# zouyunkai/MedicalSemSeg

Measured on AMD Instinct MI355X. Metric: 96^3 vols/sec fwd+bwd (train), higher is better.
Workload: dtype bf16; 1 GPU; UNet base (MONAI BasicUNet 32-32-64-128-256-32) 1->3cls, 96^3 patches, DiceCE + AdamW, per-GPU batch 2; global_batch=2, parallelism=dp1, grad_sync=none (single rank)

## Files before the change

include/msseg.h:

```cpp
#ifndef MSSEG_H_
#define MSSEG_H_

#include <stddef.h>
#include <stdint.h>

#ifdef __cplusplus
extern "C" {
#endif

#define MSSEG_ABI_VERSION 1

#define MSSEG_OK 0
#define MSSEG_EINVAL (-1)
#define MSSEG_ELAUNCH (-2)
#define MSSEG_EWORKSPACE (-3)

#define MSSEG_F32 0
#define MSSEG_BF16 1

typedef void* msseg_stream_t;

int msseg_abi_version(void);
const char* msseg_last_error(void);
int msseg_num_cus(void);

int msseg_ktimer_enable(int on);
int msseg_ktimer_reset(void);
int msseg_ktimer_count(void);
int msseg_ktimer_get(int i, char* name, int cap, float* ms);

size_t msseg_packed_weight_bytes(int M, int T, int K, int cout_block, int dtype);
int msseg_pack_weights(const float* src, void* dst, int dtype, int M, int M0, int T, int K, int K0,
                       long long s_m1, long long s_m0, long long s_t, long long s_k1, long long s_k0,
                       int flip, int cout_block, msseg_stream_t stream);
typedef struct msseg_pack_job {
    const float* src;
    void* dst;
    long long s_m1, s_m0, s_t, s_k1, s_k0;
    long long total;
    int M, M0, T, K, K0, flip, cout_block, nkb;
} msseg_pack_job;
int msseg_pack_weights_batch(const msseg_pack_job* jobs_dev, int njobs, long long max_total, long long sum_total, int dtype,
                             msseg_stream_t stream);
int msseg_cout_block(int M);
int msseg_conv3d_k3_cout_block(int N, int D, int H, int W, int Cout);
int msseg_conv3d_k3_variant(int N, int D, int H, int W, int Cout);
int msseg_conv3d_k3_kernel(int N, int D, int H, int W, int Cin, int Cout, int dtype);

int msseg_conv3d_k3_fwd(const void* x, long long ldx, const void* wp, const float* bias, void* y, long long ldy,
                        int N, int D, int H, int W, int Cin, int Cout, float* stats ,
                        void* scratch, size_t scratch_bytes, int dtype, msseg_stream_t stream);
int msseg_conv3d_k3_fwd_accumulate(const void* x, long long ldx, const void* wp, void* y, long long ldy, int N, int D, int H,
                                   int W, int Cin, int Cout, float* stats, void* scratch, size_t scratch_bytes, int dtype,
                                   msseg_stream_t stream);
int msseg_conv3d_k3_dgrad_inbwd(const void* dy, long long lddy, const void* wp, void* da, long long ldda, int N, int D,
                                int H, int W, int Cin, int Cout, const void* yraw, long long ldyraw, const void* act,
                                long long ldact, const float* fwd_stats, float slope, float eps, float* red,
                                float* dgamma, float* dbeta, int accumulate, void* scratch, size_t scratch_bytes,
                                int dtype, msseg_stream_t stream);
int msseg_conv3d_k3s2_fwd(const void* x, long long ldx, const void* wp, const float* bias, void* y, long long ldy,
                          int N, int ID, int IH, int IW, int Cin, int Cout, int dtype, msseg_stream_t stream);
int msseg_zero_stuff2(const void* dy, long long lddy, void* out, long long ldo, int N, int OD, int OH, int OW, int ID,
                      int IH, int IW, int C, int dtype, msseg_stream_t stream);
int msseg_conv3d_stem_fwd(const void* x, long long ldx, const void* wp, const float* bias, void* y, long long ldy,
                          int N, int D, int H, int W, int Cout, float* stats, void* scratch, size_t scratch_bytes,
                          int dtype, msseg_stream_t stream);
int msseg_conv3d_stem_k1_fwd(const void* x, long long ldx, const void* wp, const float* bias, void* y, long long ldy,
                             int N, int D, int H, int W, int Cout, float* stats, void* scratch, size_t scratch_bytes,
                             int dtype, msseg_stream_t stream);
int msseg_conv3d_stem_norm_fwd(const void* x, long long ldx, const void* wp, const float* bias, const float* stats,
                               const float* gamma, const float* beta, float eps, float slope, void* y, long long ldy, int N,
                               int D, int H, int W, int Cout, int dtype, msseg_stream_t stream);
int msseg_conv3d_k1_fwd(const void* x, long long ldx, const void* wp, const float* bias, void* y, long long ldy,
                        long long NV, int Cin, int Cout, int dtype, msseg_stream_t stream);
int msseg_conv3d_k1_head_fwd(const void* x, long long ldx, const float* w, const float* bias, void* y, long long ldy,
                             long long NV, int Cin, int Cout, int dtype, msseg_stream_t stream);
int msseg_conv3d_k1_head_dgrad_inbwd(const void* dy, long long lddy, const float* w, void* da, long long ldda, int N,
                                     long long S, int C, int Cout, const void* yraw, long long ldyraw,
                                     const float* fwd_stats, const float* gamma, const float* beta, float slope, float eps,
                                     float* red, float* dgamma, float* dbeta, int accumulate, void* scratch,
                                     size_t scratch_bytes, int dtype, msseg_stream_t stream);
int msseg_conv3d_k1_head_norm_fwd(const void* x, long long ldx, const float* stats, const float* gamma, const float* beta,
                                  float slope, float eps, const float* w, const float* bias, void* y, long long ldy, int N,
                                  long long S, int Cin, int Cout, int dtype, msseg_stream_t stream);
int msseg_conv3d_k1_head_bwd_fused(const void* dy, long long lddy, const float* w, void* da, long long ldda, int N,
                                   long long S, int C, int Cout, const void* yraw, long long ldyraw, const float* fwd_stats,
                                   const float* gamma, const float* beta, float slope, float eps, float* red, float* dgamma,
                                   float* dbeta, int accumulate, float* dw, int dw_accumulate, void* scratch,
                                   size_t scratch_bytes, int dtype, msseg_stream_t stream);

int msseg_conv3d_gather_fwd(const void* x, long long ldx, const void* wp, const float* bias, void* y, long long ldy,
                            int N, int ID, int IH, int IW, int Cin, int Cout, int k, int s, int p, int dtype,
                            msseg_stream_t stream);
int msseg_deconv_k2s2_fwd(const void* x, long long ldx, const void* wp, const float* bias, void* y, long long ldy,
                          int N, int D, int H, int W, int Cin, int Cout, int dtype, msseg_stream_t stream);
int msseg_deconv_k2s2_bwd_data(const void* dy, long long lddy, const void* wp, void* dx, long long lddx,
                               int N, int D, int H, int W, int Cin, int Cout, int dtype, msseg_stream_t stream);
int msseg_deconv_k4s4_fwd(const void* x, long long ldx, const void* wp, const float* bias, void* y, long long ldy,
                          int N, int D, int H, int W, int Cin, int Cout, int dtype, msseg_stream_t stream);
int msseg_deconv_k4s4_bwd_data(const void* dy, long long lddy, const void* wp, void* dx, long long lddx,
                               int N, int D, int H, int W, int Cin, int Cout, int dtype, msseg_stream_t stream);
int msseg_conv3d_k1_dgrad_inbwd(const void* dy, long long lddy, const void* wp, void* da, long long ldda, int N,
                                long long S, int Cin, int Cout, const void* yraw, long long ldyraw, const void* act,
                                long long ldact, const float* fwd_stats, float slope, float eps, float* red,
                                float* dgamma, float* dbeta, int accumulate, void* scratch, size_t scratch_bytes,
                                int dtype, msseg_stream_t stream);
int msseg_deconv_k2s2_bwd_data_inbwd(const void* dy, long long lddy, const void* wp, void* dx, long long lddx, int N,
                                     int D, int H, int W, int Cin, int Cout, const void* yraw, long long ldyraw,
                                     const void* act, long long ldact, const float* fwd_stats, float slope, float eps,
                                     float* red, float* dgamma, float* dbeta, int accumulate, void* scratch,
                                     size_t scratch_bytes, int dtype, msseg_stream_t stream);
int msseg_deconv_k2s2_bwd_fused(const void* dy, long long lddy, const void* wp, void* dx, long long lddx, int N,
                                int D, int H, int W, int Cin, int Cout, const void* yraw, long long ldyraw,
                                const void* act, long long ldact, const float* fwd_stats, float slope, float eps,
                                float* red, float* dgamma, float* dbeta, int accumulate, float* dbias, int dbias_accumulate,
                                void* scratch, size_t scratch_bytes, int dtype, msseg_stream_t stream);

int msseg_deconv_k2s2_bwd_partials_ok(int Cin, int Cout, int dtype);
int msseg_deconv_k2s2_bwd_partials(const void* dy, long long lddy, const void* wp, float* part, size_t part_bytes, int N,
                                   int D, int H, int W, int Cin, int Cout, int dtype, msseg_stream_t stream);


size_t msseg_wgrad_workspace_bytes(int M, int T, int K);
int msseg_conv3d_k3_wgrad_kernel(int N, int D, int H, int W, int Cin, int Cout, int dtype);
int msseg_conv3d_k3_wgrad(const void* x, long long ldx, const void* dy, long long lddy, float* dw,
                          int N, int D, int H, int W, int Cin, int Cout, int accumulate,
                          void* workspace, size_t workspace_bytes, int dtype, msseg_stream_t stream);
int msseg_conv3d_k1_wgrad(const void* x, long long ldx, const void* dy, long long lddy, float* dw,
                          long long NV, int Cin, int Cout, int accumulate,
                          void* workspace, size_t workspace_bytes, int dtype, msseg_stream_t stream);
int msseg_linear_wgrad_ok(long long NV, int Cin, int Cout, int dtype);
int msseg_linear_wgrad(const void* x, long long ldx, const void* dy, long long lddy, float* dw, float* dbias, long long NV,
                       int Cin, int Cout, int accumulate_w, int accumulate_b, void* workspace, size_t workspace_bytes,
                       int dtype, msseg_stream_t stream);
int msseg_conv3d_gather_wgrad(const void* x, long long ldx, const void* dy, long long lddy, float* dw,
                              int N, int ID, int IH, int IW, int Cin, int Cout, int k, int s, int p, int accumulate,
                              void* workspace, size_t workspace_bytes, int dtype, msseg_stream_t stream);
int msseg_deconv_k2s2_wgrad(const void* x, long long ldx, const void* dy, long long lddy, float* dw,
                            int N, int D, int H, int W, int Cin, int Cout, int accumulate,
                            void* workspace, size_t workspace_bytes, int dtype, msseg_stream_t stream);
int msseg_deconv_k4s4_wgrad(const void* x, long long ldx, const void* dy, long long lddy, float* dw,
                            int N, int D, int H, int W, int Cin, int Cout, int accumulate,
                            void* workspace, size_t workspace_bytes, int dtype, msseg_stream_t stream);

int msseg_conv3d_k3_small_ok(int N, int D, int H, int W, int Cin, int Cout, int dtype);
int msseg_conv3d_k3_small_stage_groups(int N, int D, int H, int W, int Cin, int Cout);
size_t msseg_conv3d_k3_small_workspace_bytes(int N, int D, int H, int W, int Cin, int Cout);
int msseg_conv3d_k3_small_partials(const void* x, long long ldx, const void* wp, float* part, size_t part_bytes, int N,
                                   int D, int H, int W, int Cin, int Cout, msseg_stream_t stream);
int msseg_conv3d_k3_small_fwd_finish(const float* part, int nstages, const float* bias, const float* gamma,
                                     const float* beta, float eps, float slope, void* yraw, long long ldy, void* act,
                                     long long lda, void* pooled, long long ldp, float* stats, int N, int D, int H, int W,
                                     int Cout, msseg_stream_t stream);
int msseg_conv3d_k3_small_fwd_finish_res(const float* part, int nstages, const float* bias, const float* gamma,
                                         const float* beta, float eps, float slope, void* yraw, long long ldy, void* act,
                                         long long lda, const void* residual, long long ldr, void* pooled, long long ldp,
                                         float* stats, int N, int D, int H, int W, int Cout, msseg_stream_t stream);
int msseg_conv3d_k3_small_bwd_finish(const float* part, int nstages, void* dx, long long lddx, const void* unit_yraw,
                                     long long lduy, const float* unit_stats, const float* unit_gamma,
                                     const float* unit_beta, float eps, float slope, float* dgamma, float* dbeta,
                                     int accumulate, int N, int D, int H, int W, int Cin, msseg_stream_t stream);

int msseg_dwconv3d_k3_fwd(const void* x, long long ldx, const void* w_taps, const float* bias, void* y, long long ldy, int N,
                          int D, int H, int W, int C, int flip, int dtype, msseg_stream_t stream);
int msseg_avgpool3d_k3(const void* x, long long ldx, void* y, long long ldy, int N, int D, int H, int W, int C, int dtype,
                       msseg_stream_t stream);
int msseg_dwconv3d_k3_wgrad(const void* x, long long ldx, const void* dy, long long lddy, float* dw, float* dbias,
                            int accumulate_w, int accumulate_b, int N, int D, int H, int W, int C, void* scratch,
                            size_t scratch_bytes, int dtype, msseg_stream_t stream);

int msseg_interp_trilinear_fwd(const void* x, long long ldx, void* y, long long ldy, int N, int ID, int IH, int IW, int OD,
                               int OH, int OW, int C, int dtype, msseg_stream_t stream);
size_t msseg_interp_trilinear_bwd_workspace_bytes(int N, int ID, int IH, int IW, int OD, int OH, int OW, int C);
int msseg_interp_trilinear_bwd(const void* dy, long long lddy, void* dx, long long lddx, int N, int ID, int IH, int IW, int OD,
                               int OH, int OW, int C, void* workspace, size_t workspace_bytes, int dtype, msseg_stream_t stream);
int msseg_kv_attention_fwd(const void* q, const void* kv, void* o, float* lse, int B, int N, int M, int heads, int head_dim,
                           float scale, int dtype, msseg_stream_t stream);
size_t msseg_kv_attention_bwd_workspace_bytes(int B, int N, int M, int heads, int head_dim);
int msseg_kv_attention_bwd(const void* q, const void* kv, const void* o, const float* lse, const void* dout, void* dq, void* dkv,
                           int B, int N, int M, int heads, int head_dim, float scale, void* workspace, size_t workspace_bytes,
                           int dtype, msseg_stream_t stream);
int msseg_scale_channels(const void* x, const float* scale, void* y, int N, long long S, int C, int dtype, msseg_stream_t stream);

size_t msseg_reduce_scratch_bytes(void);
int msseg_channel_stats(const void* x, long long ldx, float* stats, int N, long long S, int C, void* scratch,
                        size_t scratch_bytes, int dtype, msseg_stream_t stream);
int msseg_instnorm_act_fwd(const void* x, long long ldx, const float* stats, const float* gamma, const float* beta,
                           const void* residual, long long ldr, void* y, long long ldy, int N, long long S, int C,
                           float eps, float slope, int dtype, msseg_stream_t stream);
int msseg_instnorm_act_pool_fwd(const void* x, long long ldx, const float* stats, const float* gamma, const float* beta,
                                void* y, long long ldy, void* pooled, long long ldp, int N, int D, int H, int W, int C,
                                float eps, float slope, int dtype, msseg_stream_t stream);
int msseg_instnorm_act_poolbwd_reduce(const void* x, long long ldx, const float* stats, const float* gamma,
                                      const float* beta, const void* skip, long long lds, const void* g, long long ldg,
                                      void* da, long long ldda, float* red, float* dgamma, float* dbeta, int accumulate,
                                      int N, int D, int H, int W, int C, float eps, float slope, void* scratch,
                                      size_t scratch_bytes, int dtype, msseg_stream_t stream);
int msseg_instnorm_act_bwd_reduce(const void* x, long long ldx, const float* stats, const float* gamma,
                                  const float* beta, const void* y, long long ldy,
                                  const void* dy, long long lddy, float* red, float* dgamma, float* dbeta,
                                  int accumulate, int N, long long S, int C, float eps, float slope, void* scratch,
                                  size_t scratch_bytes, int dtype, msseg_stream_t stream);
int msseg_instnorm_act_bwd_apply(const void* x, long long ldx, const float* stats, const float* gamma,
                                 const float* beta, const void* y, long long ldy, const void* dy, long long lddy, const float* red, void* dx,
                                 long long lddx, void* dres, long long lddres, int N, long long S, int C, float eps,
                                 float slope, int dtype, msseg_stream_t stream);
int msseg_maxpool2_fwd(const void* x, long long ldx, void* y, long long ldy, int N, int D, int H, int W, int C,
                       int dtype, msseg_stream_t stream);
int msseg_maxpool2_bwd(const void* x, long long ldx, const void* dy, long long lddy, void* dx, long long lddx,
                       int N, int D, int H, int W, int C, int accumulate, int dtype, msseg_stream_t stream);
int msseg_ncdhw_to_ndhwc(const void* src, int src_dtype, void* dst, long long ldd, int dst_dtype, int N, int C,
                         long long S, msseg_stream_t stream);
int msseg_ndhwc_to_ncdhw(const void* src, long long lds, int src_dtype, void* dst, int dst_dtype, int N, int C,
                         long long S, msseg_stream_t stream);
int msseg_channel_sum(const void* x, long long ldx, float* out, long long rows, int C, int accumulate, void* scratch,
                      size_t scratch_bytes, int dtype, msseg_stream_t stream);
int msseg_add(const void* a, long long lda, const void* b, long long ldb, void* y, long long ldy, long long rows,
              int C, int dtype, msseg_stream_t stream);
int msseg_axpy_rows(const void* a, const void* b, const float* scale, void* y, int N, long long elems_per_sample, int dtype,
                    msseg_stream_t stream);


int msseg_window_attention_fwd(const void* qkv, const float* qkv_bias, const float* table, void* out, float* lse, int B,
                               int S, int H, int W, int C, int heads, int ws, int shift, int dtype,
                               msseg_stream_t stream);
int msseg_window_attention_bwd(const void* qkv, const float* qkv_bias, const float* table, const void* out,
                               const float* lse, const void* dout, void* dqkv, float* dtable, int B, int S, int H, int W,
                               int C, int heads, int ws, int shift, int dtype, msseg_stream_t stream);
size_t msseg_window_attention_bwd_workspace_bytes(int B, int S, int H, int W, int C, int heads, int ws, int shift, int dtype);
int msseg_window_attention_fwd2(const void* qkv, const float* qkv_bias, const float* table, void* out, float* lse, int B,
                                int S, int H, int W, int C, int heads, int ws, int shift, int bias_ws, int dtype,
                                msseg_stream_t stream);
int msseg_window_attention_bwd2(const void* qkv, const float* qkv_bias, const float* table, const void* out,
                                const float* lse, const void* dout, void* dqkv, float* dtable, int B, int S, int H, int W,
                                int C, int heads, int ws, int shift, int bias_ws, int dtype, void* workspace,
                                size_t workspace_bytes, msseg_stream_t stream);
int msseg_window_attention_bwd_ws(const void* qkv, const float* qkv_bias, const float* table, const void* out,
                                  const float* lse, const void* dout, void* dqkv, float* dtable, int B, int S, int H, int W,
                                  int C, int heads, int ws, int shift, int dtype, void* workspace, size_t workspace_bytes,
                                  msseg_stream_t stream);
int msseg_window_attention_fwd3(const void* qkv, const float* qkv_bias, const float* table, void* out, float* lse, int B,
                                int S, int H, int W, int C, int heads, int ws, int shift, int bias_ws, long long table_stride,
                                int dtype, msseg_stream_t stream);
int msseg_window_attention_bwd3(const void* qkv, const float* qkv_bias, const float* table, const void* out,
                                const float* lse, const void* dout, void* dqkv, float* dtable, int B, int S, int H, int W,
                                int C, int heads, int ws, int shift, int bias_ws, long long table_stride, int dtype,
                                void* workspace, size_t workspace_bytes, msseg_stream_t stream);
size_t msseg_window_attention_bwd3_workspace_bytes(int B, int S, int H, int W, int C, int heads, int ws, int shift,
                                                   int bias_ws, long long table_stride, int dtype);
int msseg_rel_bias_affine_fold(const float* table, const float* emb, const float* lin_w, const float* lin_b,
                               const float* aff, float* T, int B, int M3, int heads, msseg_stream_t stream);
size_t msseg_rel_bias_affine_grad_workspace_bytes(int M3, int heads);
#define MSSEG_AFFINE_ACC_TABLE 1
#define MSSEG_AFFINE_ACC_EMB 2
#define MSSEG_AFFINE_ACC_LIN_W 4
#define MSSEG_AFFINE_ACC_LIN_B 8
int msseg_rel_bias_affine_grad(const float* dT, const float* emb, const float* lin_w, const float* aff, float* dtable,
                               float* demb, float* dlin_w, float* dlin_b, int B, int M3, int heads, int flags,
                               void* workspace, size_t workspace_bytes, msseg_stream_t stream);
int msseg_layernorm_fwd(const void* x, long long ldx, const float* gamma, const float* beta, void* y, long long ldy,
                        float* mean, float* rstd, long long rows, int C, float eps, int dtype, msseg_stream_t stream);
int msseg_layernorm_bwd(const void* x, long long ldx, const float* gamma, const float* mean, const float* rstd,
                        const void* dy, long long lddy, void* dx, long long lddx, long long rows, int C, int dtype,
                        msseg_stream_t stream);
int msseg_layernorm_bwd_add(const void* x, long long ldx, const float* gamma, const float* mean, const float* rstd,
                            const void* dy, long long lddy, const void* add, long long ldadd, void* dx, long long lddx,
                            long long rows, int C, int dtype, msseg_stream_t stream);
int msseg_layernorm_param_grad(const void* x, long long ldx, const float* mean, const float* rstd, const void* dy,
                               long long lddy, float* dgamma, float* dbeta, int accumulate, long long rows, int C,
                               void* scratch, size_t scratch_bytes, int dtype, msseg_stream_t stream);
int msseg_gelu_fwd(const void* x, void* y, long long n, int dtype, msseg_stream_t stream);
int msseg_gelu_bwd(const void* x, const void* dy, void* dx, long long n, int dtype, msseg_stream_t stream);
int msseg_linear_gelu_ok(long long NV, int Cin, int Cout, int dtype);
int msseg_linear_gelu_fwd(const void* x, long long ldx, const void* wp, const float* bias, void* pre, long long ldpre, void* act,
                          long long ldact, long long NV, int Cin, int Cout, int dtype, msseg_stream_t stream);
int msseg_linear_gelu_bwd(const void* dy, long long lddy, const void* wp, const void* pre, long long ldpre, void* dpre,
                          long long lddpre, long long NV, int Cin, int Cout, int dtype, msseg_stream_t stream);
int msseg_linear_add_ok(long long NV, int Cin, int Cout, int dtype);
int msseg_linear_add_fwd(const void* x, long long ldx, const void* wp, const float* bias, const void* res, long long ldres,
                         void* y, long long ldy, long long NV, int Cin, int Cout, int dtype, msseg_stream_t stream);
// ... 74 lines not shown
```

medicalsemseg_amd/csrc/common.h:

```cpp
#pragma once
#include <hip/hip_runtime.h>
#include <stdint.h>
#include <stdio.h>

#include "../../include/msseg.h"

typedef __bf16 bf16_t;
typedef __attribute__((ext_vector_type(8))) __bf16 bf16x8_t;
typedef __attribute__((ext_vector_type(4))) __bf16 bf16x4_t;
typedef __attribute__((ext_vector_type(4))) float f32x4_t;
typedef __attribute__((ext_vector_type(4))) uint32_t u32x4_t;
typedef __attribute__((ext_vector_type(2))) uint32_t u32x2_t;

#define MSSEG_DEVFN __device__ __forceinline__

void msseg_set_error(const char* fmt, ...);
#define MSSEG_FAIL(code, ...)           \
    do {                                \
        msseg_set_error(__VA_ARGS__);   \
        return (code);                  \
    } while (0)
#define MSSEG_CHECK_LAUNCH(name)                                              \
    do {                                                                      \
        hipError_t e__ = hipGetLastError();                                   \
        if (e__ != hipSuccess) MSSEG_FAIL(MSSEG_ELAUNCH, "%s: %s", name, hipGetErrorString(e__)); \
    } while (0)

bool msseg_ktimer_on();
int msseg_ktimer_begin(const char* name, hipStream_t stream);
void msseg_ktimer_end(int slot, hipStream_t stream);
#define MSSEG_KTIMED(name, stream, launch_stmt)                               \
    do {                                                                      \
        const int kt__ = msseg_ktimer_on() ? msseg_ktimer_begin(name, stream) : -1; \
        launch_stmt;                                                          \
        if (kt__ >= 0) msseg_ktimer_end(kt__, stream);                        \
    } while (0)

#include <atomic>
struct msseg_lds_attr_once {
    std::atomic<unsigned long long> done{0};
    bool ensure(const void* kern, int bytes) {
        int dev = 0;
        if (hipGetDevice(&dev) != hipSuccess) return false;
        const bool tracked = dev >= 0 && dev < 64;
        if (tracked && ((done.load(std::memory_order_acquire) >> dev) & 1ull)) return true;
        if (hipFuncSetAttribute(kern, hipFuncAttributeMaxDynamicSharedMemorySize, bytes) != hipSuccess) return false;
        if (tracked) done.fetch_or(1ull << dev, std::memory_order_release);
        return true;
    }
};

template <typename T> struct DT;
template <> struct DT<float> {
    static constexpr int EPC = 4;
    static constexpr int CODE = MSSEG_F32;
    static MSSEG_DEVFN float ld(const float* p) { return *p; }
    static MSSEG_DEVFN void st(float* p, float v) { *p = v; }
};
template <> struct DT<bf16_t> {
    static constexpr int EPC = 8;
    static constexpr int CODE = MSSEG_BF16;
    static MSSEG_DEVFN float ld(const bf16_t* p) { return (float)*p; }
    static MSSEG_DEVFN void st(bf16_t* p, float v) { *p = (bf16_t)v; }
};

template <typename T> MSSEG_DEVFN void mma_chunk(f32x4_t& acc, const u32x4_t& a, const u32x4_t& b);
template <> MSSEG_DEVFN void mma_chunk<bf16_t>(f32x4_t& acc, const u32x4_t& a, const u32x4_t& b) {
    acc = __builtin_amdgcn_mfma_f32_16x16x32_bf16(__builtin_bit_cast(bf16x8_t, a), __builtin_bit_cast(bf16x8_t, b),
                                                  acc, 0, 0, 0);
}
template <> MSSEG_DEVFN void mma_chunk<float>(f32x4_t& acc, const u32x4_t& a, const u32x4_t& b) {
    f32x4_t af = __builtin_bit_cast(f32x4_t, a), bf = __builtin_bit_cast(f32x4_t, b);
#pragma unroll
    for (int j = 0; j < 4; ++j) acc = __builtin_amdgcn_mfma_f32_16x16x4f32(af[j], bf[j], acc, 0, 0, 0);
}

template <typename T> MSSEG_DEVFN void store4(T* p, const f32x4_t& v);
template <> MSSEG_DEVFN void store4<float>(float* p, const f32x4_t& v) { *(f32x4_t*)p = v; }
template <> MSSEG_DEVFN void store4<bf16_t>(bf16_t* p, const f32x4_t& v) {
    bf16x4_t o = {(bf16_t)v[0], (bf16_t)v[1], (bf16_t)v[2], (bf16_t)v[3]};
    *(bf16x4_t*)p = o;
}

MSSEG_DEVFN float wave_sum(float v) {
#pragma unroll
    for (int o = 32; o > 0; o >>= 1) v += __shfl_xor(v, o);
    return v;
}

MSSEG_DEVFN bool grid_last_block(unsigned int* counter, unsigned int total_blocks, int* lds_flag) {
    asm volatile("s_waitcnt vmcnt(0)" ::: "memory");
    __syncthreads();
    if (threadIdx.x == 0) {
        __builtin_amdgcn_fence(__ATOMIC_RELEASE, "agent");
        asm volatile("s_waitcnt vmcnt(0)" ::: "memory");
        const unsigned int prev = __hip_atomic_fetch_add(counter, 1u, __ATOMIC_RELAXED, __HIP_MEMORY_SCOPE_AGENT);
        const int last = (prev == total_blocks - 1u) ? 1 : 0;
        if (last) {
            __builtin_amdgcn_fence(__ATOMIC_ACQUIRE, "agent");
            asm volatile("s_waitcnt vmcnt(0)" ::: "memory");
            __hip_atomic_store(counter, 0u, __ATOMIC_RELAXED, __HIP_MEMORY_SCOPE_AGENT);
        }
        *lds_flag = last;
    }
    __syncthreads();
    return *lds_flag != 0;
}

template <int NT>
MSSEG_DEVFN void block_rows_sum(const float* rows, int R, int L, float* lds, long long stride = 0) {
    const int tid = threadIdx.x, q = L >> 2;
    const int SL = NT / q;
    const int c4 = tid % q, slot = tid / q;
    const long long q_stride = (stride ? stride : (long long)L) >> 2;
    f32x4_t* l4 = (f32x4_t*)lds;
    if (slot < SL) {
        f32x4_t acc = {0.f, 0.f, 0.f, 0.f};
        const f32x4_t* src = (const f32x4_t*)rows + c4;
#pragma unroll 8
        for (int x = slot; x < R; x += SL) acc += src[(long long)x * q_stride];
        l4[slot * q + c4] = acc;
    }
    __syncthreads();
    if (tid < q) {
        f32x4_t t = {0.f, 0.f, 0.f, 0.f};
        for (int sl = 0; sl < SL; ++sl) t += l4[sl * q + tid];
        l4[NT + tid] = t;
    }
    __syncthreads();
}

#define MSSEG_SCRATCH_COUNTER_BYTES 256
#define MSSEG_STATS_NMAX 8

static inline int ceil_div(int a, int b) { return (a + b - 1) / b; }
static inline long long ceil_div_ll(long long a, long long b) { return (a + b - 1) / b; }
```

medicalsemseg_amd/csrc/conv3d_k3_pp.hip:

```cpp
#include "k3pp.h"

#include <type_traits>

namespace {

constexpr int TD = 4, TH = 4, TW = 16;
constexpr int PD = TD + 2, PH = TH + 2, PW = TW + 2;
constexpr int HV = PD * PH * PW;
constexpr int PLANE = ((HV * 16 + 255) / 256) * 256;
constexpr int HALO_BYTES = 4 * PLANE;
constexpr int W_BYTES = 27 * 4 * 32 * 16;
constexpr int STAT_FLOATS = 8 * MSSEG_STATS_NMAX * 32 * 2;
constexpr int NTHREADS = 512;

__device__ u32x4_t g_zero_chunk;
__device__ unsigned long long g_k3pp_cycles[8];

MSSEG_DEVFN void glds16(const void* g, void* l) {
    __builtin_amdgcn_global_load_lds((const __attribute__((address_space(1))) void*)g,
                                     (__attribute__((address_space(3))) void*)l, 16, 0, 0);
}

struct TileCo { int n, d0, h0, w0; };

// ... 107 lines not shown
        for (int m = 0; m < TH; ++m)
#pragma unroll
            for (int j = 0; j < 2; ++j) acc[m][j] = bv[j];
        const int v0 = (wq * PH) * PW + r;
        const unsigned char* xb[8];
#pragma unroll
        for (int k = 0; k < 8; ++k)
            xb[k] = ldsH + grp * HALO_BYTES + v0 * 64 + ((q ^ ((((v0 + k) >> 2) & 1) << 1)) * 16);
        const unsigned char* wb = ldsW + (q * 32 + r) * 16;
        constexpr int NSTEP = 9 * PH;
        constexpr int XAHEAD = 3;
        u32x4_t wf[2][3][2], xf[XAHEAD + 1];
        auto ldw = [&](int g, int i) {
            const int kh = i >> 1, j = i & 1;
            const int tap = (g / 3) * 9 + kh * 3 + (g % 3);
            wf[g & 1][kh][j] = *(const u32x4_t*)(wb + tap * 2048 + j * 256);
        };
        auto ldx = [&](int s) {
            const int g = s / PH, hr = s % PH;
            const int off = ((g / 3) * PH + hr) * PW + (g % 3);
            xf[s % (XAHEAD + 1)] = *(const u32x4_t*)(xb[off & 7] + off * 64);
        };
#pragma unroll
        for (int i = 0; i < 6; ++i) ldw(0, i);
#pragma unroll
        for (int s = 0; s < XAHEAD; ++s) ldx(s);
#pragma unroll
        for (int g = 0; g < 9; ++g) {
#pragma unroll
            for (int hr = 0; hr < PH; ++hr) {
                const int s = g * PH + hr;
                if (s + XAHEAD < NSTEP) ldx(s + XAHEAD);
                if (g + 1 < 9) ldw(g + 1, hr);
                __builtin_amdgcn_sched_barrier(0);
#pragma unroll
                for (int kh = 0; kh < 3; ++kh) {
                    const int m = hr - kh;
                    if (m >= 0 && m < TH) {
#pragma unroll
                        for (int j = 0; j < 2; ++j)
                            mma_chunk<bf16_t>(acc[m][j], wf[g & 1][kh][j], xf[s % (XAHEAD + 1)]);
                    }
                }
                __builtin_amdgcn_sched_barrier(0);
            }
        }
    };

    unsigned o_off[TH], ny_off[TH], na_off[TH];
#pragma unroll
    for (int m = 0; m < TH; ++m) {
        const long long rel = ((long long)wq * p.H + m) * p.W + r;
        o_off[m] = (unsigned)(rel * p.ldy * 2 + q * 8);
        ny_off[m] = (unsigned)(rel * p.nb_ldy * 2 + q * 8);
        na_off[m] = (unsigned)(rel * p.nb_lda * 2 + q * 8);
    }
    float s1[2][4], s2[2][4];
    int s_n = -1;
#pragma unroll
    for (int j = 0; j < 2; ++j)
#pragma unroll
        for (int e = 0; e < 4; ++e) s1[j][e] = s2[j][e] = 0.f;
    auto flush_stats = [&]() {
        if (s_n < 0) return;
        float* slot = ldsS + ((wave * MSSEG_STATS_NMAX + s_n) * 32) * 2;
#pragma unroll
        for (int j = 0; j < 2; ++j)
#pragma unroll
            for (int e = 0; e < 4; ++e) {
                float a = s1[j][e], b = s2[j][e];
#pragma unroll
                for (int o = 1; o < 16; o <<= 1) {
                    a += __shfl_xor(a, o);
                    b += __shfl_xor(b, o);
                }
                if (r == 0) {
                    float* sp = slot + (j * 16 + q * 4 + e) * 2;
                    sp[0] += a;
                    sp[1] += b;
                }
                s1[j][e] = s2[j][e] = 0.f;
            }
    };
    auto epilogue = [&](const TileCo& tc) {
        if constexpr (STATS != 0) {
            if (tc.n != s_n) { flush_stats(); s_n = tc.n; }
        }
        const long long vox = (((long long)tc.n * p.D + tc.d0) * p.H + tc.h0) * p.W + tc.w0;
        unsigned char* ybase = (unsigned char*)yg + (vox * p.ldy + coutblk * 32) * 2;
        const unsigned char* nyb = (const unsigned char*)p.nb_y + (vox * p.nb_ldy + coutblk * 32) * 2;
        const unsigned char* nab = (const unsigned char*)p.nb_a + (vox * p.nb_lda + coutblk * 32) * 2;
        const bool full = tc.d0 + TD <= p.D && tc.h0 + TH <= p.H && tc.w0 + TW <= p.W;
        auto body = [&](auto fullc) {
            constexpr bool FULL = decltype(fullc)::value;
            const bool okdw = FULL || (tc.d0 + wq < p.D && tc.w0 + r < p.W);
            u32x2_t y4[TH][2], a4[TH][2];
            if constexpr (STATS == 2) {
#pragma unroll
                for (int m = 0; m < TH; ++m)
#pragma unroll
                    for (int j = 0; j < 2; ++j) {
                        const bool ok = FULL || (okdw && tc.h0 + m < p.H);
                        y4[m][j] = a4[m][j] = u32x2_t{0u, 0u};
                        if (ok) {
                            y4[m][j] = *(const u32x2_t*)(nyb + ny_off[m] + j * 32);
                            a4[m][j] = *(const u32x2_t*)(nab + na_off[m] + j * 32);
                        }
                    }
            }
            u32x2_t ob[TH][2];
            if constexpr (STATS == 3) {
                u32x2_t yo[TH][2];
#pragma unroll
                for (int m = 0; m < TH; ++m)
#pragma unroll
                    for (int j = 0; j < 2; ++j) {
                        const bool ok = FULL || (okdw && tc.h0 + m < p.H);
                        yo[m][j] = ok ? *(const u32x2_t*)(ybase + o_off[m] + j * 32) : u32x2_t{0u, 0u};
                    }
#pragma unroll
                for (int m = 0; m < TH; ++m)
#pragma unroll
                    for (int j = 0; j < 2; ++j)
#pragma unroll
                        for (int e = 0; e < 4; ++e) acc[m][j][e] += bf16_of_pair(yo[m][j][e >> 1], e & 1);
            }
#pragma unroll
            for (int m = 0; m < TH; ++m)
#pragma unroll
                for (int j = 0; j < 2; ++j) {
                    const bool ok = FULL || (okdw && tc.h0 + m < p.H);
                    const f32x4_t o = acc[m][j];
                    ob[m][j] = u32x2_t{pack_bf16x2(o[0], o[1]), pack_bf16x2(o[2], o[3])};
                    if (ok) *(u32x2_t*)(ybase + o_off[m] + j * 32) = ob[m][j];
                }
            if constexpr (STATS != 0) {
#pragma unroll
                for (int m = 0; m < TH; ++m)
#pragma unroll
                    for (int j = 0; j < 2; ++j) {
                        const bool ok = FULL || (okdw && tc.h0 + m < p.H);
#pragma unroll
                        for (int e = 0; e < 4; ++e) {
                            float v = bf16_of_pair(ob[m][j][e >> 1], e & 1);
                            if (!FULL) v = ok ? v : 0.f;
                            if constexpr (STATS == 1 || STATS == 3) {
                                acc_add(s1[j][e], v);
                                acc_fma(s2[j][e], v, v);
                            } else {
                                const float av = bf16_of_pair(a4[m][j][e >> 1], e & 1);
                                const float dz = v * (av > 0.f ? 1.0f : p.nb_slope);
                                acc_add(s1[j][e], dz);
                                acc_fma(s2[j][e], dz, bf16_of_pair(y4[m][j][e >> 1], e & 1));
                            }
                        }
                    }
            }
        };
        if (full) body(std::true_type{});
        else body(std::false_type{});
    };

    for (int ph = 0; ph <= n_my; ++ph) {
        unsigned long long t0 = 0;
        if constexpr (TIMING) t0 = __builtin_readcyclecounter();
        if ((ph & 1) == grp) {
            if (ph < n_my) compute();
            if constexpr (TIMING) tcyc[0] += __builtin_readcyclecounter() - t0;
        } else {
            if (ph + 1 < n_my) load_halo(tile_of(ph + 1));
            if constexpr (TIMING) {
                tcyc[4] += __builtin_readcyclecounter() - t0; t0 = __builtin_readcyclecounter();
                asm volatile("s_waitcnt vmcnt(0)" ::: "memory");
                tcyc[5] += __builtin_readcyclecounter() - t0; t0 = __builtin_readcyclecounter();
            }
            if (ph >= 1) epilogue(tile_of(ph - 1));
            if constexpr (TIMING) tcyc[1] += __builtin_readcyclecounter() - t0;
        }
        if constexpr (TIMING) t0 = __builtin_readcyclecounter();
        asm volatile("s_waitcnt vmcnt(0)" ::: "memory");
        if constexpr (TIMING) { tcyc[2] += __builtin_readcyclecounter() - t0; t0 = __builtin_readcyclecounter(); }
        __syncthreads();
        if constexpr (TIMING) tcyc[3] += __builtin_readcyclecounter() - t0;
    }
    if constexpr (TIMING) {
        if (blockIdx.x == 0 && blockIdx.y == 0 && lane == 0 && wave == 0) {
#pragma unroll
            for (int k = 0; k < 6; ++k) g_k3pp_cycles[k] = tcyc[k];
        }
    }

    if constexpr (STATS != 0) {
        flush_stats();
        __syncthreads();
        const int PN = p.N * 32 * 2;
        float* wsp = p.stats_ws + ((long long)blockIdx.y * gridDim.x + blockIdx.x) * PN;
        for (int i = tid; i < PN; i += NTHREADS) {
            float s = 0.f;
#pragma unroll
            for (int wv = 0; wv < 8; ++wv) s += ldsS[wv * MSSEG_STATS_NMAX * 64 + i];
            wsp[i] = s;
        }
    }
}

template <int STATS, int TIMING> int launch(const K3ppParams& p, hipStream_t stream) {
    const int lds = W_BYTES + 2 * HALO_BYTES + (STATS ? STAT_FLOATS * 4 : 0);
    auto kern = k3pp_kernel<STATS, TIMING>;
    static msseg_lds_attr_once attr;
    if (!attr.ensure((const void*)kern, lds)) MSSEG_FAIL(MSSEG_ELAUNCH, "conv3d_k3_pp: cannot set dynamic LDS size %d", lds);
    const int ncb = p.M / 32;
    const int tiles = p.N * ceil_div(p.D, TD) * ceil_div(p.H, TH) * ceil_div(p.W, TW);
    int gx = msseg_num_cus() / ncb;
    gx &= ~7;
    if (gx < 8) gx = 8;
    if (gx > tiles) gx = tiles;
    MSSEG_KTIMED("k3pp_kernel", stream, hipLaunchKernelGGL(kern, dim3(gx, ncb, 1), dim3(NTHREADS), lds, stream, p));
    MSSEG_CHECK_LAUNCH("conv3d_k3_pp");
    if (STATS != 0) {
        K3FinParams f{};
        f.ws = p.stats_ws; f.R = gx; f.N = p.N; f.coutb = 32; f.M = p.M; f.stats = p.stats;
        f.nb_stats = (STATS == 2) ? p.nb_stats : nullptr; f.nb_eps = p.nb_eps; f.nb_S = p.nb_S;
        f.nb_dgamma = p.nb_dgamma; f.nb_dbeta = p.nb_dbeta; f.nb_acc = p.nb_acc;
        return msseg_k3_stats_finalize(f, ncb, stream);
    }
    return MSSEG_OK;
}

}

bool msseg_k3pp_eligible(const K3ppParams& p) {
    if (p.K != 32 || p.M % 32 || p.M > 256) return false;
    if ((p.ldx % 8) || (p.ldy % 4) || ((uintptr_t)p.x & 15) || ((uintptr_t)p.y & 7)) return false;
    if (p.bias && ((uintptr_t)p.bias & 15)) return false;
    if (p.stats && p.N > MSSEG_STATS_NMAX) return false;
    if (p.nb_y && ((p.nb_ldy % 4) || (p.nb_lda % 4) || ((uintptr_t)p.nb_y & 7) || ((uintptr_t)p.nb_a & 7))) return false;
    const long long tiles = (long long)p.N * ceil_div(p.D, TD) * ceil_div(p.H, TH) * ceil_div(p.W, TW);
    if (tiles > 0x7fffffffLL) return false;
    return tiles * (p.M / 32) >= 2LL * msseg_num_cus();
}

int msseg_k3pp_launch(const K3ppParams& p, hipStream_t stream) {
    static const bool timing = getenv("MSSEG_K3PP_TIMING") != nullptr;
    if (p.accumulate) {
        if (p.stats == nullptr || p.nb_y != nullptr) MSSEG_FAIL(MSSEG_EINVAL, "conv3d_k3_pp: accumulate mode comes with forward statistics");
        return launch<3, 0>(p, stream);
    }
    if (p.stats == nullptr) return timing ? launch<0, 1>(p, stream) : launch<0, 0>(p, stream);
    if (p.nb_y == nullptr) return timing ? launch<1, 1>(p, stream) : launch<1, 0>(p, stream);
    return launch<2, 0>(p, stream);
}

extern "C" int msseg_debug_k3pp_cycles(unsigned long long* out8) {
    return hipMemcpyFromSymbol(out8, HIP_SYMBOL(g_k3pp_cycles), 8 * sizeof(unsigned long long)) == hipSuccess ? 0 : -1;
}
```

medicalsemseg_amd/csrc/elementwise.hip:

```cpp
#include "common.h"

#include <stdarg.h>
#include <string.h>

static thread_local char g_err[512] = "";
void msseg_set_error(const char* fmt, ...) {
    va_list ap;
    va_start(ap, fmt);
    vsnprintf(g_err, sizeof(g_err), fmt, ap);
    va_end(ap);
}

extern "C" {
int msseg_abi_version(void) { return MSSEG_ABI_VERSION; }
const char* msseg_last_error(void) { return g_err; }
int msseg_num_cus(void) {
    static int cus = 0;
    if (cus == 0) {
        int dev = 0;
        hipDeviceProp_t prop;
        if (hipGetDevice(&dev) == hipSuccess && hipGetDeviceProperties(&prop, dev) == hipSuccess)
            cus = prop.multiProcessorCount;
        if (cus <= 0) cus = 256;
    }
// ... 243 lines not shown
            }
        }
    }
}

inline long long reduce_blocks(long long S, int rows_par, int N, int C, int nper);

template <typename T>
int launch_ln_param_grad(const void* x, long long ldx, const void* dy, long long lddy, const float* mean, const float* rstd,
                         float* dgamma, float* dbeta, int accumulate, long long rows, int C, void* scratch, hipStream_t st) {
    const bool vec = vec_ok(x, ldx, C, sizeof(T)) && vec_ok(dy, lddy, C, sizeof(T));
    const RowMap m = row_map(C, vec ? DT<T>::EPC : 1);
    long long blocks = reduce_blocks(rows, m.rows_par, 1, C, 2);
    const long long rpb = ceil_div_ll(rows, blocks);
    blocks = ceil_div_ll(rows, rpb);
    unsigned int* counter = (unsigned int*)scratch;
    float* ws = (float*)((unsigned char*)scratch + MSSEG_SCRATCH_COUNTER_BYTES);
    if (vec)
        hipLaunchKernelGGL((ln_param_grad_kernel<T, true>), dim3((unsigned)blocks), dim3(256), 0, st, (const T*)x, ldx,
                           (const T*)dy, lddy, mean, rstd, rows, C, m.groups, m.rows_par, rpb, ws, counter, dgamma, dbeta, accumulate);
    else
        hipLaunchKernelGGL((ln_param_grad_kernel<T, false>), dim3((unsigned)blocks), dim3(256), 0, st, (const T*)x, ldx,
                           (const T*)dy, lddy, mean, rstd, rows, C, m.groups, m.rows_par, rpb, ws, counter, dgamma, dbeta, accumulate);
    MSSEG_CHECK_LAUNCH("ln_param_grad");
    {
        FinalizeArgs a{ws, 1, (int)blocks, C, 2, 2, ws + blocks * C * 2, dgamma, dbeta, accumulate};
        hipLaunchKernelGGL(channels_finalize_kernel, channels_finalize_grid(a), dim3(256), 0, st, a);
        MSSEG_CHECK_LAUNCH("channels_finalize");
    }
    return MSSEG_OK;
}

inline long long reduce_blocks(long long S, int rows_par, int N, int C, int nper) {
    long long blocks = ceil_div_ll(S, (long long)rows_par * 8);
    long long cap = (long long)msseg_num_cus() / (N > 0 ? N : 1);
    if (cap < 1) cap = 1;
    const long long fit = (long long)(((size_t)16 << 20) / ((size_t)N * C * nper * 4));
    if (cap > fit) cap = fit;
    if (blocks > cap) blocks = cap;
    if (blocks < 1) blocks = 1;
    return blocks;
}

template <typename T>
int launch_stats(const void* x, long long ldx, float* out, int N, long long S, int C, int nacc, int accumulate,
                 void* scratch, hipStream_t st) {
    const bool vec = vec_ok(x, ldx, C, sizeof(T));
    const RowMap m = row_map(C, vec ? DT<T>::EPC : 1, RED_THREADS);
    long long blocks = reduce_blocks(S, m.rows_par, N, C, nacc);
    const long long rpb = ceil_div_ll(S, blocks);
    blocks = ceil_div_ll(S, rpb);
    dim3 grid((unsigned)blocks, N);
    unsigned int* counter = (unsigned int*)scratch;
    float* ws = (float*)((unsigned char*)scratch + MSSEG_SCRATCH_COUNTER_BYTES);
    if (vec)
        hipLaunchKernelGGL((channel_stats_kernel<T, true>), grid, dim3(RED_THREADS), 0, st, (const T*)x, ldx, out, S, C,
                           m.groups, m.rows_par, rpb, nacc, accumulate, ws, counter);
    else
        hipLaunchKernelGGL((channel_stats_kernel<T, false>), grid, dim3(RED_THREADS), 0, st, (const T*)x, ldx, out, S, C,
                           m.groups, m.rows_par, rpb, nacc, accumulate, ws, counter);
    MSSEG_CHECK_LAUNCH("channel_stats");
    {
        FinalizeArgs a{ws, N, (int)blocks, C, nacc, nacc == 2 ? 0 : 1, out, nullptr, nullptr, accumulate};
        hipLaunchKernelGGL(channels_finalize_kernel, channels_finalize_grid(a), dim3(256), 0, st, a);
        MSSEG_CHECK_LAUNCH("channels_finalize");
    }
    return MSSEG_OK;
}

struct NormParams {
    const void* x; long long ldx;
    const float* stats; const float* gamma; const float* beta;
    const void* res; long long ldr;
    void* y; long long ldy;
    const void* dy; long long lddy;
    float* red;
    void* dx; long long lddx;
    void* dres; long long lddres;
    long long S; int C; float eps, slope;
    long long rows_per_block; int groups, rows_par;
    float* ws; unsigned int* counter; float* dgamma; float* dbeta; int accumulate;
};

MSSEG_DEVFN void mean_rstd(const float* stats, int n, int C, int c, long long S, float eps, float& mean, float& rstd) {
    const float inv = 1.0f / (float)S;
    const float s = stats[((long long)n * C + c) * 2 + 0], s2 = stats[((long long)n * C + c) * 2 + 1];
    mean = s * inv;
    float var = s2 * inv - mean * mean;
    var = var > 0.f ? var : 0.f;
    rstd = rsqrtf(var + eps);
}

template <typename T, bool VEC, int MODE>
__global__ __launch_bounds__(MODE == 1 ? RED_THREADS : 256) void instnorm_kernel(const NormParams p) {
    constexpr int W = VEC ? DT<T>::EPC : 1;
    __shared__ float red[(MODE == 1) ? RED_THREADS * 2 * W : 1];
    __shared__ int lflag;
    const int n = blockIdx.y;
    const int g = threadIdx.x % p.groups, rl = threadIdx.x / p.groups;
    const long long r0 = (long long)blockIdx.x * p.rows_per_block;
    long long r1 = r0 + p.rows_per_block;
    if (r1 > p.S) r1 = p.S;
    const T* xn = (const T*)p.x + (long long)n * p.S * p.ldx;
    const T* yn = (MODE != 0 && p.y != nullptr) ? (const T*)p.y + (long long)n * p.S * p.ldy : nullptr;
    T* yo = (MODE == 0) ? (T*)p.y + (long long)n * p.S * p.ldy : nullptr;
    const T* dyn = (MODE != 0) ? (const T*)p.dy + (long long)n * p.S * p.lddy : nullptr;
    const T* resn = (MODE == 0 && p.res) ? (const T*)p.res + (long long)n * p.S * p.ldr : nullptr;
    T* dxn = (MODE == 2) ? (T*)p.dx + (long long)n * p.S * p.lddx : nullptr;
    T* drn = (MODE == 2 && p.dres) ? (T*)p.dres + (long long)n * p.S * p.lddres : nullptr;
    const float invS = 1.0f / (float)p.S;

    for (int gbase = 0; gbase * W < p.C; gbase += p.groups) {
        const int gg = gbase + g;
        const bool act = gg * W < p.C;
        float mean[W], rstd[W], sc[W], sh[W], k0[W], k1[W], a0[W], a1[W];
#pragma unroll
        for (int e = 0; e < W; ++e) {
            const int c = act ? gg * W + e : 0;
            mean_rstd(p.stats, n, p.C, c, p.S, p.eps, mean[e], rstd[e]);
            const float ga = p.gamma ? p.gamma[c] : 1.f;
            sc[e] = rstd[e] * ga;
            sh[e] = (p.beta ? p.beta[c] : 0.f) - mean[e] * sc[e];
            a0[e] = a1[e] = 0.f;
            if constexpr (MODE == 2) {
                k0[e] = p.red[((long long)n * p.C + c) * 2 + 0] * invS;
                k1[e] = p.red[((long long)n * p.C + c) * 2 + 1] * invS;
            }
        }
        if (act && rl < p.rows_par) {
#pragma unroll 4
            for (long long r = r0 + rl; r < r1; r += p.rows_par) {
                float xv[W], o[W], yv[W], dv[W];
                if constexpr (VEC) {
                    Chunk<T> c; c.load(xn + r * p.ldx + gg * W);
#pragma unroll
                    for (int e = 0; e < W; ++e) xv[e] = c.v[e];
                } else {
                    xv[0] = DT<T>::ld(xn + r * p.ldx + gg);
                }
                if constexpr (MODE == 0) {
                    float rv[W];
#pragma unroll
                    for (int e = 0; e < W; ++e) rv[e] = 0.f;
                    if (resn) {
                        if constexpr (VEC) {
                            Chunk<T> c; c.load(resn + r * p.ldr + gg * W);
#pragma unroll
                            for (int e = 0; e < W; ++e) rv[e] = c.v[e];
                        } else {
                            rv[0] = DT<T>::ld(resn + r * p.ldr + gg);
                        }
                    }
#pragma unroll
                    for (int e = 0; e < W; ++e) {
                        const float z = xv[e] * sc[e] + sh[e] + rv[e];
                        o[e] = z > 0.f ? z : z * p.slope;
                    }
                    if constexpr (VEC) {
                        Chunk<T> c;
#pragma unroll
                        for (int e = 0; e < W; ++e) c.v[e] = o[e];
                        c.store(yo + r * p.ldy + gg * W);
                    } else {
                        DT<T>::st(yo + r * p.ldy + gg, o[0]);
                    }
                } else {
                    if constexpr (VEC) {
                        Chunk<T> d; d.load(dyn + r * p.lddy + gg * W);
#pragma unroll
                        for (int e = 0; e < W; ++e) dv[e] = d.v[e];
                        if (yn != nullptr) {
                            Chunk<T> c; c.load(yn + r * p.ldy + gg * W);
#pragma unroll
                            for (int e = 0; e < W; ++e) yv[e] = c.v[e];
                        } else {
// ... 53 lines not shown
                        a += red[((k * p.groups + g) * W + e) * 2 + 0];
                        b += red[((k * p.groups + g) * W + e) * 2 + 1];
                    }
                    const int c = gg * W + e;
                    float* wsb = p.ws + ((long long)n * gridDim.x + blockIdx.x) * p.C * 2;
                    wsb[c * 2 + 0] = a;
                    wsb[c * 2 + 1] = b;
                }
            }
        }
    }
}

struct NormPoolParams {
    const void* x; long long ldx;
    const float* stats; const float* gamma; const float* beta;
    void* y; long long ldy;
    void* pooled; long long ldp;
    int N, D, H, W, C; float eps, slope;
};

template <typename T>
__global__ __launch_bounds__(256) void instnorm_pool_fwd_kernel(const NormPoolParams p) {
    constexpr int WD = DT<T>::EPC;
    const int OD = p.D / 2, OH = p.H / 2, OW = p.W / 2;
    const unsigned ug = (unsigned)(p.C / WD);
    const unsigned total = (unsigned)((long long)p.N * OD * OH * OW * ug);
    const long long S = (long long)p.D * p.H * p.W;
    for (unsigned i = blockIdx.x * 256u + threadIdx.x; i < total; i += gridDim.x * 256u) {
        unsigned t = i / ug;
        const int g = (int)(i - t * ug);
        unsigned t2 = t / (unsigned)OW;
        const int ow = (int)(t - t2 * (unsigned)OW);
        t = t2 / (unsigned)OH;
        const int oh = (int)(t2 - t * (unsigned)OH);
        const int n = (int)(t / (unsigned)OD);
        const int od = (int)(t - (unsigned)n * (unsigned)OD);
        float sc[WD], sh[WD], best[WD];
#pragma unroll
        for (int e = 0; e < WD; ++e) {
            const int c = g * WD + e;
            float mean, rstd;
            mean_rstd(p.stats, n, p.C, c, S, p.eps, mean, rstd);
            sc[e] = rstd * (p.gamma ? p.gamma[c] : 1.f);
            sh[e] = (p.beta ? p.beta[c] : 0.f) - mean * sc[e];
            best[e] = -INFINITY;
        }
        Chunk<T> in[8];
#pragma unroll
        for (int k = 0; k < 8; ++k) {
            const long long vox = (((long long)n * p.D + 2 * od + (k >> 2)) * p.H + 2 * oh + ((k >> 1) & 1)) * p.W + 2 * ow + (k & 1);
            in[k].load((const T*)p.x + vox * p.ldx + g * WD);
        }
#pragma unroll
        for (int k = 0; k < 8; ++k) {
            const long long vox = (((long long)n * p.D + 2 * od + (k >> 2)) * p.H + 2 * oh + ((k >> 1) & 1)) * p.W + 2 * ow + (k & 1);
            Chunk<T> o;
#pragma unroll
            for (int e = 0; e < WD; ++e) {
                const float z = in[k].v[e] * sc[e] + sh[e];
                const float a = (float)(T)(z > 0.f ? z : z * p.slope);
                o.v[e] = a;
                if (a > best[e] || a != a) best[e] = a;
            }
            o.store((T*)p.y + vox * p.ldy + g * WD);
        }
        Chunk<T> b;
#pragma unroll
        for (int e = 0; e < WD; ++e) b.v[e] = best[e];
        const long long ovox = (((long long)n * OD + od) * OH + oh) * OW + ow;
        b.store((T*)p.pooled + ovox * p.ldp + g * WD);
    }
}

struct NormPoolBwdParams {
    const void* x; long long ldx;
    const float* stats; const float* gamma; const float* beta;
    const void* skip; long long lds;
    const void* g; long long ldg;
    void* da; long long ldda;
    int N, D, H, W, C; float eps, slope;
    int groups, rows_par; long long cells_per_block;
    float* ws;
};

template <typename T>
__global__ __launch_bounds__(RED_THREADS) void instnorm_poolbwd_reduce_kernel(const NormPoolBwdParams p) {
    constexpr int WD = DT<T>::EPC;
    __shared__ float red[RED_THREADS * 2 * WD];
    const int n = blockIdx.y;
    const int g = threadIdx.x % p.groups, rl = threadIdx.x / p.groups;
    const int OD = p.D / 2, OH = p.H / 2, OW = p.W / 2;
    const long long cells = (long long)OD * OH * OW, S = (long long)p.D * p.H * p.W;
    const long long c0 = (long long)blockIdx.x * p.cells_per_block;
    long long c1 = c0 + p.cells_per_block;
    if (c1 > cells) c1 = cells;
    const T* xn = (const T*)p.x + (long long)n * S * p.ldx;
    const T* sn = (const T*)p.skip + (long long)n * S * p.lds;
    const T* gn = (const T*)p.g + (long long)n * cells * p.ldg;
    T* dn = (T*)p.da + (long long)n * S * p.ldda;
    for (int gbase = 0; gbase * WD < p.C; gbase += p.groups) {
        const int gg = gbase + g;
        const bool act = gg * WD < p.C;
        float mean[WD], rstd[WD], sc[WD], sh[WD], a0[WD], a1[WD];
#pragma unroll
        for (int e = 0; e < WD; ++e) {
            const int c = act ? gg * WD + e : 0;
            mean_rstd(p.stats, n, p.C, c, S, p.eps, mean[e], rstd[e]);
            sc[e] = rstd[e] * (p.gamma ? p.gamma[c] : 1.f);
            sh[e] = (p.beta ? p.beta[c] : 0.f) - mean[e] * sc[e];
            a0[e] = a1[e] = 0.f;
        }
        if (act && rl < p.rows_par) {
            for (long long cell = c0 + rl; cell < c1; cell += p.rows_par) {
                const int ow = (int)(cell % OW), oh = (int)((cell / OW) % OH), od = (int)(cell / ((long long)OW * OH));
                Chunk<T> xin[8], gv;
                Chunk<T> skin[8];
                long long vox[8];
#pragma unroll
                for (int k = 0; k < 8; ++k) {
                    vox[k] = ((long long)(2 * od + (k >> 2)) * p.H + 2 * oh + ((k >> 1) & 1)) * p.W + 2 * ow + (k & 1);
                    xin[k].load(xn + vox[k] * p.ldx + gg * WD);
                }
#pragma unroll
                for (int k = 0; k < 8; ++k) skin[k].load(sn + vox[k] * p.lds + gg * WD);
                gv.load(gn + cell * p.ldg + gg * WD);
                float best[WD];
                int arg[WD];
#pragma unroll
                for (int e = 0; e < WD; ++e) { best[e] = -INFINITY; arg[e] = 0; }
#pragma unroll
                for (int k = 0; k < 8; ++k) {
#pragma unroll
                    for (int e = 0; e < WD; ++e) {
                        const float z = xin[k].v[e] * sc[e] + sh[e];
                        const float a = (float)(T)(z > 0.f ? z : z * p.slope);
                        if (a > best[e] || a != a) { best[e] = a; arg[e] = k; }
                    }
                }
#pragma unroll
                for (int k = 0; k < 8; ++k) {
                    Chunk<T> o;
#pragma unroll
                    for (int e = 0; e < WD; ++e) {
                        const float dv = (float)(T)(skin[k].v[e] + (arg[e] == k ? gv.v[e] : 0.f));
                        o.v[e] = dv;
                        const float z = xin[k].v[e] * sc[e] + sh[e];
                        const float dz = z > 0.f ? dv : dv * p.slope;
                        a0[e] += dz;
                        a1[e] += dz * ((xin[k].v[e] - mean[e]) * rstd[e]);
                    }
                    o.store(dn + vox[k] * p.ldda + gg * WD);
                }
            }
        }
        __syncthreads();
#pragma unroll
        for (int e = 0; e < WD; ++e) {
            red[(threadIdx.x * WD + e) * 2 + 0] = a0[e];
            red[(threadIdx.x * WD + e) * 2 + 1] = a1[e];
        }
        __syncthreads();
        block_rows_reduce<WD>(red, p.groups, p.rows_par, g, rl, act);
        if (act && rl == 0) {
            const int kmax = p.rows_par < RED_STAGE2 ? p.rows_par : RED_STAGE2;
#pragma unroll
            for (int e = 0; e < WD; ++e) {
                float a = 0.f, b = 0.f;
                for (int k = 0; k < kmax; ++k) {
                    a += red[((k * p.groups + g) * WD + e) * 2 + 0];
                    b += red[((k * p.groups + g) * WD + e) * 2 + 1];
                }
                float* wsb = p.ws + ((long long)n * gridDim.x + blockIdx.x) * p.C * 2;
                wsb[(gg * WD + e) * 2 + 0] = a;
                wsb[(gg * WD + e) * 2 + 1] = b;
            }
        }
    }
}

struct HeadBwdParams {
    const void* dy; long long lddy;
    const float* w;
    const void* x; long long ldx;
    const float* stats; const float* gamma; const float* beta;
    void* da; long long ldda;
    long long S; int C, Cout; float eps, slope;
    int groups, rows_par; long long rows_per_block;
    float* ws;
    int want_dw;
};

struct HeadFinArgs {
    const float* ws; int N, nblk, C, nper, Cout; float* red; float* dbeta; float* dgamma; float* dw; int acc_norm, acc_dw;
};
__global__ __launch_bounds__(256) void head_finalize_kernel(const HeadFinArgs a) {
    __shared__ __attribute__((aligned(16))) float fin[256 * 4 + 64 * 6];
    __shared__ float tot_n[64 * 6];
    const int L = a.C * a.nper;
    for (int o = threadIdx.x; o < L; o += 256) tot_n[o] = 0.f;
    for (int n = 0; n < a.N; ++n) {
        block_rows_sum<256>(a.ws + (long long)n * a.nblk * L, a.nblk, L, fin);
        const float* t = fin + 256 * 4;
        for (int o = threadIdx.x; o < L; o += 256) {
            const int c = o / a.nper, k = o % a.nper;
            if (k < 2) a.red[((long long)n * a.C + c) * 2 + k] = t[o];
            tot_n[o] += t[o];
        }
        __syncthreads();
    }
    for (int o = threadIdx.x; o < L; o += 256) {
        const int c = o / a.nper, k = o % a.nper;
        const float tot = tot_n[o];
        if (k == 0) { if (a.dbeta) a.dbeta[c] = a.acc_norm ? a.dbeta[c] + tot : tot; }
        else if (k == 1) { if (a.dgamma) a.dgamma[c] = a.acc_norm ? a.dgamma[c] + tot : tot; }
        else if (k - 2 < a.Cout && a.dw) a.dw[(k - 2) * a.C + c] = a.acc_dw ? a.dw[(k - 2) * a.C + c] + tot : tot;
    }
}

template <typename T, bool DW>
__global__ __launch_bounds__(RED_THREADS) void head_dgrad_inbwd_kernel(const HeadBwdParams p) {
    constexpr int WD = DT<T>::EPC;
    __shared__ float red[RED_THREADS * 2 * WD];
    const int n = blockIdx.y;
    const int g = threadIdx.x % p.groups, rl = threadIdx.x / p.groups;
    const long long r0 = (long long)blockIdx.x * p.rows_per_block;
    long long r1 = r0 + p.rows_per_block;
    if (r1 > p.S) r1 = p.S;
    const T* xn = (const T*)p.x + (long long)n * p.S * p.ldx;
    const T* dyn = (const T*)p.dy + (long long)n * p.S * p.lddy;
    T* dan = (T*)p.da + (long long)n * p.S * p.ldda;
    for (int gbase = 0; gbase * WD < p.C; gbase += p.groups) {
        const int gg = gbase + g;
        const bool act = gg * WD < p.C;
        float mean[WD], rstd[WD], sc[WD], sh[WD], a0[WD], a1[WD], wv[4][WD];
        float gw[DW ? 4 : 1][WD];
#pragma unroll
        for (int e = 0; e < WD; ++e) {
            const int c = act ? gg * WD + e : 0;
            mean_rstd(p.stats, n, p.C, c, p.S, p.eps, mean[e], rstd[e]);
            sc[e] = rstd[e] * (p.gamma ? p.gamma[c] : 1.f);
            sh[e] = (p.beta ? p.beta[c] : 0.f) - mean[e] * sc[e];
            a0[e] = a1[e] = 0.f;
#pragma unroll
            for (int k = 0; k < 4; ++k) wv[k][e] = k < p.Cout ? (float)(T)p.w[k * p.C + c] : 0.f;
#pragma unroll
            for (int k = 0; k < (DW ? 4 : 1); ++k) gw[k][e] = 0.f;
        }
        if (act && rl < p.rows_par) {
            constexpr int UNR = DW ? 2 : 4;
#pragma unroll UNR
            for (long long r = r0 + rl; r < r1; r += p.rows_par) {
                Chunk<T> xc, dc, o;
                xc.load(xn + r * p.ldx + gg * WD);
                dc.load(dyn + r * p.lddy);
#pragma unroll
                for (int e = 0; e < WD; ++e) {
                    float acc = 0.f;
#pragma unroll
// ... 638 lines not shown
    blocks = ceil_div_ll(S, p.rows_per_block);
    dim3 grid((unsigned)blocks, N);
    if (dw) {
        DISPATCH_T(dtype, hipLaunchKernelGGL((head_dgrad_inbwd_kernel<float, true>), grid, dim3(RED_THREADS), 0, (hipStream_t)stream, p),
                   hipLaunchKernelGGL((head_dgrad_inbwd_kernel<bf16_t, true>), grid, dim3(RED_THREADS), 0, (hipStream_t)stream, p));
    } else {
        DISPATCH_T(dtype, hipLaunchKernelGGL((head_dgrad_inbwd_kernel<float, false>), grid, dim3(RED_THREADS), 0, (hipStream_t)stream, p),
                   hipLaunchKernelGGL((head_dgrad_inbwd_kernel<bf16_t, false>), grid, dim3(RED_THREADS), 0, (hipStream_t)stream, p));
    }
    MSSEG_CHECK_LAUNCH("conv3d_k1_head_dgrad_inbwd");
    HeadFinArgs a{p.ws, N, (int)blocks, C, nper, Cout, red, dbeta, dgamma, dw, accumulate, dw_accumulate};
    hipLaunchKernelGGL(head_finalize_kernel, dim3(1), dim3(256), 0, (hipStream_t)stream, a);
    MSSEG_CHECK_LAUNCH("head_finalize");
    return MSSEG_OK;
}

int msseg_conv3d_k1_head_dgrad_inbwd(const void* dy, long long lddy, const float* w, void* da, long long ldda, int N,
                                     long long S, int C, int Cout, const void* yraw, long long ldyraw,
                                     const float* fwd_stats, const float* gamma, const float* beta, float slope, float eps,
                                     float* red, float* dgamma, float* dbeta, int accumulate, void* scratch,
                                     size_t scratch_bytes, int dtype, msseg_stream_t stream) {
    return head_bwd_impl(dy, lddy, w, da, ldda, N, S, C, Cout, yraw, ldyraw, fwd_stats, gamma, beta, slope, eps, red, dgamma,
                         dbeta, accumulate, nullptr, 0, scratch, scratch_bytes, dtype, stream);
}

int msseg_conv3d_k1_head_bwd_fused(const void* dy, long long lddy, const float* w, void* da, long long ldda, int N,
                                   long long S, int C, int Cout, const void* yraw, long long ldyraw, const float* fwd_stats,
                                   const float* gamma, const float* beta, float slope, float eps, float* red, float* dgamma,
                                   float* dbeta, int accumulate, float* dw, int dw_accumulate, void* scratch,
                                   size_t scratch_bytes, int dtype, msseg_stream_t stream) {
    if (!dw) MSSEG_FAIL(MSSEG_EINVAL, "conv3d_k1_head_bwd_fused: dw is required");
    return head_bwd_impl(dy, lddy, w, da, ldda, N, S, C, Cout, yraw, ldyraw, fwd_stats, gamma, beta, slope, eps, red, dgamma,
                         dbeta, accumulate, dw, dw_accumulate, scratch, scratch_bytes, dtype, stream);
}

int msseg_conv3d_k1_head_norm_fwd(const void* x, long long ldx, const float* stats, const float* gamma, const float* beta,
                                  float slope, float eps, const float* w, const float* bias, void* y, long long ldy, int N,
                                  long long S, int Cin, int Cout, int dtype, msseg_stream_t stream) {
    if (!x || !stats || !w || !y || N < 1 || S < 1) MSSEG_FAIL(MSSEG_EINVAL, "conv3d_k1_head_norm: bad args");
    const int esz = dtype == MSSEG_F32 ? 4 : 2;
    if (dtype != MSSEG_F32 && dtype != MSSEG_BF16) MSSEG_FAIL(MSSEG_EINVAL, "conv3d_k1_head_norm: bad dtype");
    if ((gamma == nullptr) != (beta == nullptr)) MSSEG_FAIL(MSSEG_EINVAL, "conv3d_k1_head_norm: gamma/beta go together");
    if (Cout < 1 || Cout > 4 || Cin < 1 || Cin > 64 || !vec_ok(x, ldx, Cin, esz) || ldy < Cout)
        MSSEG_FAIL(MSSEG_EINVAL, "conv3d_k1_head_norm: needs 1 <= Cout <= 4, Cin <= 64 in 16-byte chunks (got %d -> %d)", Cin, Cout);
    long long gx = ceil_div_ll(S, 256);
    const long long cap = (long long)msseg_num_cus() * 16 / N + 1;
    if (gx > cap) gx = cap;
    dim3 grid((unsigned)gx, N);
#define HEADN(T_, C_) hipLaunchKernelGGL((conv1x1_head_norm_kernel<T_, C_>), grid, dim3(256), 0, (hipStream_t)stream, \
                                         (const T_*)x, ldx, stats, gamma, beta, slope, eps, w, bias, (T_*)y, ldy, S, Cin)
#define HEADN_C(T_) do { if (Cout == 1) HEADN(T_, 1); else if (Cout == 2) HEADN(T_, 2); else if (Cout == 3) HEADN(T_, 3); else HEADN(T_, 4); } while (0)
    DISPATCH_T(dtype, HEADN_C(float), HEADN_C(bf16_t));
#undef HEADN_C
#undef HEADN
    MSSEG_CHECK_LAUNCH("conv3d_k1_head_norm");
    return MSSEG_OK;
}

int msseg_instnorm_act_pool_fwd(const void* x, long long ldx, const float* stats, const float* gamma, const float* beta,
                                void* y, long long ldy, void* pooled, long long ldp, int N, int D, int H, int W, int C,
                                float eps, float slope, int dtype, msseg_stream_t stream) {
    if (!x || !stats || !y || !pooled || N < 1 || D < 2 || H < 2 || W < 2 || C < 1)
        MSSEG_FAIL(MSSEG_EINVAL, "instnorm_act_pool_fwd: bad args");
    if ((D | H | W) & 1) MSSEG_FAIL(MSSEG_EINVAL, "instnorm_act_pool_fwd: odd spatial size %dx%dx%d", D, H, W);
    const int esz = dtype == MSSEG_F32 ? 4 : 2;
    if (dtype != MSSEG_F32 && dtype != MSSEG_BF16) MSSEG_FAIL(MSSEG_EINVAL, "instnorm_act_pool_fwd: bad dtype");
    if (!(vec_ok(x, ldx, C, esz) && vec_ok(y, ldy, C, esz) && vec_ok(pooled, ldp, C, esz)))
        MSSEG_FAIL(MSSEG_EINVAL, "instnorm_act_pool_fwd: needs 16-byte aligned rows and a channel count multiple of %d", 16 / esz);
    const long long total = (long long)N * (D / 2) * (H / 2) * (W / 2) * (C / (16 / esz));
    if (total >= 0x7fffffffLL) MSSEG_FAIL(MSSEG_EINVAL, "instnorm_act_pool_fwd: too many elements");
    NormPoolParams p{x, ldx, stats, gamma, beta, y, ldy, pooled, ldp, N, D, H, W, C, eps, slope};
    const int g = grid_for(total, 1);
    DISPATCH_T(dtype, hipLaunchKernelGGL(instnorm_pool_fwd_kernel<float>, dim3(g), dim3(256), 0, (hipStream_t)stream, p),
               hipLaunchKernelGGL(instnorm_pool_fwd_kernel<bf16_t>, dim3(g), dim3(256), 0, (hipStream_t)stream, p));
    MSSEG_CHECK_LAUNCH("instnorm_act_pool_fwd");
    return MSSEG_OK;
}

int msseg_instnorm_act_poolbwd_reduce(const void* x, long long ldx, const float* stats, const float* gamma,
                                      const float* beta, const void* skip, long long lds, const void* g, long long ldg,
                                      void* da, long long ldda, float* red, float* dgamma, float* dbeta, int accumulate,
                                      int N, int D, int H, int W, int C, float eps, float slope, void* scratch,
                                      size_t scratch_bytes, int dtype, msseg_stream_t stream) {
    if (!x || !stats || !skip || !g || !da || !red || N < 1 || D < 2 || H < 2 || W < 2 || C < 1)
        MSSEG_FAIL(MSSEG_EINVAL, "instnorm_act_poolbwd_reduce: bad args");
    if ((D | H | W) & 1) MSSEG_FAIL(MSSEG_EINVAL, "instnorm_act_poolbwd_reduce: odd spatial size %dx%dx%d", D, H, W);
    if (dtype != MSSEG_F32 && dtype != MSSEG_BF16) MSSEG_FAIL(MSSEG_EINVAL, "instnorm_act_poolbwd_reduce: bad dtype");
    if (int rc = scratch_ok(scratch, scratch_bytes, "instnorm_act_poolbwd_reduce")) return rc;
    const int esz = dtype == MSSEG_F32 ? 4 : 2;
    if (!(vec_ok(x, ldx, C, esz) && vec_ok(skip, lds, C, esz) && vec_ok(g, ldg, C, esz) && vec_ok(da, ldda, C, esz)))
        MSSEG_FAIL(MSSEG_EINVAL, "instnorm_act_poolbwd_reduce: needs 16-byte aligned rows and a channel count multiple of %d",
                   16 / esz);
    NormPoolBwdParams p{x, ldx, stats, gamma, beta, skip, lds, g, ldg, da, ldda, N, D, H, W, C, eps, slope, 0, 0, 0, nullptr};
    p.ws = (float*)((unsigned char*)scratch + MSSEG_SCRATCH_COUNTER_BYTES);
    const RowMap m = row_map(C, 16 / esz, RED_THREADS);
    p.groups = m.groups; p.rows_par = m.rows_par;
    const long long cells = (long long)(D / 2) * (H / 2) * (W / 2);
    long long blocks = reduce_blocks(cells * 8, m.rows_par, N, C, 2);
    p.cells_per_block = ceil_div_ll(cells, blocks);
    blocks = ceil_div_ll(cells, p.cells_per_block);
    dim3 grid((unsigned)blocks, N);
    DISPATCH_T(dtype,
               hipLaunchKernelGGL(instnorm_poolbwd_reduce_kernel<float>, grid, dim3(RED_THREADS), 0, (hipStream_t)stream, p),
               hipLaunchKernelGGL(instnorm_poolbwd_reduce_kernel<bf16_t>, grid, dim3(RED_THREADS), 0, (hipStream_t)stream, p));
    MSSEG_CHECK_LAUNCH("instnorm_act_poolbwd_reduce");
    FinalizeArgs a{p.ws, N, (int)blocks, C, 2, 2, red, dbeta, dgamma, accumulate};
    hipLaunchKernelGGL(channels_finalize_kernel, channels_finalize_grid(a), dim3(256), 0, (hipStream_t)stream, a);
    MSSEG_CHECK_LAUNCH("channels_finalize");
    return MSSEG_OK;
}

int msseg_instnorm_act_bwd_reduce(const void* x, long long ldx, const float* stats, const float* gamma,
                                  const float* beta, const void* y, long long ldy,
                                  const void* dy, long long lddy, float* red, float* dgamma, float* dbeta,
                                  int accumulate, int N, long long S, int C, float eps, float slope, void* scratch,
                                  size_t scratch_bytes, int dtype, msseg_stream_t stream) {
    if (!x || !stats || !dy || !red) MSSEG_FAIL(MSSEG_EINVAL, "instnorm_act_bwd_reduce: null pointer");
    if (int rc = scratch_ok(scratch, scratch_bytes, "instnorm_act_bwd_reduce")) return rc;
    NormParams p{};
    p.counter = (unsigned int*)scratch;
    p.ws = (float*)((unsigned char*)scratch + MSSEG_SCRATCH_COUNTER_BYTES);
    p.dgamma = dgamma; p.dbeta = dbeta; p.accumulate = accumulate;
    p.x = x; p.ldx = ldx; p.stats = stats; p.gamma = gamma; p.beta = beta; p.y = (void*)y; p.ldy = ldy; p.dy = dy; p.lddy = lddy; p.red = red;
    p.S = S; p.C = C; p.eps = eps; p.slope = slope;
    const int esz = dtype == MSSEG_F32 ? 4 : 2;
    const bool vec = vec_ok(x, ldx, C, esz) && vec_ok(y, ldy, C, esz) && vec_ok(dy, lddy, C, esz);
    DISPATCH_T(dtype, return (launch_norm<float, 1>(p, N, vec, (hipStream_t)stream)),
               return (launch_norm<bf16_t, 1>(p, N, vec, (hipStream_t)stream)));
}

int msseg_instnorm_act_bwd_apply(const void* x, long long ldx, const float* stats, const float* gamma,
                                 const float* beta, const void* y, long long ldy, const void* dy, long long lddy, const float* red, void* dx,
                                 long long lddx, void* dres, long long lddres, int N, long long S, int C, float eps,
                                 float slope, int dtype, msseg_stream_t stream) {
    if (!x || !stats || !dy || !red || !dx) MSSEG_FAIL(MSSEG_EINVAL, "instnorm_act_bwd_apply: null pointer");
    NormParams p{};
    p.x = x; p.ldx = ldx; p.stats = stats; p.gamma = gamma; p.beta = beta; p.y = (void*)y; p.ldy = ldy; p.dy = dy; p.lddy = lddy;
    p.red = (float*)red; p.dx = dx; p.lddx = lddx; p.dres = dres; p.lddres = lddres;
    p.S = S; p.C = C; p.eps = eps; p.slope = slope;
    const int esz = dtype == MSSEG_F32 ? 4 : 2;
    const bool vec = vec_ok(x, ldx, C, esz) && vec_ok(y, ldy, C, esz) && vec_ok(dy, lddy, C, esz) &&
                     vec_ok(dx, lddx, C, esz) && (!dres || vec_ok(dres, lddres, C, esz));
    DISPATCH_T(dtype, return (launch_norm<float, 2>(p, N, vec, (hipStream_t)stream)),
               return (launch_norm<bf16_t, 2>(p, N, vec, (hipStream_t)stream)));
}

int msseg_maxpool2_fwd(const void* x, long long ldx, void* y, long long ldy, int N, int D, int H, int W, int C,
                       int dtype, msseg_stream_t stream) {
    if (!x || !y || D < 2 || H < 2 || W < 2 || C < 1) MSSEG_FAIL(MSSEG_EINVAL, "maxpool2_fwd: bad args");
    const int esz = dtype == MSSEG_F32 ? 4 : 2;
    const bool vec = vec_ok(x, ldx, C, esz) && vec_ok(y, ldy, C, esz);
    const long long total = (long long)N * (D / 2) * (H / 2) * (W / 2) * ceil_div(C, vec ? 16 / esz : 1);
    if (total >= 0x7fffffffLL) MSSEG_FAIL(MSSEG_EINVAL, "maxpool2_fwd: too many elements");
    const int g = grid_for(total, 1);
#define MP_F(T_, V_) hipLaunchKernelGGL((maxpool2_kernel<T_, V_, false>), dim3(g), dim3(256), 0, (hipStream_t)stream, \
                                        (const T_*)x, ldx, (const T_*)nullptr, 0LL, (T_*)y, ldy, N, D, H, W, C, 0)
    DISPATCH_T(dtype, if (vec) MP_F(float, true); else MP_F(float, false),
               if (vec) MP_F(bf16_t, true); else MP_F(bf16_t, false));
#undef MP_F
    MSSEG_CHECK_LAUNCH("maxpool2_fwd");
    return MSSEG_OK;
}

int msseg_maxpool2_bwd(const void* x, long long ldx, const void* dy, long long lddy, void* dx, long long lddx, int N,
                       int D, int H, int W, int C, int accumulate, int dtype, msseg_stream_t stream) {
    if (!x || !dy || !dx || D < 2 || H < 2 || W < 2 || C < 1) MSSEG_FAIL(MSSEG_EINVAL, "maxpool2_bwd: bad args");
    const int esz = dtype == MSSEG_F32 ? 4 : 2;
    const bool vec = vec_ok(x, ldx, C, esz) && vec_ok(dy, lddy, C, esz) && vec_ok(dx, lddx, C, esz);
    const long long total = (long long)N * (D / 2) * (H / 2) * (W / 2) * ceil_div(C, vec ? 16 / esz : 1);
    if (total >= 0x7fffffffLL) MSSEG_FAIL(MSSEG_EINVAL, "maxpool2_bwd: too many elements");
    const int g = grid_for(total, 1);
#define MP_B(T_, V_) hipLaunchKernelGGL((maxpool2_kernel<T_, V_, true>), dim3(g), dim3(256), 0, (hipStream_t)stream, \
                                        (const T_*)x, ldx, (const T_*)dy, lddy, (T_*)dx, lddx, N, D, H, W, C, accumulate)
    DISPATCH_T(dtype, if (vec) MP_B(float, true); else MP_B(float, false),
               if (vec) MP_B(bf16_t, true); else MP_B(bf16_t, false));
#undef MP_B
    MSSEG_CHECK_LAUNCH("maxpool2_bwd");
    return MSSEG_OK;
}

int msseg_ncdhw_to_ndhwc(const void* src, int src_dtype, void* dst, long long ldd, int dst_dtype, int N, int C,
                         long long S, msseg_stream_t stream) {
    if (!src || !dst || N < 1 || C < 1 || S < 1 || ldd < C) MSSEG_FAIL(MSSEG_EINVAL, "ncdhw_to_ndhwc: bad args");
    const int g = grid_for((long long)N * C * S);
    hipStream_t st = (hipStream_t)stream;
    if (src_dtype == MSSEG_F32 && dst_dtype == MSSEG_F32)
        hipLaunchKernelGGL((ncdhw_to_ndhwc_kernel<float, float>), dim3(g), dim3(256), 0, st, (const float*)src, (float*)dst, ldd, N, C, S);
    else if (src_dtype == MSSEG_F32 && dst_dtype == MSSEG_BF16)
        hipLaunchKernelGGL((ncdhw_to_ndhwc_kernel<float, bf16_t>), dim3(g), dim3(256), 0, st, (const float*)src, (bf16_t*)dst, ldd, N, C, S);
    else if (src_dtype == MSSEG_BF16 && dst_dtype == MSSEG_BF16)
        hipLaunchKernelGGL((ncdhw_to_ndhwc_kernel<bf16_t, bf16_t>), dim3(g), dim3(256), 0, st, (const bf16_t*)src, (bf16_t*)dst, ldd, N, C, S);
// ... 110 lines not shown
```

medicalsemseg_amd/csrc/igemm_fwd.hip:

```cpp
#include "common.h"
#include "k3pp.h"

#include <type_traits>

namespace {

enum { SRC_DIRECT = 0, SRC_GATHER = 1, SRC_DECONV_BWD = 2 };
enum { EPI_STORE = 0, EPI_DECONV = 1 };

struct IgemmParams {
    const void* x;
    long long ldx;
    const void* wp;
    const float* bias;
    void* y;
    long long ldy;
    int N, D, H, W;
    int ID, IH, IW;
    int OD, OH, OW;
    int K, M, NKB;
    int tiles_d, tiles_h, tiles_w;
    int ntiles;
    int cin, k, s, p;
    int creal;
// ... 638 lines not shown
    if (M <= 16) return 16;
    if (M % 32 == 0) return 32;
    if (M % 48 == 0) return 48;
    return 32;
}

int msseg_conv3d_k3_cout_block(int N, int D, int H, int W, int Cout) {
    int cfg, cb;
    k3_plan(N, D, H, W, Cout, &cfg, &cb);
    return cb;
}

int msseg_conv3d_k3_variant(int N, int D, int H, int W, int Cout) {
    int cfg, cb;
    k3_plan(N, D, H, W, Cout, &cfg, &cb);
    return cfg;
}

int msseg_conv3d_k3_kernel(int N, int D, int H, int W, int Cin, int Cout, int dtype) {
    int cfg, cb;
    if (dtype == MSSEG_BF16 && Cin == 48 && msseg_k3c48_shape_ok(N, D, H, W, Cout)) return 4;
    k3_plan(N, D, H, W, Cout, &cfg, &cb);
    if (dtype == MSSEG_BF16 && cb == 32) {
        K3ppParams pp{};
        pp.x = (const void*)256; pp.y = (void*)256; pp.ldx = Cin; pp.ldy = Cout;
        pp.N = N; pp.D = D; pp.H = H; pp.W = W; pp.K = Cin; pp.M = Cout;
        if ((Cin % 8) == 0 && (Cout % 4) == 0 && msseg_k3pp_eligible(pp)) return 3;
    }
    return cfg;
}

static int k3_fwd_impl(const void* x, long long ldx, const void* wp, const float* bias, void* y, long long ldy, int N,
                       int D, int H, int W, int Cin, int Cout, float* stats, void* scratch, size_t scratch_bytes,
                       const void* nb_y, long long nb_ldy, const void* nb_a, long long nb_lda, const float* nb_stats,
                       float nb_slope, float nb_eps, float* nb_dgamma, float* nb_dbeta, int nb_acc, int dtype,
                       msseg_stream_t stream);

int msseg_conv3d_k3_fwd(const void* x, long long ldx, const void* wp, const float* bias, void* y, long long ldy,
                        int N, int D, int H, int W, int Cin, int Cout, float* stats, void* scratch,
                        size_t scratch_bytes, int dtype, msseg_stream_t stream) {
    return k3_fwd_impl(x, ldx, wp, bias, y, ldy, N, D, H, W, Cin, Cout, stats, scratch, scratch_bytes, nullptr, 0, nullptr,
                       0, nullptr, 0.f, 0.f, nullptr, nullptr, 0, dtype, stream);
}

int msseg_conv3d_k3_fwd_accumulate(const void* x, long long ldx, const void* wp, void* y, long long ldy, int N, int D, int H,
                                   int W, int Cin, int Cout, float* stats, void* scratch, size_t scratch_bytes, int dtype,
                                   msseg_stream_t stream) {
    if (!x || !wp || !y || !stats) MSSEG_FAIL(MSSEG_EINVAL, "conv3d_k3_fwd_accumulate: null pointer");
    if (dtype != MSSEG_BF16 || N < 1 || N > MSSEG_STATS_NMAX) MSSEG_FAIL(MSSEG_EINVAL, "conv3d_k3_fwd_accumulate: bf16, N <= %d", MSSEG_STATS_NMAX);
    if (!scratch || ((uintptr_t)scratch & 255) || scratch_bytes < msseg_reduce_scratch_bytes())
        MSSEG_FAIL(MSSEG_EWORKSPACE, "conv3d_k3_fwd_accumulate: needs the reduce scratch of %zu bytes", msseg_reduce_scratch_bytes());
    K3ppParams pp{};
    pp.x = x; pp.ldx = ldx; pp.wp = wp; pp.y = y; pp.ldy = ldy;
    pp.N = N; pp.D = D; pp.H = H; pp.W = W; pp.K = Cin; pp.M = Cout;
    pp.stats = stats; pp.counter = (unsigned int*)scratch;
    pp.stats_ws = (float*)((unsigned char*)scratch + MSSEG_SCRATCH_COUNTER_BYTES);
    pp.accumulate = 1;
    if (Cin == 48) {
        if (!msseg_k3c48_eligible(pp))
            MSSEG_FAIL(MSSEG_EINVAL, "conv3d_k3_fwd_accumulate: 48 input channels need a shape and operands the 48-channel "
                                     "kernel takes (msseg_conv3d_k3_kernel() == 4, 16-byte aligned x, N <= 4)");
        return msseg_k3c48_launch(pp, (hipStream_t)stream);
    }
    if (!msseg_k3pp_eligible(pp))
        MSSEG_FAIL(MSSEG_EINVAL, "conv3d_k3_fwd_accumulate: only shapes of the ping-pong kernel (32 input channels, Cout %% 32 == 0, "
                                 "large grids; msseg_conv3d_k3_kernel() == 3)");
    return msseg_k3pp_launch(pp, (hipStream_t)stream);
}

int msseg_conv3d_k3_dgrad_inbwd(const void* dy, long long lddy, const void* wp, void* da, long long ldda, int N, int D,
                                int H, int W, int Cin, int Cout, const void* yraw, long long ldyraw, const void* act,
                                long long ldact, const float* fwd_stats, float slope, float eps, float* red,
                                float* dgamma, float* dbeta, int accumulate, void* scratch, size_t scratch_bytes,
                                int dtype, msseg_stream_t stream) {
    if (!yraw || !act || !fwd_stats || !red) MSSEG_FAIL(MSSEG_EINVAL, "conv3d_k3_dgrad_inbwd: null pointer");
    if ((dgamma == nullptr) != (dbeta == nullptr)) MSSEG_FAIL(MSSEG_EINVAL, "conv3d_k3_dgrad_inbwd: dgamma/dbeta go together");
    const int esz = dtype == MSSEG_F32 ? 4 : 2;
    if (Cout % 4 || (ldyraw % 4) || (ldact % 4) || ((uintptr_t)yraw % (4 * esz)) || ((uintptr_t)act % (4 * esz)))
        MSSEG_FAIL(MSSEG_EINVAL, "conv3d_k3_dgrad_inbwd: channel count / strides must be multiples of 4");
    return k3_fwd_impl(dy, lddy, wp, nullptr, da, ldda, N, D, H, W, Cin, Cout, red, scratch, scratch_bytes, yraw, ldyraw,
                       act, ldact, fwd_stats, slope, eps, dgamma, dbeta, accumulate, dtype, stream);
}

static int k3_fwd_impl(const void* x, long long ldx, const void* wp, const float* bias, void* y, long long ldy, int N,
                       int D, int H, int W, int Cin, int Cout, float* stats, void* scratch, size_t scratch_bytes,
                       const void* nb_y, long long nb_ldy, const void* nb_a, long long nb_lda, const float* nb_stats,
                       float nb_slope, float nb_eps, float* nb_dgamma, float* nb_dbeta, int nb_acc, int dtype,
                       msseg_stream_t stream) {
    const int esz = dtype == MSSEG_F32 ? 4 : 2;
    int rc = check_common(x, ldx, wp, y, ldy, dtype, esz);
    if (rc) return rc;
    if (N < 1 || D < 1 || H < 1 || W < 1 || Cin < 1 || Cout < 1) MSSEG_FAIL(MSSEG_EINVAL, "conv3d_k3: bad shape");
    if (Cin % (16 / esz)) MSSEG_FAIL(MSSEG_EINVAL, "conv3d_k3: Cin=%d must be a multiple of %d (use conv3d_gather)", Cin, 16 / esz);
    if (ldx < Cin || ldy < Cout) MSSEG_FAIL(MSSEG_EINVAL, "conv3d_k3: ld smaller than channels");
    IgemmParams p{};
    p.x = x; p.ldx = ldx; p.wp = wp; p.bias = bias; p.y = y; p.ldy = ldy;
    p.N = N; p.D = D; p.H = H; p.W = W; p.K = Cin; p.M = Cout;
    if (stats) {
        if (N > MSSEG_STATS_NMAX) MSSEG_FAIL(MSSEG_EINVAL, "conv3d_k3: fused statistics need N <= %d", MSSEG_STATS_NMAX);
        if (Cout > 64 * 16) MSSEG_FAIL(MSSEG_EINVAL, "conv3d_k3: fused statistics need Cout <= 1024 (one counter per cout block)");
        if (!scratch || ((uintptr_t)scratch & 255) || scratch_bytes < msseg_reduce_scratch_bytes())
            MSSEG_FAIL(MSSEG_EWORKSPACE, "conv3d_k3: fused statistics need a zero-initialised scratch of %zu bytes",
                       msseg_reduce_scratch_bytes());
        p.stats = stats;
        p.counter = (unsigned int*)scratch;
        p.stats_ws = (float*)((unsigned char*)scratch + MSSEG_SCRATCH_COUNTER_BYTES);
        p.nb_y = nb_y; p.nb_ldy = nb_ldy; p.nb_a = nb_a; p.nb_lda = nb_lda; p.nb_stats = nb_stats;
        p.nb_slope = nb_slope; p.nb_eps = nb_eps; p.nb_S = (long long)D * H * W;
        p.nb_dgamma = nb_dgamma; p.nb_dbeta = nb_dbeta; p.nb_acc = nb_acc;
    }
    if (dtype == MSSEG_BF16) {
        K3ppParams pp{};
        pp.x = x; pp.ldx = ldx; pp.wp = wp; pp.bias = bias; pp.y = y; pp.ldy = ldy;
        pp.N = N; pp.D = D; pp.H = H; pp.W = W; pp.K = Cin; pp.M = Cout;
        pp.stats = p.stats; pp.stats_ws = p.stats_ws; pp.counter = p.counter;
        pp.nb_y = p.nb_y; pp.nb_ldy = p.nb_ldy; pp.nb_a = p.nb_a; pp.nb_lda = p.nb_lda; pp.nb_stats = p.nb_stats;
        pp.nb_slope = p.nb_slope; pp.nb_eps = p.nb_eps; pp.nb_S = p.nb_S;
        pp.nb_dgamma = p.nb_dgamma; pp.nb_dbeta = p.nb_dbeta; pp.nb_acc = p.nb_acc;
        if (Cin == 48 && msseg_k3c48_shape_ok(N, D, H, W, Cout)) {
            if (!msseg_k3c48_eligible(pp))
                MSSEG_FAIL(MSSEG_EINVAL, "conv3d_k3: 48-input-channel layer on a large grid needs 16-byte aligned x, 8-byte "
                                         "aligned y and ldx <= 256");
            return msseg_k3c48_launch(pp, (hipStream_t)stream);
        }
        int cfg, cb;
        k3_plan(N, D, H, W, Cout, &cfg, &cb);
        if (cb == 32 && msseg_k3pp_eligible(pp)) return msseg_k3pp_launch(pp, (hipStream_t)stream);
    }
    return dtype == MSSEG_F32 ? launch_k3<float>(p, (hipStream_t)stream) : launch_k3<bf16_t>(p, (hipStream_t)stream);
}

int msseg_conv3d_k3s2_fwd(const void* x, long long ldx, const void* wp, const float* bias, void* y, long long ldy,
                          int N, int ID, int IH, int IW, int Cin, int Cout, int dtype, msseg_stream_t stream) {
    const int esz = dtype == MSSEG_F32 ? 4 : 2;
    int rc = check_common(x, ldx, wp, y, ldy, dtype, esz);
    if (rc) return rc;
    if (N < 1 || ID < 1 || IH < 1 || IW < 1 || Cin < 1 || Cout < 1) MSSEG_FAIL(MSSEG_EINVAL, "conv3d_k3s2: bad shape");
    if (Cin % (16 / esz)) MSSEG_FAIL(MSSEG_EINVAL, "conv3d_k3s2: Cin=%d must be a multiple of %d", Cin, 16 / esz);
    IgemmParams p{};
    p.x = x; p.ldx = ldx; p.wp = wp; p.bias = bias; p.y = y; p.ldy = ldy;
    p.N = N; p.ID = ID; p.IH = IH; p.IW = IW;
    p.D = (ID - 1) / 2 + 1; p.H = (IH - 1) / 2 + 1; p.W = (IW - 1) / 2 + 1;
    p.K = Cin; p.M = Cout;
    return dtype == MSSEG_F32 ? launch_nt<float, 27, SRC_DIRECT, EPI_STORE, 2, 4, 8, 4, 2>(p, (hipStream_t)stream)
                              : launch_nt<bf16_t, 27, SRC_DIRECT, EPI_STORE, 2, 4, 8, 4, 2>(p, (hipStream_t)stream);
}

int msseg_conv3d_stem_norm_fwd(const void* x, long long ldx, const void* wp, const float* bias, const float* stats,
                               const float* gamma, const float* beta, float eps, float slope, void* y, long long ldy, int N,
                               int D, int H, int W, int Cout, int dtype, msseg_stream_t stream) {
    if (!x || !wp || !y || !stats || N < 1 || D < 1 || H < 1 || W < 1) MSSEG_FAIL(MSSEG_EINVAL, "conv3d_stem_norm: bad args");
    if (!msseg_stem_eligible(dtype, 1, Cout, 3, 1, 1, ldx, ldy, y))
        MSSEG_FAIL(MSSEG_EINVAL, "conv3d_stem_norm: bf16, Cout a multiple of 32 or 48 (<= 256), 8-byte aligned output rows only");
    StemParams sp{};
    sp.x = x; sp.ldx = ldx; sp.wp = wp; sp.bias = bias; sp.y = y; sp.ldy = ldy;
    sp.N = N; sp.D = D; sp.H = H; sp.W = W; sp.M = Cout;
    sp.nstats = stats; sp.gamma = gamma; sp.beta = beta; sp.eps = eps; sp.slope = slope;
    return msseg_stem_fwd_launch(sp, (hipStream_t)stream);
}

int msseg_conv3d_k1_fwd(const void* x, long long ldx, const void* wp, const float* bias, void* y, long long ldy,
                        long long NV, int Cin, int Cout, int dtype, msseg_stream_t stream) {
    const int esz = dtype == MSSEG_F32 ? 4 : 2;
    int rc = check_common(x, ldx, wp, y, ldy, dtype, esz);
    if (rc) return rc;
    if (NV < 1 || NV > 0x7fffffffLL || Cin < 1 || Cout < 1) MSSEG_FAIL(MSSEG_EINVAL, "conv3d_k1: bad shape");
// ... 206 lines not shown
```

medicalsemseg_amd/csrc/k3pp.h:

```cpp
#pragma once
#include "common.h"

struct K3ppParams {
    const void* x;
    long long ldx;
    const void* wp;
    const float* bias;
    void* y;
    long long ldy;
    int N, D, H, W, K, M;
    float* stats;
    float* stats_ws;
    unsigned int* counter;
    const void* nb_y; long long nb_ldy;
    const void* nb_a; long long nb_lda;
    const float* nb_stats;
    float nb_slope, nb_eps; long long nb_S;
    float* nb_dgamma; float* nb_dbeta; int nb_acc;
    int accumulate;
};

bool msseg_k3pp_eligible(const K3ppParams& p);
int msseg_k3pp_launch(const K3ppParams& p, hipStream_t stream);

bool msseg_k3c48_shape_ok(int N, int D, int H, int W, int M);
bool msseg_k3c48_eligible(const K3ppParams& p);
int msseg_k3c48_launch(const K3ppParams& p, hipStream_t stream);

struct K3FinParams {
    const float* ws;
    int R, N, coutb, M;
    float* stats;
    const float* nb_stats;
    float nb_eps; long long nb_S;
    float* nb_dgamma; float* nb_dbeta; int nb_acc;
};
int msseg_k3_stats_finalize(const K3FinParams& f, int ncb, hipStream_t stream);

struct K3WgParams {
    const void* pten; long long ldp;
    const void* qten; long long ldq;
    float* slabs;
    int N, D, H, W, M, K, kblks;
};
bool msseg_k3wg_pp_eligible(const K3WgParams& p);
int msseg_k3wg_pp_grid(const K3WgParams& p);
int msseg_k3wg_pp_launch(const K3WgParams& p, int gx, hipStream_t stream);

struct StemParams {
    const void* x; long long ldx;
    const void* wp;
    const float* bias;
    void* y; long long ldy;
    int N, D, H, W, M;
    float* stats; float* stats_ws;
    int taps;
    const float* nstats; const float* gamma; const float* beta; float eps, slope;
};
struct StemWgParams {
    const void* x; long long ldx;
    const void* dy; long long lddy;
    float* slabs;
    int N, D, H, W, M;
};
bool msseg_stem_eligible(int dtype, int Cin, int Cout, int k, int s, int pd, long long ldx, long long ldy, const void* y);
int msseg_stem_fwd_launch(const StemParams& p, hipStream_t stream);
int msseg_stem_wgrad_grid(const StemWgParams& p);
int msseg_stem_wgrad_launch(const StemWgParams& p, int gx, hipStream_t stream);

bool msseg_deconv2_fast_eligible(int dtype, int Cin, int Cout, const void* coarse, long long ldc, const void* fine,
                                 long long ldf, const float* bias);
int msseg_deconv2_fwd_launch(const void* x, long long ldx, const void* wp, const float* bias, void* y, long long ldy, int N,
                             int D, int H, int W, int Cin, int Cout, hipStream_t stream);
int msseg_deconv2_bwd_launch(const void* dy, long long lddy, const void* wp, void* dx, long long lddx, int N, int D, int H,
                             int W, int Cin, int Cout, const void* yraw, long long ldyraw, const void* act, long long ldact,
                             const float* fwd_stats, float slope, float eps, float* red, float* dgamma, float* dbeta,
                             int accumulate, float* dbias, int dbias_accumulate, void* scratch, size_t scratch_bytes,
                             hipStream_t stream);

bool msseg_deconv2g_fwd_eligible(int dtype, int Cin, int Cout, const void* coarse, long long ldc, const void* fine,
                                 long long ldf, const float* bias);
int msseg_deconv2g_fwd_launch(const void* x, long long ldx, const void* wp, const float* bias, void* y, long long ldy, int N,
                              int D, int H, int W, int Cin, int Cout, hipStream_t stream);
bool msseg_deconv2g_bwd_eligible(int dtype, int Cin, int Cout, const void* coarse, long long ldc, const void* fine,
                                 long long ldf);
int msseg_deconv2g_bwd_launch(const void* dy, long long lddy, const void* wp, void* dx, long long lddx, float* part, int N,
                              int D, int H, int W, int Cin, int Cout, hipStream_t stream);
bool msseg_linear_regw_eligible(int dtype, long long NV, int Cin, int Cout, const void* x, long long ldx, const void* y,
                                long long ldy, const float* bias);
int msseg_linear_regw_launch(const void* x, long long ldx, const void* wp, const float* bias, void* y, long long ldy,
                             long long NV, int Cin, int Cout, hipStream_t stream);
```

medicalsemseg_amd/hip.py:

```python
from __future__ import annotations

import ctypes as C
import os
from typing import Optional

import torch

_HERE = os.path.dirname(os.path.abspath(__file__))
LIB_PATH = os.environ.get("MSSEG_LIB") or os.path.join(_HERE, "libmsseg_hip.so")

F32, BF16 = 0, 1
_DT = {torch.float32: F32, torch.bfloat16: BF16}
_LAB = {torch.float32: 0, torch.bfloat16: 1, torch.uint8: 2, torch.int64: 3}

_lib = None

_vp, _ll, _i, _f, _sz = C.c_void_p, C.c_longlong, C.c_int, C.c_float, C.c_size_t

SIGNATURES = {
    "msseg_abi_version": ([], _i),
    "msseg_last_error": ([], C.c_char_p),
    "msseg_num_cus": ([], _i),
    "msseg_packed_weight_bytes": ([_i, _i, _i, _i, _i], _sz),
    "msseg_pack_weights": ([_vp, _vp, _i, _i, _i, _i, _i, _i, _ll, _ll, _ll, _ll, _ll, _i, _i, _vp], _i),
    "msseg_pack_weights_batch": ([_vp, _i, _ll, _ll, _i, _vp], _i),
    "msseg_cout_block": ([_i], _i),
    "msseg_conv3d_k3_cout_block": ([_i, _i, _i, _i, _i], _i),
    "msseg_conv3d_k3_variant": ([_i, _i, _i, _i, _i], _i),
    "msseg_conv3d_k3_kernel": ([_i, _i, _i, _i, _i, _i, _i], _i),
    "msseg_conv3d_k3_fwd": ([_vp, _ll, _vp, _vp, _vp, _ll, _i, _i, _i, _i, _i, _i, _vp, _vp, _sz, _i, _vp], _i),
    "msseg_conv3d_k3_fwd_accumulate": ([_vp, _ll, _vp, _vp, _ll, _i, _i, _i, _i, _i, _i, _vp, _vp, _sz, _i, _vp], _i),
    "msseg_dwconv3d_k3_fwd": ([_vp, _ll, _vp, _vp, _vp, _ll, _i, _i, _i, _i, _i, _i, _i, _vp], _i),
    "msseg_dwconv3d_k3_wgrad": ([_vp, _ll, _vp, _ll, _vp, _vp, _i, _i, _i, _i, _i, _i, _i, _vp, _sz, _i, _vp], _i),
    "msseg_interp_trilinear_fwd": ([_vp, _ll, _vp, _ll, _i, _i, _i, _i, _i, _i, _i, _i, _i, _vp], _i),
    "msseg_interp_trilinear_bwd_workspace_bytes": ([_i, _i, _i, _i, _i, _i, _i, _i], _sz),
    "msseg_interp_trilinear_bwd": ([_vp, _ll, _vp, _ll, _i, _i, _i, _i, _i, _i, _i, _i, _vp, _sz, _i, _vp], _i),
    "msseg_kv_attention_fwd": ([_vp, _vp, _vp, _vp, _i, _i, _i, _i, _i, _f, _i, _vp], _i),
    "msseg_kv_attention_bwd_workspace_bytes": ([_i, _i, _i, _i, _i], _sz),
    "msseg_kv_attention_bwd": ([_vp, _vp, _vp, _vp, _vp, _vp, _vp, _i, _i, _i, _i, _i, _f, _vp, _sz, _i, _vp], _i),
    "msseg_scale_channels": ([_vp, _vp, _vp, _i, _ll, _i, _i, _vp], _i),
    "msseg_reduce_scratch_bytes": ([], _sz),
    "msseg_conv3d_k3_dgrad_inbwd": ([_vp, _ll, _vp, _vp, _ll, _i, _i, _i, _i, _i, _i, _vp, _ll, _vp, _ll, _vp, _f, _f, _vp,
                                     _vp, _vp, _i, _vp, _sz, _i, _vp], _i),
    "msseg_conv3d_k1_dgrad_inbwd": ([_vp, _ll, _vp, _vp, _ll, _i, _ll, _i, _i, _vp, _ll, _vp, _ll, _vp, _f, _f, _vp,
                                     _vp, _vp, _i, _vp, _sz, _i, _vp], _i),
    "msseg_deconv_k2s2_bwd_data_inbwd": ([_vp, _ll, _vp, _vp, _ll, _i, _i, _i, _i, _i, _i, _vp, _ll, _vp, _ll, _vp, _f, _f,
                                          _vp, _vp, _vp, _i, _vp, _sz, _i, _vp], _i),
    "msseg_deconv_k2s2_bwd_fused": ([_vp, _ll, _vp, _vp, _ll, _i, _i, _i, _i, _i, _i, _vp, _ll, _vp, _ll, _vp, _f, _f,
                                     _vp, _vp, _vp, _i, _vp, _i, _vp, _sz, _i, _vp], _i),
    "msseg_conv3d_k3s2_fwd": ([_vp, _ll, _vp, _vp, _vp, _ll, _i, _i, _i, _i, _i, _i, _i, _vp], _i),
    "msseg_zero_stuff2": ([_vp, _ll, _vp, _ll, _i, _i, _i, _i, _i, _i, _i, _i, _i, _vp], _i),
    "msseg_window_attention_fwd": ([_vp, _vp, _vp, _vp, _vp, _i, _i, _i, _i, _i, _i, _i, _i, _i, _vp], _i),
    "msseg_window_attention_bwd": ([_vp, _vp, _vp, _vp, _vp, _vp, _vp, _vp, _i, _i, _i, _i, _i, _i, _i, _i, _i, _vp], _i),
    "msseg_window_attention_bwd_ws": ([_vp, _vp, _vp, _vp, _vp, _vp, _vp, _vp, _i, _i, _i, _i, _i, _i, _i, _i, _i, _vp,
                                       _sz, _vp], _i),
    "msseg_window_attention_fwd2": ([_vp, _vp, _vp, _vp, _vp, _i, _i, _i, _i, _i, _i, _i, _i, _i, _i, _vp], _i),
    "msseg_window_attention_bwd2": ([_vp, _vp, _vp, _vp, _vp, _vp, _vp, _vp, _i, _i, _i, _i, _i, _i, _i, _i, _i, _i, _vp,
                                     _sz, _vp], _i),
    "msseg_window_attention_bwd_workspace_bytes": ([_i, _i, _i, _i, _i, _i, _i, _i, _i], _sz),
    "msseg_window_attention_fwd3": ([_vp, _vp, _vp, _vp, _vp, _i, _i, _i, _i, _i, _i, _i, _i, _i, _ll, _i, _vp], _i),
    "msseg_window_attention_bwd3": ([_vp, _vp, _vp, _vp, _vp, _vp, _vp, _vp, _i, _i, _i, _i, _i, _i, _i, _i, _i, _ll, _i,
                                     _vp, _sz, _vp], _i),
    "msseg_window_attention_bwd3_workspace_bytes": ([_i, _i, _i, _i, _i, _i, _i, _i, _i, _ll, _i], _sz),
    "msseg_rel_bias_affine_fold": ([_vp, _vp, _vp, _vp, _vp, _vp, _i, _i, _i, _vp], _i),
    "msseg_rel_bias_affine_grad_workspace_bytes": ([_i, _i], _sz),
    "msseg_rel_bias_affine_grad": ([_vp, _vp, _vp, _vp, _vp, _vp, _vp, _vp, _i, _i, _i, _i, _vp, _sz, _vp], _i),
    "msseg_layernorm_fwd": ([_vp, _ll, _vp, _vp, _vp, _ll, _vp, _vp, _ll, _i, _f, _i, _vp], _i),
    "msseg_layernorm_bwd": ([_vp, _ll, _vp, _vp, _vp, _vp, _ll, _vp, _ll, _ll, _i, _i, _vp], _i),
    "msseg_layernorm_bwd_add": ([_vp, _ll, _vp, _vp, _vp, _vp, _ll, _vp, _ll, _vp, _ll, _ll, _i, _i, _vp], _i),
    "msseg_layernorm_param_grad": ([_vp, _ll, _vp, _vp, _vp, _ll, _vp, _vp, _i, _ll, _i, _vp, _sz, _i, _vp], _i),
    "msseg_gelu_fwd": ([_vp, _vp, _ll, _i, _vp], _i),
    "msseg_gelu_bwd": ([_vp, _vp, _vp, _ll, _i, _vp], _i),
    "msseg_linear_wgrad_ok": ([_ll, _i, _i, _i], _i),
    "msseg_linear_wgrad": ([_vp, _ll, _vp, _ll, _vp, _vp, _ll, _i, _i, _i, _i, _vp, _sz, _i, _vp], _i),
    "msseg_linear_gelu_ok": ([_ll, _i, _i, _i], _i),
    "msseg_linear_gelu_fwd": ([_vp, _ll, _vp, _vp, _vp, _ll, _vp, _ll, _ll, _i, _i, _i, _vp], _i),
    "msseg_linear_gelu_bwd": ([_vp, _ll, _vp, _vp, _ll, _vp, _ll, _ll, _i, _i, _i, _vp], _i),
    "msseg_linear_add_ok": ([_ll, _i, _i, _i], _i),
    "msseg_linear_add_fwd": ([_vp, _ll, _vp, _vp, _vp, _ll, _vp, _ll, _ll, _i, _i, _i, _vp], _i),
    "msseg_conv3d_stem_fwd": ([_vp, _ll, _vp, _vp, _vp, _ll, _i, _i, _i, _i, _i, _vp, _vp, _sz, _i, _vp], _i),
    "msseg_conv3d_stem_k1_fwd": ([_vp, _ll, _vp, _vp, _vp, _ll, _i, _i, _i, _i, _i, _vp, _vp, _sz, _i, _vp], _i),
    "msseg_conv3d_stem_norm_fwd": ([_vp, _ll, _vp, _vp, _vp, _vp, _vp, _f, _f, _vp, _ll, _i, _i, _i, _i, _i, _i, _vp], _i),
    "msseg_conv3d_k1_head_dgrad_inbwd": ([_vp, _ll, _vp, _vp, _ll, _i, _ll, _i, _i, _vp, _ll, _vp, _vp, _vp, _f, _f, _vp, _vp,
                                          _vp, _i, _vp, _sz, _i, _vp], _i),
    "msseg_conv3d_k1_head_norm_fwd": ([_vp, _ll, _vp, _vp, _vp, _f, _f, _vp, _vp, _vp, _ll, _i, _ll, _i, _i, _i, _vp], _i),
    "msseg_conv3d_k1_head_bwd_fused": ([_vp, _ll, _vp, _vp, _ll, _i, _ll, _i, _i, _vp, _ll, _vp, _vp, _vp, _f, _f, _vp, _vp,
                                        _vp, _i, _vp, _i, _vp, _sz, _i, _vp], _i),
    "msseg_conv3d_k1_head_fwd": ([_vp, _ll, _vp, _vp, _vp, _ll, _ll, _i, _i, _i, _vp], _i),
    "msseg_conv3d_k1_fwd": ([_vp, _ll, _vp, _vp, _vp, _ll, _ll, _i, _i, _i, _vp], _i),
    "msseg_conv3d_gather_fwd": ([_vp, _ll, _vp, _vp, _vp, _ll, _i, _i, _i, _i, _i, _i, _i, _i, _i, _i, _vp], _i),
    "msseg_deconv_k2s2_fwd": ([_vp, _ll, _vp, _vp, _vp, _ll, _i, _i, _i, _i, _i, _i, _i, _vp], _i),
    "msseg_deconv_k2s2_bwd_data": ([_vp, _ll, _vp, _vp, _ll, _i, _i, _i, _i, _i, _i, _i, _vp], _i),
    "msseg_deconv_k4s4_fwd": ([_vp, _ll, _vp, _vp, _vp, _ll, _i, _i, _i, _i, _i, _i, _i, _vp], _i),
    "msseg_deconv_k4s4_bwd_data": ([_vp, _ll, _vp, _vp, _ll, _i, _i, _i, _i, _i, _i, _i, _vp], _i),
    "msseg_wgrad_workspace_bytes": ([_i, _i, _i], _sz),
    "msseg_conv3d_k3_wgrad_kernel": ([_i, _i, _i, _i, _i, _i, _i], _i),
    "msseg_conv3d_k3_wgrad": ([_vp, _ll, _vp, _ll, _vp, _i, _i, _i, _i, _i, _i, _i, _vp, _sz, _i, _vp], _i),
    "msseg_conv3d_k1_wgrad": ([_vp, _ll, _vp, _ll, _vp, _ll, _i, _i, _i, _vp, _sz, _i, _vp], _i),
    "msseg_conv3d_gather_wgrad": ([_vp, _ll, _vp, _ll, _vp, _i, _i, _i, _i, _i, _i, _i, _i, _i, _i, _vp, _sz, _i, _vp], _i),
    "msseg_deconv_k2s2_wgrad": ([_vp, _ll, _vp, _ll, _vp, _i, _i, _i, _i, _i, _i, _i, _vp, _sz, _i, _vp], _i),
    "msseg_deconv_k4s4_wgrad": ([_vp, _ll, _vp, _ll, _vp, _i, _i, _i, _i, _i, _i, _i, _vp, _sz, _i, _vp], _i),
    "msseg_channel_stats": ([_vp, _ll, _vp, _i, _ll, _i, _vp, _sz, _i, _vp], _i),
    "msseg_instnorm_act_fwd": ([_vp, _ll, _vp, _vp, _vp, _vp, _ll, _vp, _ll, _i, _ll, _i, _f, _f, _i, _vp], _i),
    "msseg_instnorm_act_poolbwd_reduce": ([_vp, _ll, _vp, _vp, _vp, _vp, _ll, _vp, _ll, _vp, _ll, _vp, _vp, _vp, _i,
                                           _i, _i, _i, _i, _i, _f, _f, _vp, _sz, _i, _vp], _i),
    "msseg_instnorm_act_pool_fwd": ([_vp, _ll, _vp, _vp, _vp, _vp, _ll, _vp, _ll, _i, _i, _i, _i, _i, _f, _f, _i, _vp], _i),
    "msseg_instnorm_act_bwd_reduce": ([_vp, _ll, _vp, _vp, _vp, _vp, _ll, _vp, _ll, _vp, _vp, _vp, _i, _i, _ll, _i, _f, _f, _vp, _sz, _i, _vp], _i),
    "msseg_instnorm_act_bwd_apply": ([_vp, _ll, _vp, _vp, _vp, _vp, _ll, _vp, _ll, _vp, _vp, _ll, _vp, _ll, _i, _ll, _i, _f, _f, _i, _vp], _i),
    "msseg_maxpool2_fwd": ([_vp, _ll, _vp, _ll, _i, _i, _i, _i, _i, _i, _vp], _i),
    "msseg_maxpool2_bwd": ([_vp, _ll, _vp, _ll, _vp, _ll, _i, _i, _i, _i, _i, _i, _i, _vp], _i),
    "msseg_ncdhw_to_ndhwc": ([_vp, _i, _vp, _ll, _i, _i, _i, _ll, _vp], _i),
    "msseg_ndhwc_to_ncdhw": ([_vp, _ll, _i, _vp, _i, _i, _i, _ll, _vp], _i),
    "msseg_channel_sum": ([_vp, _ll, _vp, _ll, _i, _i, _vp, _sz, _i, _vp], _i),
    "msseg_axpy_rows": ([_vp, _vp, _vp, _vp, _i, _ll, _i, _vp], _i),
    "msseg_add": ([_vp, _ll, _vp, _ll, _vp, _ll, _ll, _i, _i, _vp], _i),
    "msseg_dice_ce_partials": ([_vp, _ll, _i, _vp, _i, _vp, _vp, _i, _ll, _i, _vp], _i),
    "msseg_dice_ce_fwd": ([_vp, _ll, _i, _vp, _i, _vp, _vp, _vp, _i, _ll, _i, _f, _f, _vp, _sz, _vp], _i),
    "msseg_dice_ce_finalize": ([_vp, _vp, _i, _ll, _i, _f, _f, _vp], _i),
    "msseg_dice_ce_bwd": ([_vp, _ll, _i, _vp, _i, _vp, _vp, _vp, _ll, _i, _ll, _i, _f, _f, _vp], _i),
    "msseg_adamw_step": ([_vp, _vp, _vp, _vp, _vp, _ll, _f, _f, _f, _f, _f, _i, _vp, _vp, _vp], _i),
    "msseg_sumsq": ([_vp, _ll, _vp, _vp, _i, _vp], _i),
    "msseg_sw_blend": ([_vp, _ll, _i, _vp, _vp, _vp, _i, _i, _i, _i, _i, _i, _i, _i, _i, _i, _vp], _i),
    "msseg_sw_normalize": ([_vp, _vp, _i, _ll, _vp], _i),
    "msseg_sw_gather": ([_vp, _vp, _i, _i, _i, _i, _i, _i, _i, _i, _i, _i, _i, _f, _vp], _i),
    "msseg_box_copy": ([_vp, _ll, _i, _i, _i, _vp, _ll, _i, _i, _i, _i, _i, _i, _vp], _i),
    "msseg_merge_gather_fwd": ([_vp, _ll, _i, _i, _i, _vp, _ll, _i, _i, C.c_uint, _i, _vp], _i),
    "msseg_merge_gather_bwd": ([_vp, _ll, _vp, _ll, _i, _i, _i, _i, _i, C.c_uint, _i, _vp], _i),
    "msseg_argmax_u8": ([_vp, _i, _ll, _vp, _vp], _i),
    "msseg_resample_nearest_u8": ([_vp, _i, _i, _i, _vp, _i, _i, _i, _vp], _i),
    "msseg_majority_vote_u8": ([_vp, _i, _ll, _i, _vp, _vp], _i),
    "msseg_aug_crop_batch": ([_vp, _vp, _i, _i, _i, _i, _vp, _i, _vp, _i, _vp, _i, _vp], _i),
    "msseg_intensity_prep": ([_vp, _i, _i, _i, _i, _i, _i, _f, _f, _i, _f, _f, _vp, _vp, _vp], _i),
    "msseg_resample_spacing": ([_vp, _i, _i, _i, _i, _i, _vp, _i, _i, _i, C.c_double, C.c_double, C.c_double, _vp], _i),
    "msseg_crop_pad_copy": ([_vp, _i, _i, _i, _i, _i, _vp, _vp, _i, _i, _i, _vp, _f, _i, _vp], _i),
    "msseg_slab_counts": ([_vp, _vp, _i, _i, _i, _f, _vp, _vp], _i),
    "msseg_pick_voxels": ([_vp, _i, _vp, _i, _i, _f, _vp, _vp], _i),
    "msseg_aug_crop_multi": ([_vp, _i, _vp, _vp, _i, _i, _vp, _i, _vp, _i, _vp], _i),
    "msseg_sw_gather_batch": ([_vp, _ll, _vp, _ll, _i, _vp, _i, _i, _i, _i, _i, _i, _i, _i, _f, _vp], _i),
    "msseg_sw_blend_batch": ([_vp, _ll, _i, _vp, _vp, _ll, _vp, _ll, _vp, _i, _i, _i, _i, _i, _i, _i, _i, _vp], _i),
    "msseg_deconv_k2s2_bwd_partials_ok": ([_i, _i, _i], _i),
    "msseg_deconv_k2s2_bwd_partials": ([_vp, _ll, _vp, _vp, _sz, _i, _i, _i, _i, _i, _i, _i, _vp], _i),
    "msseg_conv3d_k3_small_ok": ([_i, _i, _i, _i, _i, _i, _i], _i),
    "msseg_conv3d_k3_small_workspace_bytes": ([_i, _i, _i, _i, _i, _i], _sz),
    "msseg_conv3d_k3_small_stage_groups": ([_i, _i, _i, _i, _i, _i], _i),
    "msseg_conv3d_k3_small_partials": ([_vp, _ll, _vp, _vp, _sz, _i, _i, _i, _i, _i, _i, _vp], _i),
    "msseg_conv3d_k3_small_fwd_finish": ([_vp, _i, _vp, _vp, _vp, _f, _f, _vp, _ll, _vp, _ll, _vp, _ll, _vp, _i, _i, _i, _i,
                                          _i, _vp], _i),
    "msseg_conv3d_k3_small_fwd_finish_res": ([_vp, _i, _vp, _vp, _vp, _f, _f, _vp, _ll, _vp, _ll, _vp, _ll, _vp, _ll, _vp, _i, _i, _i, _i,
                                              _i, _vp], _i),
    "msseg_conv3d_k3_small_bwd_finish": ([_vp, _i, _vp, _ll, _vp, _ll, _vp, _vp, _vp, _f, _f, _vp, _vp, _i, _i, _i, _i, _i,
                                          _i, _vp], _i),
    "msseg_avgpool3d_k3": ([_vp, _ll, _vp, _ll, _i, _i, _i, _i, _i, _i, _vp], _i),
    "msseg_hd_edges": ([_vp, _vp, _i, _i, _i, _i, _vp, _vp, _vp, _vp], _i),
    "msseg_hd_directed_workspace_bytes": ([_i, _i, _i], _sz),
    "msseg_hd_directed_hist": ([_vp, _vp, _i, _i, _i, _i, _vp, _vp, _sz, _vp, _i, _vp], _i),
    "msseg_ktimer_enable": ([_i], _i),
    "msseg_ktimer_reset": ([], _i),
    "msseg_ktimer_count": ([], _i),
    "msseg_ktimer_get": ([_i, C.c_char_p, _i, C.POINTER(C.c_float)], _i),
}


def load_library(path: Optional[str] = None):
    global _lib
    if _lib is not None and path is None:
        return _lib
    p = path or LIB_PATH
    if not os.path.exists(p):
        raise RuntimeError(
            f"{p} not found: build it with `python -c 'import __graft_entry__ as g; g.build()'` "
            f"(or `make -C medicalsemseg_amd/csrc`).  There is no CPU fallback.")
    lib = C.CDLL(p)
    for name, (args, res) in SIGNATURES.items():
        fn = getattr(lib, name)
        fn.argtypes = args
        fn.restype = res
    if lib.msseg_abi_version() != 1:
        raise RuntimeError("libmsseg_hip.so ABI version mismatch")
    _lib = lib
    return lib


def lib():
    real = _lib if _lib is not None else load_library()
    if TIMER.enabled:
        return _TimedLib(real)
    return real


class MssegError(RuntimeError):
# ... 218 lines not shown
    torch.cuda.synchronize()
    out = {}
    buf = C.create_string_buffer(96)
    ms = C.c_float()
    for i in range(L.msseg_ktimer_count()):
        if L.msseg_ktimer_get(i, buf, 96, C.byref(ms)) == 0:
            r = out.setdefault(buf.value.decode(), {"launches": 0, "total_ms": 0.0})
            r["launches"] += 1
            r["total_ms"] += float(ms.value)
    for r in out.values():
        r["avg_ms"] = r["total_ms"] / r["launches"]
    if reset:
        L.msseg_ktimer_reset()
    return out


TIMER = KernelTimer()


_scratch_cache = {}


def scratch(device) -> torch.Tensor:
    key = device.index if device.index is not None else torch.cuda.current_device()
    buf = _scratch_cache.get(key)
    if buf is None:
        buf = torch.zeros(lib().msseg_reduce_scratch_bytes() + 256, dtype=torch.uint8, device=device)
        off = (-buf.data_ptr()) % 256
        buf = buf[off:off + lib().msseg_reduce_scratch_bytes()]
        _scratch_cache[key] = buf
    return buf


def conv3d_k3(x, wp, bias, y, cin, cout, stats=None):
    _need_gpu(x, wp, y)
    N, D, H, W = x.shape[:4]
    nv = N * D * H * W
    esz = x.element_size()
    sc = scratch(x.device) if stats is not None else None

    def go():
        _ck(lib().msseg_conv3d_k3_fwd(_p(x), ld(x), _p(wp), _p(bias), _p(y), ld(y), N, D, H, W, cin, cout, _p(stats),
                                      _p(sc), sc.numel() if sc is not None else 0, dt(x), _stream()), "conv3d_k3_fwd")
    key = "conv3d_k3_fwd"
    if TIMER.enabled:
        key += "/v%d" % lib().msseg_conv3d_k3_kernel(N, D, H, W, cin, cout, dt(x))
    TIMER.launch(key, 2.0 * nv * 27 * cin * cout, nv * (cin + cout) * esz + 27 * cin * cout * esz, go)
    return y


def conv3d_k3_accumulate(x, wp, y, cin, cout, stats):
    _need_gpu(x, wp, y, stats)
    N, D, H, W = x.shape[:4]
    nv = N * D * H * W
    sc = scratch(x.device)
    TIMER.launch("conv3d_k3_fwd/v%d" % (4 if cin == 48 else 3), 2.0 * nv * 27 * cin * cout, nv * (cin + 2 * cout) * x.element_size() + 27 * cin * cout * 2,
                 lambda: _ck(lib().msseg_conv3d_k3_fwd_accumulate(_p(x), ld(x), _p(wp), _p(y), ld(y), N, D, H, W, cin, cout,
                                                                 _p(stats), _p(sc), sc.numel(), dt(x), _stream()),
                             "conv3d_k3_fwd_accumulate"))
    return y


def conv3d_k3_dgrad_inbwd(dy, wp, da, cin, cout, yraw, act, fwd_stats, slope, eps, dgamma=None, dbeta=None,
                          accumulate=False):
    _need_gpu(dy, wp, da, yraw, act, fwd_stats)
    N, D, H, W = dy.shape[:4]
    nv = N * D * H * W
    esz = dy.element_size()
    red = torch.empty(N, cout, 2, dtype=torch.float32, device=dy.device)
    sc = scratch(dy.device)

    def go():
        _ck(lib().msseg_conv3d_k3_dgrad_inbwd(_p(dy), ld(dy), _p(wp), _p(da), ld(da), N, D, H, W, cin, cout, _p(yraw),
                                              ld(yraw), _p(act), ld(act), _p(fwd_stats), slope, eps, _p(red),
                                              _p(dgamma), _p(dbeta), int(accumulate), _p(sc), sc.numel(), dt(dy),
                                              _stream()), "conv3d_k3_dgrad_inbwd")
    key = "conv3d_k3_fwd"
    if TIMER.enabled:
        key += "/v%d" % lib().msseg_conv3d_k3_kernel(N, D, H, W, cin, cout, dt(dy))
    TIMER.launch(key, 2.0 * nv * 27 * cin * cout, nv * (cin + 3 * cout) * esz + 27 * cin * cout * esz, go)
    return red


def conv3d_k3_small_ok(x, cin, cout) -> bool:
    if os.environ.get("MSSEG_NO_K3_SMALL") or x.dim() != 5 or x.dtype != torch.bfloat16:
        return False
    N, D, H, W = x.shape[:4]
    return bool(lib().msseg_conv3d_k3_small_ok(N, D, H, W, cin, cout, BF16))


_k3s_ws = {}


def _k3s_workspace(nbytes, device):
    key = device.index if device.index is not None else torch.cuda.current_device()
    buf = _k3s_ws.get(key)
    if buf is None or buf.numel() * 4 < nbytes:
        if buf is not None:
            _ws_retired.append(buf)
        buf = torch.empty(max(nbytes, 32 << 20) // 4, dtype=torch.float32, device=device)
        _k3s_ws[key] = buf
    return buf


def conv3d_k3_small_partials(x, wp, cin, cout):
    _need_gpu(x, wp)
    N, D, H, W = x.shape[:4]
    nv = N * D * H * W
    ng = lib().msseg_conv3d_k3_small_stage_groups(N, D, H, W, cin, cout)
    part = _k3s_workspace(lib().msseg_conv3d_k3_small_workspace_bytes(N, D, H, W, cin, cout), x.device)
    TIMER.launch("conv3d_k3_small", 2.0 * nv * 27 * cin * cout, nv * (cin * x.element_size() + ng * cout * 4) + 27 * cin * cout * 2,
                 lambda: _ck(lib().msseg_conv3d_k3_small_partials(_p(x), ld(x), _p(wp), _p(part), part.numel() * 4, N, D, H, W, cin,
                                                                  cout, _stream()), "conv3d_k3_small_partials"))
    return part, ng


def deconv_k2s2_small_unit_ok(dx_shape, cin, cout, dtype) -> bool:
    if os.environ.get("MSSEG_NO_K3_SMALL") or dtype != torch.bfloat16 or len(dx_shape) != 5:
        return False
    N, D, H, W = dx_shape[:4]
    return N <= 8 and D * H * W <= 2048 and bool(lib().msseg_deconv_k2s2_bwd_partials_ok(cin, cout, BF16))


def deconv_k2s2_bwd_partials(dy, wp, cin, cout):
    _need_gpu(dy, wp)
    N, D, H, W = dy.shape[0], dy.shape[1] // 2, dy.shape[2] // 2, dy.shape[3] // 2
    nv = N * D * H * W
    part = _k3s_workspace(nv * cin * 4, dy.device)
    TIMER.launch("deconv_k2s2_bwd_partials", 2.0 * nv * 8 * cin * cout, nv * (8 * cout * dy.element_size() + cin * 4) + 8 * cin * cout * 2,
                 lambda: _ck(lib().msseg_deconv_k2s2_bwd_partials(_p(dy), ld(dy), _p(wp), _p(part), part.numel() * 4, N, D, H, W, cin,
                                                                  cout, dt(dy), _stream()), "deconv_k2s2_bwd_partials"))
    return part


def conv3d_k3_small_fwd_finish(part, nstages, bias, gamma, beta, eps, slope, yraw, act, pooled, stats, residual=None):
    _need_gpu(part, yraw, act, stats)
    N, D, H, W, cout = yraw.shape
    _ck(lib().msseg_conv3d_k3_small_fwd_finish_res(_p(part), nstages, _p(bias), _p(gamma), _p(beta), eps, slope, _p(yraw), ld(yraw),
                                                   _p(act), ld(act), _p(residual), ld(residual) if residual is not None else 0,
                                                   _p(pooled), ld(pooled) if pooled is not None else 0,
                                                   _p(stats), N, D, H, W, cout, _stream()), "conv3d_k3_small_fwd_finish")


def conv3d_k3_small_bwd_finish(part, nstages, dx, unit=None, dgamma=None, dbeta=None, accumulate=False):
    _need_gpu(part, dx)
    N, D, H, W, cin = dx.shape
    uy = ustats = ug = ub = None
    eps, slope = 1e-5, 1.0
    if unit is not None:
        uy, ustats, ug, ub, eps, slope = unit
    _ck(lib().msseg_conv3d_k3_small_bwd_finish(_p(part), nstages, _p(dx), ld(dx), _p(uy), ld(uy) if uy is not None else 0,
                                               _p(ustats), _p(ug), _p(ub), eps, slope, _p(dgamma), _p(dbeta),
                                               int(accumulate), N, D, H, W, cin, _stream()), "conv3d_k3_small_bwd_finish")
    return dx


def conv3d_k1_head(x, w, bias, y, cin, cout):
    _need_gpu(x, w, y)
    nv = x.numel() // x.shape[-1]
    _ck(lib().msseg_conv3d_k1_head_fwd(_p(x), ld(x), _p(w), _p(bias), _p(y), ld(y), nv, cin, cout, dt(x), _stream()),
        "conv3d_k1_head_fwd")
    return y


def conv3d_k1_head_dgrad_inbwd(dy, w, da, cin, cout, yraw, fwd_stats, gamma, beta, slope, eps, dgamma=None, dbeta=None,
                               accumulate=False):
# ... 275 lines not shown
    N, ID, IH, IW, C = x.shape
    _ck(lib().msseg_interp_trilinear_fwd(_p(x), ld(x), _p(y), ld(y), N, ID, IH, IW, y.shape[1], y.shape[2], y.shape[3], C,
                                         dt(x), _stream()), "interp_trilinear_fwd")
    return y


def interp_trilinear_bwd(dy, dx):
    _need_gpu(dy, dx)
    N, ID, IH, IW, C = dx.shape
    OD, OH, OW = dy.shape[1:4]
    nb = lib().msseg_interp_trilinear_bwd_workspace_bytes(N, ID, IH, IW, OD, OH, OW, C)
    ws = torch.empty(nb, dtype=torch.uint8, device=dx.device)
    _ck(lib().msseg_interp_trilinear_bwd(_p(dy), ld(dy), _p(dx), ld(dx), N, ID, IH, IW, OD, OH, OW, C, _p(ws), nb, dt(dx),
                                         _stream()), "interp_trilinear_bwd")
    return dx


def kv_attention_fwd(q, kv, heads, scale):
    _need_gpu(q, kv)
    B, N, C = q.shape
    M = kv.shape[1]
    o = torch.empty_like(q)
    lse = torch.empty(B, heads, N, dtype=torch.float32, device=q.device)
    _ck(lib().msseg_kv_attention_fwd(_p(q), _p(kv), _p(o), _p(lse), B, N, M, heads, C // heads, scale, dt(q), _stream()),
        "kv_attention_fwd")
    return o, lse


def kv_attention_bwd(q, kv, o, lse, dout, heads, scale):
    _need_gpu(q, kv, o, lse, dout)
    B, N, C = q.shape
    M = kv.shape[1]
    dq, dkv = torch.empty_like(q), torch.empty_like(kv)
    nb = lib().msseg_kv_attention_bwd_workspace_bytes(B, N, M, heads, C // heads)
    ws = torch.empty(nb, dtype=torch.uint8, device=q.device)
    _ck(lib().msseg_kv_attention_bwd(_p(q), _p(kv), _p(o), _p(lse), _p(dout), _p(dq), _p(dkv), B, N, M, heads, C // heads,
                                     scale, _p(ws), nb, dt(q), _stream()), "kv_attention_bwd")
    return dq, dkv


def scale_channels(x, scale, y):
    _need_gpu(x, scale, y)
    N, C = x.shape[0], x.shape[-1]
    _ck(lib().msseg_scale_channels(_p(x), _p(scale), _p(y), N, x.numel() // (N * C), C, dt(x), _stream()), "scale_channels")
    return y


def channel_stats(x, stats=None):
    _need_gpu(x)
    N, S, Cc = _nsc(x)
    if stats is None:
        stats = torch.empty(N, Cc, 2, dtype=torch.float32, device=x.device)
    sc = scratch(x.device)
    _ck(lib().msseg_channel_stats(_p(x), ld(x), _p(stats), N, S, Cc, _p(sc), sc.numel(), dt(x), _stream()),
        "channel_stats")
    return stats


def instnorm_act_fwd(x, stats, gamma, beta, y, slope, eps=1e-5, residual=None):
    _need_gpu(x, stats, y)
    N, S, Cc = _nsc(x)
    TIMER.launch("instnorm_act_fwd", 0.0, _nbytes(x, y, residual), lambda: _ck(lib().msseg_instnorm_act_fwd(_p(x), ld(x), _p(stats), _p(gamma), _p(beta), _p(residual),
                                     ld(residual) if residual is not None else 0, _p(y), ld(y), N, S, Cc, eps, slope,
                                     dt(x), _stream()), "instnorm_act_fwd"))
    return y


def instnorm_pool_ok(x, y, pooled) -> bool:
    epc = 16 // x.element_size()
    return (x.dim() == 5 and all(int(d) % 2 == 0 for d in x.shape[1:4]) and x.shape[-1] % epc == 0
            and all(ld(t) % epc == 0 and t.data_ptr() % 16 == 0 for t in (x, y, pooled)))


def instnorm_act_pool_fwd(x, stats, gamma, beta, y, pooled, slope, eps=1e-5):
    _need_gpu(x, stats, y, pooled)
    N, D, H, W, Cc = x.shape
    TIMER.launch("instnorm_act_pool_fwd", 0.0, _nbytes(x, y, pooled), lambda: _ck(lib().msseg_instnorm_act_pool_fwd(_p(x), ld(x), _p(stats), _p(gamma), _p(beta), _p(y), ld(y), _p(pooled), ld(pooled),
                                          N, D, H, W, Cc, eps, slope, dt(x), _stream()), "instnorm_act_pool_fwd"))
    return y, pooled


def instnorm_act_poolbwd_reduce(x, stats, gamma, beta, skip, g, da, slope, eps=1e-5, dgamma=None, dbeta=None,
                                accumulate=False):
    _need_gpu(x, stats, skip, g, da)
    N, D, H, W, Cc = x.shape
    red = torch.empty(N, Cc, 2, dtype=torch.float32, device=x.device)
    sc = scratch(x.device)
    TIMER.launch("instnorm_act_poolbwd_reduce", 0.0, _nbytes(x, skip, g, da), lambda: _ck(lib().msseg_instnorm_act_poolbwd_reduce(_p(x), ld(x), _p(stats), _p(gamma), _p(beta), _p(skip), ld(skip), _p(g),
                                                ld(g), _p(da), ld(da), _p(red), _p(dgamma), _p(dbeta), int(accumulate),
                                                N, D, H, W, Cc, eps, slope, _p(sc), sc.numel(), dt(x), _stream()),
        "instnorm_act_poolbwd_reduce"))
    return red


def instnorm_act_bwd(x, stats, gamma, y, dy, dx, slope, eps=1e-5, dres=None, dgamma=None, dbeta=None,
                     accumulate=False, beta=None):
    _need_gpu(x, stats, dy, dx)
    red = instnorm_act_bwd_reduce(x, stats, gamma, y, dy, slope, eps, dgamma, dbeta, accumulate, beta)
    instnorm_act_bwd_apply(x, stats, gamma, y, dy, red, dx, slope, eps, dres, beta)
    return red


def instnorm_act_bwd_reduce(x, stats, gamma, y, dy, slope, eps=1e-5, dgamma=None, dbeta=None, accumulate=False, beta=None):
    _need_gpu(x, stats, dy)
    N, S, Cc = _nsc(x)
    red = torch.empty(N, Cc, 2, dtype=torch.float32, device=x.device)
    sc = scratch(x.device)
    TIMER.launch("instnorm_act_bwd_reduce", 0.0, _nbytes(x, y, dy), lambda: _ck(lib().msseg_instnorm_act_bwd_reduce(_p(x), ld(x), _p(stats), _p(gamma), _p(beta), _p(y),
                                            ld(y) if y is not None else 0, _p(dy), ld(dy), _p(red),
                                            _p(dgamma), _p(dbeta), int(accumulate), N, S, Cc, eps, slope, _p(sc),
                                            sc.numel(), dt(x), _stream()), "instnorm_act_bwd_reduce"))
    return red


def instnorm_act_bwd_apply(x, stats, gamma, y, dy, red, dx, slope, eps=1e-5, dres=None, beta=None):
    _need_gpu(x, stats, dy, dx, red)
    N, S, Cc = _nsc(x)
    TIMER.launch("instnorm_act_bwd_apply", 0.0, _nbytes(x, y, dy, dx, dres), lambda: _ck(lib().msseg_instnorm_act_bwd_apply(_p(x), ld(x), _p(stats), _p(gamma), _p(beta), _p(y),
                                           ld(y) if y is not None else 0, _p(dy), ld(dy), _p(red),
                                           _p(dx), ld(dx), _p(dres), ld(dres) if dres is not None else 0, N, S, Cc, eps,
                                           slope, dt(x), _stream()), "instnorm_act_bwd_apply"))
    return red


def maxpool2_fwd(x, y):
    _need_gpu(x, y)
    N, D, H, W, Cc = x.shape
    _ck(lib().msseg_maxpool2_fwd(_p(x), ld(x), _p(y), ld(y), N, D, H, W, Cc, dt(x), _stream()), "maxpool2_fwd")
    return y


def maxpool2_bwd(x, dy, dx, accumulate=False):
    _need_gpu(x, dy, dx)
    N, D, H, W, Cc = x.shape
    _ck(lib().msseg_maxpool2_bwd(_p(x), ld(x), _p(dy), ld(dy), _p(dx), ld(dx), N, D, H, W, Cc, int(accumulate), dt(x),
                                 _stream()), "maxpool2_bwd")
    return dx


def to_channels_last(src: torch.Tensor, dst: torch.Tensor):
    _need_gpu(src, dst)
    src = src.contiguous()
    N, Cc = src.shape[0], src.shape[1]
    S = src.numel() // (N * Cc)
    _ck(lib().msseg_ncdhw_to_ndhwc(_p(src), dt(src), _p(dst), ld(dst), dt(dst), N, Cc, S, _stream()), "ncdhw_to_ndhwc")
    return dst


def to_channels_first(src: torch.Tensor, dst: torch.Tensor):
    _need_gpu(src, dst)
    N, Cc = dst.shape[0], dst.shape[1]
    S = dst.numel() // (N * Cc)
    assert dst.is_contiguous()
    _ck(lib().msseg_ndhwc_to_ncdhw(_p(src), ld(src), dt(src), _p(dst), dt(dst), N, Cc, S, _stream()), "ndhwc_to_ncdhw")
    return dst


def channel_sum(x, out, accumulate=False):
    _need_gpu(x, out)
    Cc = x.shape[-1]
    rows = x.numel() // Cc
    sc = scratch(x.device)
    _ck(lib().msseg_channel_sum(_p(x), ld(x), _p(out), rows, Cc, int(accumulate), _p(sc), sc.numel(), dt(x),
                                _stream()), "channel_sum")
    return out


def axpy_rows(a, b, scale, y):
    _need_gpu(b, y)
    assert b.is_contiguous() and y.is_contiguous() and (a is None or a.is_contiguous())
    N = b.shape[0]
    _ck(lib().msseg_axpy_rows(_p(a), _p(b), _p(scale), _p(y), N, b.numel() // N, dt(b), _stream()), "axpy_rows")
    return y


# ... 470 lines not shown
```

medicalsemseg_amd/layers.py:

```python
from __future__ import annotations

import os

from typing import Optional

import torch

from . import hip

weights_epoch = 0


def bump_weights_epoch():
    global weights_epoch
    weights_epoch += 1


class _PackRegistry:

    def __init__(self):
        self.groups = {}

    def add(self, device, dtype, src, dst, job):
        g = self.groups.setdefault((device, dtype), {"jobs": [], "table": None, "keep": []})
# ... 168 lines not shown
        h = self.halves_ok(vol, dtype)
        y = _empty_like_vol(x, self.cout)
        stats = torch.empty(x.shape[0], self.cout, 2, dtype=torch.float32, device=x.device)
        for i in range(self.cin // h):
            wi = self.w.detach()[:, i * h:(i + 1) * h]
            pi = self.cache.get(wi, dtype, ("fp", i, h, vol), lambda wi=wi: hip.pack_conv_k3(wi, dtype, vol=vol))
            xi = x[..., i * h:(i + 1) * h]
            if i == 0:
                hip.conv3d_k3(xi, pi, self.b, y, h, self.cout)
            else:
                hip.conv3d_k3_accumulate(xi, pi, y, h, self.cout, stats)
        return y, stats

    def split_ok(self, vol, dtype, ca, cb_) -> bool:
        if (os.environ.get("MSSEG_NO_SPLIT_CAT") or dtype != torch.bfloat16 or ca + cb_ != self.cin or ca != 32 or cb_ != 32
                or self.cout % 32 or vol[0] > 8):
            return False
        return hip.lib().msseg_conv3d_k3_kernel(*vol, 32, self.cout, hip.BF16) == 3

    def fwd_split(self, xa, xb):
        dtype = xa.dtype
        vol = tuple(xa.shape[:4])
        wa, wb = self.w.detach()[:, :32], self.w.detach()[:, 32:]
        pa = self.cache.get(wa, dtype, ("fa", vol), lambda: hip.pack_conv_k3(wa, dtype, vol=vol))
        pb = self.cache.get(wb, dtype, ("fb", vol), lambda: hip.pack_conv_k3(wb, dtype, vol=vol))
        y = _empty_like_vol(xa, self.cout)
        hip.conv3d_k3(xa, pa, self.b, y, 32, self.cout)
        stats = torch.empty(xa.shape[0], self.cout, 2, dtype=torch.float32, device=xa.device)
        hip.conv3d_k3_accumulate(xb, pb, y, 32, self.cout, stats)
        return y, stats

    def dgrad_accumulate_ok(self, dy) -> bool:
        if dy.dtype != torch.bfloat16 or self.cout not in (32, 48) or dy.shape[0] > 4 or os.environ.get("MSSEG_NO_DGRAD_ACCUM"):
            return False
        vol = tuple(dy.shape[:4])
        return hip.lib().msseg_conv3d_k3_kernel(*vol, self.cout, self.cin, hip.BF16) == (4 if self.cout == 48 else 3)

    def bwd(self, x, dy, need_dx=True, dx_out=None, bias_grad_is_zero=False, next_norm=None, accumulate_dx=False):
        dtype = x.dtype
        if self.w.requires_grad:
            g, acc = _grad_buf(self.w)
            if self._gather(dtype):
                hip.conv3d_gather_wgrad(x, dy, g, self.cin, self.cout, 3, 1, 1, acc)
            else:
                hip.conv3d_k3_wgrad(x, dy, g, self.cin, self.cout, acc)
        if self.b is not None and self.b.requires_grad:
            g, acc = _grad_buf(self.b)
            if bias_grad_is_zero:
                if not acc and not getattr(self.b, "_msseg_grad_is_zero", False):
                    g.zero_()
                    self.b._msseg_grad_is_zero = getattr(self.b, "_msseg_gowner", None) is not None
            else:
                hip.channel_sum(dy, g, acc)
        if not need_dx:
            return None
        if self._gather(dtype):
            raise NotImplementedError("input gradient of a few-channel stem conv is never needed on this path")
        vol = tuple(dy.shape[:4])
        if accumulate_dx:
            assert dx_out is not None and next_norm is None and self.dgrad_accumulate_ok(dy)
            wp = self.cache.get(self.w, dtype, ("d", vol),
                                lambda: hip.pack_conv_k3(self.w.detach(), dtype, dgrad=True, vol=vol))
            unused = torch.empty(dy.shape[0], self.cin, 2, dtype=torch.float32, device=dy.device)
            hip.conv3d_k3_accumulate(dy, wp, dx_out, self.cout, self.cin, unused)
            return dx_out
        if hip.conv3d_k3_small_ok(dy, self.cout, self.cin):
            wp = self.cache.get(self.w, dtype, "ds", lambda: hip.pack_conv_k3(self.w.detach(), dtype, dgrad=True, cb=32))
            part, ng = hip.conv3d_k3_small_partials(dy, wp, self.cout, self.cin)
            dx = dx_out if dx_out is not None else _empty_like_vol(dy, self.cin)
            if next_norm is not None:
                nrm, yraw, stats, act = next_norm
                dg, db, acc = _norm_grad_bufs(nrm)
                hip.conv3d_k3_small_bwd_finish(part, ng, dx, (yraw, stats, nrm.gamma, nrm.beta, nrm.eps, nrm.slope),
                                               dg, db, acc)
                return dx, APPLIED
            return hip.conv3d_k3_small_bwd_finish(part, ng, dx)
        wp = self.cache.get(self.w, dtype, ("d", vol),
                            lambda: hip.pack_conv_k3(self.w.detach(), dtype, dgrad=True, vol=vol))
        dx = dx_out if dx_out is not None else _empty_like_vol(dy, self.cin)
        if next_norm is not None:
            nrm, yraw, stats, act = next_norm
            if dy.shape[0] <= 8 and self.cin % 4 == 0:
                dg, db, acc = _norm_grad_bufs(nrm)
                red = hip.conv3d_k3_dgrad_inbwd(dy, wp, dx, self.cout, self.cin, yraw, act, stats, nrm.slope, nrm.eps,
                                                dg, db, acc)
                return dx, red
            hip.conv3d_k3(dy, wp, None, dx, self.cout, self.cin)
            return dx, None
        hip.conv3d_k3(dy, wp, None, dx, self.cout, self.cin)
        return dx


class Conv1:

    def __init__(self, weight, bias):
        self.w, self.b = weight, bias
        self.cout, self.cin = weight.shape[0], weight.shape[1]
        self.cache = PackedCache()

    def _gather(self, dtype):
        return self.cin % (8 if dtype == torch.bfloat16 else 4) != 0

    def fwd(self, x, out=None, want_stats=False):
        dtype = x.dtype
        y = out if out is not None else _empty_like_vol(x, self.cout)
        if self._gather(dtype):
            wp = self.cache.get(self.w, dtype, "g", lambda: hip.pack_conv_gather(self.w.detach(), dtype))
            if (want_stats and self.cin == 1 and dtype == torch.bfloat16 and x.dim() == 5 and x.shape[0] <= 8 and hip.ld(y) == self.cout
                    and (self.cout % 32 == 0 or self.cout % 48 == 0) and self.cout <= 256):
                stats = torch.empty(x.shape[0], self.cout, 2, dtype=torch.float32, device=x.device)
                hip.conv3d_stem(x, wp, self.b, y, self.cout, stats, k=1)
                return y, stats
            hip.conv3d_gather(x, wp, self.b, y, self.cin, self.cout, 1, 1, 0)
        elif self.cout <= 4 and self.cin <= 64 and x.shape[-1] == self.cin and self.w.is_contiguous():
            hip.conv3d_k1_head(x, self.w.detach(), self.b, y, self.cin, self.cout)
        else:
            wp = self.cache.get(self.w, dtype, "f",
                                lambda: hip.pack_conv_k1(self.w.detach().reshape(self.cout, self.cin), dtype))
            hip.conv3d_k1(x, wp, self.b, y, self.cin, self.cout)
        if want_stats:
            return y, hip.channel_stats(y)
        return y

    def head_norm_ok(self, yraw) -> bool:
        epc = 16 // yraw.element_size()
        return (self.cout <= 4 and self.cin <= 64 and self.cin % epc == 0 and yraw.shape[-1] == self.cin
                and hip.ld(yraw) % epc == 0 and yraw.data_ptr() % 16 == 0 and self.w.is_contiguous())

    def fwd_norm(self, yraw, stats, nrm, out):
        return hip.conv3d_k1_head_norm(yraw, stats, nrm.gamma, nrm.beta, nrm.slope, nrm.eps, self.w.detach(), self.b, out,
                                       self.cin, self.cout)

    def bwd_norm(self, dy, dy_channels, nrm, yraw, stats):
        dyk = dy[..., :dy_channels]
        dx = torch.empty(yraw.shape, dtype=yraw.dtype, device=yraw.device)
        dg, db, acc = _norm_grad_bufs(nrm)
        if self.b is not None and self.b.requires_grad:
            g, bacc = _grad_buf(self.b)
            hip.channel_sum(dy[..., :self.cout], g, bacc)
        if self.w.requires_grad:
            gw, wacc = _grad_buf(self.w)
            red = hip.conv3d_k1_head_bwd_fused(dyk, self.w.detach(), dx, self.cin, self.cout, yraw, stats, nrm.gamma, nrm.beta,
                                               nrm.slope, nrm.eps, gw, wacc, dg, db, acc)
        else:
            red = hip.conv3d_k1_head_dgrad_inbwd(dyk, self.w.detach(), dx, self.cin, self.cout, yraw, stats, nrm.gamma,
                                                 nrm.beta, nrm.slope, nrm.eps, dg, db, acc)
        return dx, red

    def bwd(self, x, dy, need_dx=True, dy_channels=None, next_norm=None):
        dtype = x.dtype
        fused_bias = False
        if self.w.requires_grad:
            g, acc = _grad_buf(self.w)
            if self._gather(dtype):
                hip.conv3d_gather_wgrad(x, dy[..., :self.cout], g, self.cin, self.cout, 1, 1, 0, acc)
            elif hip.linear_wgrad_ok(x, self.cin, self.cout):
                gb, bacc = _grad_buf(self.b) if (self.b is not None and self.b.requires_grad) else (None, False)
                hip.linear_wgrad(x, dy[..., :self.cout], g.view(self.cout, self.cin), gb, self.cin, self.cout, acc, bacc)
                fused_bias = True
            else:
                hip.conv3d_k1_wgrad(x, dy[..., :self.cout], g, self.cin, self.cout, acc)
        if self.b is not None and self.b.requires_grad and not fused_bias:
            g, acc = _grad_buf(self.b)
            hip.channel_sum(dy[..., :self.cout], g, acc)
        if not need_dx:
            return None
# ... 43 lines not shown
        if k == 4:
            hip.deconv_k4s4(x, wp, self.b, y, self.cin, self.cout)
        else:
            hip.deconv_k2s2(x, wp, self.b, y, self.cin, self.cout)
        return y

    def _bwd_k4(self, x, dy, need_dx, next_norm):
        dtype = x.dtype
        if self.w.requires_grad:
            g, acc = _grad_buf(self.w)
            hip.deconv_k4s4_wgrad(x, dy, g, self.cin, self.cout, acc)
        if self.b is not None and self.b.requires_grad:
            g, acc = _grad_buf(self.b)
            hip.channel_sum(dy, g, acc)
        if not need_dx:
            return None
        wp = self.cache.get(self.w, dtype, "d", lambda: hip.pack_deconv(self.w.detach(), dtype, bwd=True))
        dx = torch.empty_like(x, memory_format=torch.contiguous_format)
        hip.deconv_k4s4_bwd_data(dy, wp, dx, self.cin, self.cout)
        return (dx, None) if next_norm is not None else dx

    def bwd(self, x, dy, need_dx=True, next_norm=None):
        if self.k == 4:
            return self._bwd_k4(x, dy, need_dx, next_norm)
        dtype = x.dtype
        if self.w.requires_grad:
            g, acc = _grad_buf(self.w)
            hip.deconv_k2s2_wgrad(x, dy, g, self.cin, self.cout, acc)
        want_db = self.b is not None and self.b.requires_grad
        if not need_dx:
            if want_db:
                g, acc = _grad_buf(self.b)
                hip.channel_sum(dy, g, acc)
            return None
        wp = self.cache.get(self.w, dtype, "d", lambda: hip.pack_deconv(self.w.detach(), dtype, bwd=True))
        dx = torch.empty_like(x, memory_format=torch.contiguous_format)
        db, dbacc = _grad_buf(self.b) if want_db else (None, False)
        if next_norm is not None and hip.deconv_k2s2_small_unit_ok(tuple(x.shape), self.cin, self.cout, dtype):
            nrm, yraw, stats, act = next_norm
            part = hip.deconv_k2s2_bwd_partials(dy, wp, self.cin, self.cout)
            dg, dbt, nacc = _norm_grad_bufs(nrm)
            hip.conv3d_k3_small_bwd_finish(part, 1, dx, (yraw, stats, nrm.gamma, nrm.beta, nrm.eps, nrm.slope), dg, dbt, nacc)
            if want_db:
                hip.channel_sum(dy, db, dbacc)
            return dx, APPLIED
        nn_ = None
        dg = dbt = None
        nacc = False
        if next_norm is not None:
            nrm, yraw, stats, act = next_norm
            if dy.shape[0] <= 8 and self.cin % 4 == 0:
                dg, dbt, nacc = _norm_grad_bufs(nrm)
                nn_ = (yraw, act, stats, nrm.slope, nrm.eps)
        red = hip.deconv_k2s2_bwd_fused(dy, wp, dx, self.cin, self.cout, nn_, db, dbacc, dg, dbt, nacc)
        return (dx, red) if next_norm is not None else dx


Deconv4 = Deconv2


class InstNormAct:

    def __init__(self, gamma: Optional[torch.nn.Parameter], beta: Optional[torch.nn.Parameter], slope: float,
                 eps: float = 1e-5):
        self.gamma, self.beta, self.slope, self.eps = gamma, beta, float(slope), float(eps)

    def fwd(self, y_raw, out=None, residual=None, stats=None, pooled=None):
        if stats is None:
            stats = hip.channel_stats(y_raw)
        a = out if out is not None else torch.empty_like(y_raw, memory_format=torch.contiguous_format)
        if pooled is not None:
            if residual is None and hip.instnorm_pool_ok(y_raw, a, pooled):
                hip.instnorm_act_pool_fwd(y_raw, stats, self.gamma, self.beta, a, pooled, self.slope, self.eps)
                return a, stats
            hip.instnorm_act_fwd(y_raw, stats, self.gamma, self.beta, a, self.slope, self.eps, residual)
            hip.maxpool2_fwd(a, pooled)
            return a, stats
        hip.instnorm_act_fwd(y_raw, stats, self.gamma, self.beta, a, self.slope, self.eps, residual)
        return a, stats

    def pool_bwd_reduce(self, y_raw, stats, skip_grad, pooled_grad):
        if not hip.instnorm_pool_ok(y_raw, skip_grad, pooled_grad):
            return None
        da = torch.empty(y_raw.shape, dtype=y_raw.dtype, device=y_raw.device)
        dg, db, acc = _norm_grad_bufs(self)
        red = hip.instnorm_act_poolbwd_reduce(y_raw, stats, self.gamma, self.beta, skip_grad, pooled_grad, da, self.slope,
                                              self.eps, dg, db, acc)
        return da, red

    def bwd(self, y_raw, stats, a, da, want_dres=False, red=None):
        if red is APPLIED:
            if want_dres:
                raise RuntimeError("a residual unit cannot take an already-applied gradient")
            return da
        dy = torch.empty(y_raw.shape, dtype=y_raw.dtype, device=y_raw.device)
        dres = torch.empty(y_raw.shape, dtype=y_raw.dtype, device=y_raw.device) if want_dres else None
        a_in = a if want_dres else None
        if red is not None:
            hip.instnorm_act_bwd_apply(y_raw, stats, self.gamma, a_in, da, red, dy, self.slope, self.eps, dres, self.beta)
            return (dy, dres) if want_dres else dy
        dg = db = None
        acc = False
        if self.gamma is not None and self.gamma.requires_grad:
            dg, acc = _grad_buf(self.gamma)
            db, acc2 = _grad_buf(self.beta)
            assert acc == acc2
        hip.instnorm_act_bwd(y_raw, stats, self.gamma, a_in, da, dy, self.slope, self.eps, dres, dg, db, acc, self.beta)
        return (dy, dres) if want_dres else dy


class ConvNormAct:

    def __init__(self, conv: Conv3, norm: InstNormAct):
        self.conv, self.norm = conv, norm

    def fwd(self, x, out=None, pooled=None):
        cv, nm = self.conv, self.norm
        if (INFERENCE_FORWARD and pooled is None and cv.cin == 1 and x.dtype == torch.bfloat16 and x.shape[0] <= 8
                and (cv.cout % 32 == 0 or cv.cout % 48 == 0) and cv.cout <= 256 and not os.environ.get("MSSEG_NO_STEM_TWICE")):
            wp = cv.cache.get(cv.w, x.dtype, "g", lambda: hip.pack_conv_gather(cv.w.detach(), x.dtype))
            stats = torch.empty(x.shape[0], cv.cout, 2, dtype=torch.float32, device=x.device)
            hip.conv3d_stem(x, wp, cv.b, None, cv.cout, stats)
            a = out if out is not None else _empty_like_vol(x, cv.cout)
            hip.conv3d_stem_norm(x, wp, cv.b, stats, nm.gamma, nm.beta, nm.eps, nm.slope, a, cv.cout)
            return a, (x, None, stats, a)
        if (not cv._gather(x.dtype) and hip.conv3d_k3_small_ok(x, cv.cin, cv.cout)
                and (pooled is None or hip.instnorm_pool_ok(x, x, pooled))):
            wp = cv.cache.get(cv.w, x.dtype, "fs", lambda: hip.pack_conv_k3(cv.w.detach(), x.dtype, cb=32))
            part, ng = hip.conv3d_k3_small_partials(x, wp, cv.cin, cv.cout)
            y = _empty_like_vol(x, cv.cout)
            a = out if out is not None else _empty_like_vol(x, cv.cout)
            stats = torch.empty(x.shape[0], cv.cout, 2, dtype=torch.float32, device=x.device)
            hip.conv3d_k3_small_fwd_finish(part, ng, cv.b, nm.gamma, nm.beta, nm.eps, nm.slope, y, a, pooled, stats)
            return a, (x, y, stats, a)
        y, stats = self.conv.fwd(x, want_stats=True)
        a, stats = self.norm.fwd(y, out, stats=stats, pooled=pooled)
        return a, (x, y, stats, a)

    def bwd(self, saved, da, need_dx=True, red=None, next_saved=None, next_cna=None):
        x, y, stats, a = saved
        dy = self.norm.bwd(y, stats, a, da, red=red)
        if next_cna is not None and need_dx:
            nx, ny, nstats, na = next_saved
            return self.conv.bwd(x, dy, True, bias_grad_is_zero=True, next_norm=(next_cna.norm, ny, nstats, na))
        return self.conv.bwd(x, dy, need_dx, bias_grad_is_zero=True)


def maxpool_fwd(x):
    N, D, H, W, C = x.shape
    y = torch.empty(N, D // 2, H // 2, W // 2, C, dtype=x.dtype, device=x.device)
    return hip.maxpool2_fwd(x, y)


class ResBlock:

    def __init__(self, conv1_w, conv2_w, conv3_w=None, slope=0.01):
        self.c1, self.c2 = Conv3(conv1_w, None), Conv3(conv2_w, None)
        self.c3 = Conv1(conv3_w, None) if conv3_w is not None else None
        self.n1, self.n2 = InstNormAct(None, None, slope), InstNormAct(None, None, slope)
        self.n3 = InstNormAct(None, None, 1.0) if conv3_w is not None else None

    @staticmethod
    def _small_unit(conv, nrm, x, residual=None, out=None):
        wp = conv.cache.get(conv.w, x.dtype, "fs", lambda: hip.pack_conv_k3(conv.w.detach(), x.dtype, cb=32))
        part, ng = hip.conv3d_k3_small_partials(x, wp, conv.cin, conv.cout)
        y = _empty_like_vol(x, conv.cout)
        a = out if out is not None else _empty_like_vol(x, conv.cout)
        stats = torch.empty(x.shape[0], conv.cout, 2, dtype=torch.float32, device=x.device)
        hip.conv3d_k3_small_fwd_finish(part, ng, conv.b, nrm.gamma, nrm.beta, nrm.eps, nrm.slope, y, a, None, stats, residual)
        return a, y, stats

    def fwd(self, x, out=None):
        small = (not self.c1._gather(x.dtype) and hip.conv3d_k3_small_ok(x, self.c1.cin, self.c1.cout)
                 and hip.conv3d_k3_small_ok(x, self.c2.cin, self.c2.cout))
        if small:
            a1, y1, s1 = self._small_unit(self.c1, self.n1, x)
        else:
            y1, s1 = self.c1.fwd(x, want_stats=True)
# ... 159 lines not shown
```

Baseline: 536.1 vol/s.

## Recompute norm activations in-kernel to skip materializing pooled-bwd and activation reads

Adds a conv dgrad variant (STATS==4) that recomputes the following norm's activation from yraw, stats, gamma and beta in the epilogue instead of reading the stored activation tensor. Also splits the pool-backward into a reduce pass that no longer writes the full-resolution da and an apply pass that recomputes the pooled gradient while producing the final norm backward output. This avoids writing and re-reading a full-size intermediate gradient and one activation read, at the cost of extra arithmetic and an extra argmax recompute.

```diff
diff --git a/include/msseg.h b/include/msseg.h
--- a/include/msseg.h
+++ b/include/msseg.h
@@ -58,6 +58,11 @@
                                 long long ldact, const float* fwd_stats, float slope, float eps, float* red,
                                 float* dgamma, float* dbeta, int accumulate, void* scratch, size_t scratch_bytes,
                                 int dtype, msseg_stream_t stream);
+int msseg_conv3d_k3_dgrad_inbwd_nz(const void* dy, long long lddy, const void* wp, void* da, long long ldda, int N, int D,
+                                   int H, int W, int Cin, int Cout, const void* yraw, long long ldyraw,
+                                   const float* fwd_stats, const float* gamma, const float* beta, float slope, float eps,
+                                   float* red, float* dgamma, float* dbeta, int accumulate, void* scratch,
+                                   size_t scratch_bytes, int dtype, msseg_stream_t stream);
 int msseg_conv3d_k3s2_fwd(const void* x, long long ldx, const void* wp, const float* bias, void* y, long long ldy,
                           int N, int ID, int IH, int IW, int Cin, int Cout, int dtype, msseg_stream_t stream);
 int msseg_zero_stuff2(const void* dy, long long lddy, void* out, long long ldo, int N, int OD, int OH, int OW, int ID,
@@ -196,6 +201,10 @@
                                       void* da, long long ldda, float* red, float* dgamma, float* dbeta, int accumulate,
                                       int N, int D, int H, int W, int C, float eps, float slope, void* scratch,
                                       size_t scratch_bytes, int dtype, msseg_stream_t stream);
+int msseg_instnorm_act_poolbwd_apply(const void* x, long long ldx, const float* stats, const float* gamma,
+                                     const float* beta, const void* skip, long long lds, const void* g, long long ldg,
+                                     const float* red, void* dx, long long lddx, int N, int D, int H, int W, int C,
+                                     float eps, float slope, int dtype, msseg_stream_t stream);
 int msseg_instnorm_act_bwd_reduce(const void* x, long long ldx, const float* stats, const float* gamma,
                                   const float* beta, const void* y, long long ldy,
                                   const void* dy, long long lddy, float* red, float* dgamma, float* dbeta,
diff --git a/medicalsemseg_amd/csrc/common.h b/medicalsemseg_amd/csrc/common.h
--- a/medicalsemseg_amd/csrc/common.h
+++ b/medicalsemseg_amd/csrc/common.h
@@ -82,6 +82,15 @@
     *(bf16x4_t*)p = o;
 }
 
+MSSEG_DEVFN void mean_rstd(const float* stats, int n, int C, int c, long long S, float eps, float& mean, float& rstd) {
+    const float inv = 1.0f / (float)S;
+    const float s = stats[((long long)n * C + c) * 2 + 0], s2 = stats[((long long)n * C + c) * 2 + 1];
+    mean = s * inv;
+    float var = s2 * inv - mean * mean;
+    var = var > 0.f ? var : 0.f;
+    rstd = rsqrtf(var + eps);
+}
+
 MSSEG_DEVFN float wave_sum(float v) {
 #pragma unroll
     for (int o = 32; o > 0; o >>= 1) v += __shfl_xor(v, o);
diff --git a/medicalsemseg_amd/csrc/conv3d_k3_pp.hip b/medicalsemseg_amd/csrc/conv3d_k3_pp.hip
--- a/medicalsemseg_amd/csrc/conv3d_k3_pp.hip
+++ b/medicalsemseg_amd/csrc/conv3d_k3_pp.hip
@@ -213,9 +213,29 @@
                 s1[j][e] = s2[j][e] = 0.f;
             }
     };
+    float* ldsN = ldsS + STAT_FLOATS + wave * 64;
     auto epilogue = [&](const TileCo& tc) {
         if constexpr (STATS != 0) {
-            if (tc.n != s_n) { flush_stats(); s_n = tc.n; }
+            if (tc.n != s_n) {
+                flush_stats();
+                s_n = tc.n;
+                if constexpr (STATS == 4) {
+#pragma unroll
+                    for (int j = 0; j < 2; ++j)
+#pragma unroll
+                        for (int e = 0; e < 4; ++e) {
+                            const int c = coutblk * 32 + j * 16 + q * 4 + e;
+                            float mean, rstd;
+                            mean_rstd(p.nb_stats, tc.n, p.M, c, p.nb_S, p.nb_eps, mean, rstd);
+                            const float sc = rstd * (p.nb_gamma ? p.nb_gamma[c] : 1.f);
+                            const float sh = (p.nb_beta ? p.nb_beta[c] : 0.f) - mean * sc;
+                            if (r == 0) {
+                                ldsN[j * 16 + q * 4 + e] = sc;
+                                ldsN[32 + j * 16 + q * 4 + e] = sh;
+                            }
+                        }
+                }
+            }
         }
         const long long vox = (((long long)tc.n * p.D + tc.d0) * p.H + tc.h0) * p.W + tc.w0;
         unsigned char* ybase = (unsigned char*)yg + (vox * p.ldy + coutblk * 32) * 2;
@@ -226,7 +246,7 @@
             constexpr bool FULL = decltype(fullc)::value;
             const bool okdw = FULL || (tc.d0 + wq < p.D && tc.w0 + r < p.W);
             u32x2_t y4[TH][2], a4[TH][2];
-            if constexpr (STATS == 2) {
+            if constexpr (STATS == 2 || STATS == 4) {
 #pragma unroll
                 for (int m = 0; m < TH; ++m)
 #pragma unroll
@@ -235,7 +255,7 @@
                         y4[m][j] = a4[m][j] = u32x2_t{0u, 0u};
                         if (ok) {
                             y4[m][j] = *(const u32x2_t*)(nyb + ny_off[m] + j * 32);
-                            a4[m][j] = *(const u32x2_t*)(nab + na_off[m] + j * 32);
+                            if constexpr (STATS == 2) a4[m][j] = *(const u32x2_t*)(nab + na_off[m] + j * 32);
                         }
                     }
             }
@@ -266,6 +286,14 @@
                     if (ok) *(u32x2_t*)(ybase + o_off[m] + j * 32) = ob[m][j];
                 }
             if constexpr (STATS != 0) {
+                f32x4_t nsc[2], nsh[2];
+                if constexpr (STATS == 4) {
+#pragma unroll
+                    for (int j = 0; j < 2; ++j) {
+                        nsc[j] = *(const f32x4_t*)(ldsN + j * 16 + q * 4);
+                        nsh[j] = *(const f32x4_t*)(ldsN + 32 + j * 16 + q * 4);
+                    }
+                }
 #pragma unroll
                 for (int m = 0; m < TH; ++m)
 #pragma unroll
@@ -279,10 +307,13 @@
                                 acc_add(s1[j][e], v);
                                 acc_fma(s2[j][e], v, v);
                             } else {
-                                const float av = bf16_of_pair(a4[m][j][e >> 1], e & 1);
+                                const float yv = bf16_of_pair(y4[m][j][e >> 1], e & 1);
+                                float av;
+                                if constexpr (STATS == 2) av = bf16_of_pair(a4[m][j][e >> 1], e & 1);
+                                else asm("v_fma_f32 %0, %1, %2, %3" : "=v"(av) : "v"(yv), "v"(nsc[j][e]), "v"(nsh[j][e]));
                                 const float dz = v * (av > 0.f ? 1.0f : p.nb_slope);
                                 acc_add(s1[j][e], dz);
-                                acc_fma(s2[j][e], dz, bf16_of_pair(y4[m][j][e >> 1], e & 1));
+                                acc_fma(s2[j][e], dz, yv);
                             }
                         }
                     }
@@ -336,7 +367,7 @@
 }
 
 template <int STATS, int TIMING> int launch(const K3ppParams& p, hipStream_t stream) {
-    const int lds = W_BYTES + 2 * HALO_BYTES + (STATS ? STAT_FLOATS * 4 : 0);
+    const int lds = W_BYTES + 2 * HALO_BYTES + (STATS ? STAT_FLOATS * 4 : 0) + (STATS == 4 ? 8 * 64 * 4 : 0);
     auto kern = k3pp_kernel<STATS, TIMING>;
     static msseg_lds_attr_once attr;
     if (!attr.ensure((const void*)kern, lds)) MSSEG_FAIL(MSSEG_ELAUNCH, "conv3d_k3_pp: cannot set dynamic LDS size %d", lds);
@@ -351,7 +382,7 @@
     if (STATS != 0) {
         K3FinParams f{};
         f.ws = p.stats_ws; f.R = gx; f.N = p.N; f.coutb = 32; f.M = p.M; f.stats = p.stats;
-        f.nb_stats = (STATS == 2) ? p.nb_stats : nullptr; f.nb_eps = p.nb_eps; f.nb_S = p.nb_S;
+        f.nb_stats = (STATS == 2 || STATS == 4) ? p.nb_stats : nullptr; f.nb_eps = p.nb_eps; f.nb_S = p.nb_S;
         f.nb_dgamma = p.nb_dgamma; f.nb_dbeta = p.nb_dbeta; f.nb_acc = p.nb_acc;
         return msseg_k3_stats_finalize(f, ncb, stream);
     }
@@ -379,7 +410,7 @@
     }
     if (p.stats == nullptr) return timing ? launch<0, 1>(p, stream) : launch<0, 0>(p, stream);
     if (p.nb_y == nullptr) return timing ? launch<1, 1>(p, stream) : launch<1, 0>(p, stream);
-    return launch<2, 0>(p, stream);
+    return p.nb_a != nullptr ? launch<2, 0>(p, stream) : launch<4, 0>(p, stream);
 }
 
 extern "C" int msseg_debug_k3pp_cycles(unsigned long long* out8) {
diff --git a/medicalsemseg_amd/csrc/elementwise.hip b/medicalsemseg_amd/csrc/elementwise.hip
--- a/medicalsemseg_amd/csrc/elementwise.hip
+++ b/medicalsemseg_amd/csrc/elementwise.hip
@@ -349,15 +349,6 @@
     float* ws; unsigned int* counter; float* dgamma; float* dbeta; int accumulate;
 };
 
-MSSEG_DEVFN void mean_rstd(const float* stats, int n, int C, int c, long long S, float eps, float& mean, float& rstd) {
-    const float inv = 1.0f / (float)S;
-    const float s = stats[((long long)n * C + c) * 2 + 0], s2 = stats[((long long)n * C + c) * 2 + 1];
-    mean = s * inv;
-    float var = s2 * inv - mean * mean;
-    var = var > 0.f ? var : 0.f;
-    rstd = rsqrtf(var + eps);
-}
-
 template <typename T, bool VEC, int MODE>
 __global__ __launch_bounds__(MODE == 1 ? RED_THREADS : 256) void instnorm_kernel(const NormParams p) {
     constexpr int W = VEC ? DT<T>::EPC : 1;
@@ -577,7 +568,29 @@
     int N, D, H, W, C; float eps, slope;
     int groups, rows_par; long long cells_per_block;
     float* ws;
+    const float* red; void* dx; long long lddx;
 };
+
+template <typename T>
+MSSEG_DEVFN void pool_cell_argmax(const Chunk<T> (&xin)[8], const float* sc, const float* sh, float slope,
+                                  int (&arg)[DT<T>::EPC]) {
+    constexpr int WD = DT<T>::EPC;
+    float best[WD];
+#pragma unroll
+    for (int e = 0; e < WD; ++e) { best[e] = -INFINITY; arg[e] = 0; }
+#pragma unroll
+    for (int k = 0; k < 8; ++k) {
+#pragma unroll
+        for (int e = 0; e < WD; ++e) {
+            const float z = xin[k].v[e] * sc[e] + sh[e];
+            const float a = (float)(T)(z > 0.f ? z : z * slope);
+            if (a > best[e] || a != a) { best[e] = a; arg[e] = k; }
+        }
+    }
+}
+template <typename T> MSSEG_DEVFN float pool_cell_da(float skip, float g, int arg, int k) {
+    return (float)(T)(skip + (arg == k ? g : 0.f));
+}
 
 template <typename T>
 __global__ __launch_bounds__(RED_THREADS) void instnorm_poolbwd_reduce_kernel(const NormPoolBwdParams p) {
@@ -593,7 +606,7 @@
     const T* xn = (const T*)p.x + (long long)n * S * p.ldx;
     const T* sn = (const T*)p.skip + (long long)n * S * p.lds;
     const T* gn = (const T*)p.g + (long long)n * cells * p.ldg;
-    T* dn = (T*)p.da + (long long)n * S * p.ldda;
+    T* dn = p.da ? (T*)p.da + (long long)n * S * p.ldda : nullptr;
     for (int gbase = 0; gbase * WD < p.C; gbase += p.groups) {
         const int gg = gbase + g;
         const bool act = gg * WD < p.C;
@@ -620,32 +633,21 @@
 #pragma unroll
                 for (int k = 0; k < 8; ++k) skin[k].load(sn + vox[k] * p.lds + gg * WD);
                 gv.load(gn + cell * p.ldg + gg * WD);
-                float best[WD];
                 int arg[WD];
-#pragma unroll
-                for (int e = 0; e < WD; ++e) { best[e] = -INFINITY; arg[e] = 0; }
-#pragma unroll
-                for (int k = 0; k < 8; ++k) {
-#pragma unroll
-                    for (int e = 0; e < WD; ++e) {
-                        const float z = xin[k].v[e] * sc[e] + sh[e];
-                        const float a = (float)(T)(z > 0.f ? z : z * p.slope);
-                        if (a > best[e] || a != a) { best[e] = a; arg[e] = k; }
-                    }
-                }
+                pool_cell_argmax<T>(xin, sc, sh, p.slope, arg);
 #pragma unroll
                 for (int k = 0; k < 8; ++k) {
                     Chunk<T> o;
 #pragma unroll
                     for (int e = 0; e < WD; ++e) {
-                        const float dv = (float)(T)(skin[k].v[e] + (arg[e] == k ? gv.v[e] : 0.f));
+                        const float dv = pool_cell_da<T>(skin[k].v[e], gv.v[e], arg[e], k);
                         o.v[e] = dv;
                         const float z = xin[k].v[e] * sc[e] + sh[e];
                         const float dz = z > 0.f ? dv : dv * p.slope;
                         a0[e] += dz;
                         a1[e] += dz * ((xin[k].v[e] - mean[e]) * rstd[e]);
                     }
-                    o.store(dn + vox[k] * p.ldda + gg * WD);
+                    if (dn) o.store(dn + vox[k] * p.ldda + gg * WD);
                 }
             }
         }
@@ -670,6 +672,63 @@
                 wsb[(gg * WD + e) * 2 + 0] = a;
                 wsb[(gg * WD + e) * 2 + 1] = b;
             }
+        }
+    }
+}
+
+template <typename T>
+__global__ __launch_bounds__(256) void instnorm_poolbwd_apply_kernel(const NormPoolBwdParams p) {
+    constexpr int WD = DT<T>::EPC;
+    const int OD = p.D / 2, OH = p.H / 2, OW = p.W / 2;
+    const unsigned ug = (unsigned)(p.C / WD);
+    const unsigned total = (unsigned)((long long)p.N * OD * OH * OW * ug);
+    const long long S = (long long)p.D * p.H * p.W;
+    const float invS = 1.0f / (float)S;
+    for (unsigned i = blockIdx.x * 256u + threadIdx.x; i < total; i += gridDim.x * 256u) {
+        unsigned t = i / ug;
+        const int g = (int)(i - t * ug);
+        unsigned t2 = t / (unsigned)OW;
+        const int ow = (int)(t - t2 * (unsigned)OW);
+        t = t2 / (unsigned)OH;
+        const int oh = (int)(t2 - t * (unsigned)OH);
+        const int n = (int)(t / (unsigned)OD);
+        const int od = (int)(t - (unsigned)n * (unsigned)OD);
+        float mean[WD], rstd[WD], sc[WD], sh[WD], k0[WD], k1[WD];
+#pragma unroll
+        for (int e = 0; e < WD; ++e) {
+            const int c = g * WD + e;
+            mean_rstd(p.stats, n, p.C, c, S, p.eps, mean[e], rstd[e]);
+            sc[e] = rstd[e] * (p.gamma ? p.gamma[c] : 1.f);
+            sh[e] = (p.beta ? p.beta[c] : 0.f) - mean[e] * sc[e];
+            k0[e] = p.red[((long long)n * p.C + c) * 2 + 0] * invS;
+            k1[e] = p.red[((long long)n * p.C + c) * 2 + 1] * invS;
+        }
+        Chunk<T> xin[8], skin[8], gv;
+        long long vox[8];
+#pragma unroll
+        for (int k = 0; k < 8; ++k) {
+            vox[k] = (((long long)n * p.D + 2 * od + (k >> 2)) * p.H + 2 * oh + ((k >> 1) & 1)) * p.W + 2 * ow + (k & 1);
+            xin[k].load((const T*)p.x + vox[k] * p.ldx + g * WD);
+        }
+#pragma unroll
+        for (int k = 0; k < 8; ++k) skin[k].load((const T*)p.skip + vox[k] * p.lds + g * WD);
+        const long long cell = (((long long)n * OD + od) * OH + oh) * OW + ow;
+        gv.load((const T*)p.g + cell * p.ldg + g * WD);
+        int arg[WD];
+        pool_cell_argmax<T>(xin, sc, sh, p.slope, arg);
+#pragma unroll
+        for (int k = 0; k < 8; ++k) {
+            Chunk<T> o;
+#pragma unroll
+            for (int e = 0; e < WD; ++e) {
+                const float xv = xin[k].v[e];
+                const float z = xv * sc[e] + sh[e];
+                const float dv = pool_cell_da<T>(skin[k].v[e], gv.v[e], arg[e], k);
+                const float dz = z > 0.f ? dv : dv * p.slope;
+                const float xh = (xv - mean[e]) * rstd[e];
+                o.v[e] = sc[e] * (dz - k0[e] - xh * k1[e]);
+            }
+            o.store((T*)p.dx + vox[k] * p.lddx + g * WD);
         }
     }
 }
@@ -1474,16 +1533,17 @@
                                       void* da, long long ldda, float* red, float* dgamma, float* dbeta, int accumulate,
                                       int N, int D, int H, int W, int C, float eps, float slope, void* scratch,
                                       size_t scratch_bytes, int dtype, msseg_stream_t stream) {
-    if (!x || !stats || !skip || !g || !da || !red || N < 1 || D < 2 || H < 2 || W < 2 || C < 1)
+    if (!x || !stats || !skip || !g || !red || N < 1 || D < 2 || H < 2 || W < 2 || C < 1)
         MSSEG_FAIL(MSSEG_EINVAL, "instnorm_act_poolbwd_reduce: bad args");
     if ((D | H | W) & 1) MSSEG_FAIL(MSSEG_EINVAL, "instnorm_act_poolbwd_reduce: odd spatial size %dx%dx%d", D, H, W);
     if (dtype != MSSEG_F32 && dtype != MSSEG_BF16) MSSEG_FAIL(MSSEG_EINVAL, "instnorm_act_poolbwd_reduce: bad dtype");
     if (int rc = scratch_ok(scratch, scratch_bytes, "instnorm_act_poolbwd_reduce")) return rc;
     const int esz = dtype == MSSEG_F32 ? 4 : 2;
-    if (!(vec_ok(x, ldx, C, esz) && vec_ok(skip, lds, C, esz) && vec_ok(g, ldg, C, esz) && vec_ok(da, ldda, C, esz)))
+    if (!(vec_ok(x, ldx, C, esz) && vec_ok(skip, lds, C, esz) && vec_ok(g, ldg, C, esz) && (!da || vec_ok(da, ldda, C, esz))))
         MSSEG_FAIL(MSSEG_EINVAL, "instnorm_act_poolbwd_reduce: needs 16-byte aligned rows and a channel count multiple of %d",
                    16 / esz);
-    NormPoolBwdParams p{x, ldx, stats, gamma, beta, skip, lds, g, ldg, da, ldda, N, D, H, W, C, eps, slope, 0, 0, 0, nullptr};
+    NormPoolBwdParams p{x, ldx, stats, gamma, beta, skip, lds, g, ldg, da, ldda, N, D, H, W, C, eps, slope, 0, 0, 0, nullptr,
+                        nullptr, nullptr, 0};
     p.ws = (float*)((unsigned char*)scratch + MSSEG_SCRATCH_COUNTER_BYTES);
     const RowMap m = row_map(C, 16 / esz, RED_THREADS);
     p.groups = m.groups; p.rows_par = m.rows_par;
@@ -1499,6 +1559,29 @@
     FinalizeArgs a{p.ws, N, (int)blocks, C, 2, 2, red, dbeta, dgamma, accumulate};
     hipLaunchKernelGGL(channels_finalize_kernel, channels_finalize_grid(a), dim3(256), 0, (hipStream_t)stream, a);
     MSSEG_CHECK_LAUNCH("channels_finalize");
+    return MSSEG_OK;
+}
+
+int msseg_instnorm_act_poolbwd_apply(const void* x, long long ldx, const float* stats, const float* gamma,
+                                     const float* beta, const void* skip, long long lds, const void* g, long long ldg,
+                                     const float* red, void* dx, long long lddx, int N, int D, int H, int W, int C,
+                                     float eps, float slope, int dtype, msseg_stream_t stream) {
+    if (!x || !stats || !skip || !g || !red || !dx || N < 1 || D < 2 || H < 2 || W < 2 || C < 1)
+        MSSEG_FAIL(MSSEG_EINVAL, "instnorm_act_poolbwd_apply: bad args");
+    if ((D | H | W) & 1) MSSEG_FAIL(MSSEG_EINVAL, "instnorm_act_poolbwd_apply: odd spatial size %dx%dx%d", D, H, W);
+    if (dtype != MSSEG_F32 && dtype != MSSEG_BF16) MSSEG_FAIL(MSSEG_EINVAL, "instnorm_act_poolbwd_apply: bad dtype");
+    const int esz = dtype == MSSEG_F32 ? 4 : 2;
+    if (!(vec_ok(x, ldx, C, esz) && vec_ok(skip, lds, C, esz) && vec_ok(g, ldg, C, esz) && vec_ok(dx, lddx, C, esz)))
+        MSSEG_FAIL(MSSEG_EINVAL, "instnorm_act_poolbwd_apply: needs 16-byte aligned rows and a channel count multiple of %d",
+                   16 / esz);
+    const long long total = (long long)N * (D / 2) * (H / 2) * (W / 2) * (C / (16 / esz));
+    if (total >= 0x7fffffffLL) MSSEG_FAIL(MSSEG_EINVAL, "instnorm_act_poolbwd_apply: too many elements");
+    NormPoolBwdParams p{x, ldx, stats, gamma, beta, skip, lds, g, ldg, nullptr, 0, N, D, H, W, C, eps, slope, 0, 0, 0, nullptr,
+                        red, dx, lddx};
+    const int gr = grid_for(total, 1);
+    DISPATCH_T(dtype, hipLaunchKernelGGL(instnorm_poolbwd_apply_kernel<float>, dim3(gr), dim3(256), 0, (hipStream_t)stream, p),
+               hipLaunchKernelGGL(instnorm_poolbwd_apply_kernel<bf16_t>, dim3(gr), dim3(256), 0, (hipStream_t)stream, p));
+    MSSEG_CHECK_LAUNCH("instnorm_act_poolbwd_apply");
     return MSSEG_OK;
 }
 
diff --git a/medicalsemseg_amd/csrc/igemm_fwd.hip b/medicalsemseg_amd/csrc/igemm_fwd.hip
--- a/medicalsemseg_amd/csrc/igemm_fwd.hip
+++ b/medicalsemseg_amd/csrc/igemm_fwd.hip
@@ -744,6 +744,33 @@
                        act, ldact, fwd_stats, slope, eps, dgamma, dbeta, accumulate, dtype, stream);
 }
 
+int msseg_conv3d_k3_dgrad_inbwd_nz(const void* dy, long long lddy, const void* wp, void* da, long long ldda, int N, int D,
+                                   int H, int W, int Cin, int Cout, const void* yraw, long long ldyraw,
+                                   const float* fwd_stats, const float* gamma, const float* beta, float slope, float eps,
+                                   float* red, float* dgamma, float* dbeta, int accumulate, void* scratch,
+                                   size_t scratch_bytes, int dtype, msseg_stream_t stream) {
+    if (!dy || !wp || !da || !yraw || !fwd_stats || !red) MSSEG_FAIL(MSSEG_EINVAL, "conv3d_k3_dgrad_inbwd_nz: null pointer");
+    if ((dgamma == nullptr) != (dbeta == nullptr)) MSSEG_FAIL(MSSEG_EINVAL, "conv3d_k3_dgrad_inbwd_nz: dgamma/dbeta go together");
+    if ((gamma == nullptr) != (beta == nullptr)) MSSEG_FAIL(MSSEG_EINVAL, "conv3d_k3_dgrad_inbwd_nz: gamma/beta go together");
+    if (N < 1 || D < 1 || H < 1 || W < 1) MSSEG_FAIL(MSSEG_EINVAL, "conv3d_k3_dgrad_inbwd_nz: bad shape");
+    if (!scratch || ((uintptr_t)scratch & 255) || scratch_bytes < msseg_reduce_scratch_bytes())
+        MSSEG_FAIL(MSSEG_EWORKSPACE, "conv3d_k3_dgrad_inbwd_nz: needs the reduce scratch of %zu bytes", msseg_reduce_scratch_bytes());
+    K3ppParams pp{};
+    pp.x = dy; pp.ldx = lddy; pp.wp = wp; pp.y = da; pp.ldy = ldda;
+    pp.N = N; pp.D = D; pp.H = H; pp.W = W; pp.K = Cin; pp.M = Cout;
+    pp.stats = red; pp.counter = (unsigned int*)scratch;
+    pp.stats_ws = (float*)((unsigned char*)scratch + MSSEG_SCRATCH_COUNTER_BYTES);
+    pp.nb_y = yraw; pp.nb_ldy = ldyraw; pp.nb_gamma = gamma; pp.nb_beta = beta; pp.nb_stats = fwd_stats;
+    pp.nb_slope = slope; pp.nb_eps = eps; pp.nb_S = (long long)D * H * W;
+    pp.nb_dgamma = dgamma; pp.nb_dbeta = dbeta; pp.nb_acc = accumulate;
+    int cfg, cb;
+    k3_plan(N, D, H, W, Cout, &cfg, &cb);
+    if (dtype != MSSEG_BF16 || cb != 32 || !msseg_k3pp_eligible(pp))
+        MSSEG_FAIL(MSSEG_EINVAL, "conv3d_k3_dgrad_inbwd_nz: only shapes of the ping-pong kernel (bf16, 32 input channels, "
+                                 "Cout %% 32 == 0, large grids; msseg_conv3d_k3_kernel() == 3)");
+    return msseg_k3pp_launch(pp, (hipStream_t)stream);
+}
+
 static int k3_fwd_impl(const void* x, long long ldx, const void* wp, const float* bias, void* y, long long ldy, int N,
                        int D, int H, int W, int Cin, int Cout, float* stats, void* scratch, size_t scratch_bytes,
                        const void* nb_y, long long nb_ldy, const void* nb_a, long long nb_lda, const float* nb_stats,
diff --git a/medicalsemseg_amd/csrc/k3pp.h b/medicalsemseg_amd/csrc/k3pp.h
--- a/medicalsemseg_amd/csrc/k3pp.h
+++ b/medicalsemseg_amd/csrc/k3pp.h
@@ -14,6 +14,7 @@
     unsigned int* counter;
     const void* nb_y; long long nb_ldy;
     const void* nb_a; long long nb_lda;
+    const float* nb_gamma; const float* nb_beta;
     const float* nb_stats;
     float nb_slope, nb_eps; long long nb_S;
     float* nb_dgamma; float* nb_dbeta; int nb_acc;
diff --git a/medicalsemseg_amd/hip.py b/medicalsemseg_amd/hip.py
--- a/medicalsemseg_amd/hip.py
+++ b/medicalsemseg_amd/hip.py
@@ -42,6 +42,8 @@
     "msseg_reduce_scratch_bytes": ([], _sz),
     "msseg_conv3d_k3_dgrad_inbwd": ([_vp, _ll, _vp, _vp, _ll, _i, _i, _i, _i, _i, _i, _vp, _ll, _vp, _ll, _vp, _f, _f, _vp,
                                      _vp, _vp, _i, _vp, _sz, _i, _vp], _i),
+    "msseg_conv3d_k3_dgrad_inbwd_nz": ([_vp, _ll, _vp, _vp, _ll, _i, _i, _i, _i, _i, _i, _vp, _ll, _vp, _vp, _vp, _f, _f, _vp,
+                                        _vp, _vp, _i, _vp, _sz, _i, _vp], _i),
     "msseg_conv3d_k1_dgrad_inbwd": ([_vp, _ll, _vp, _vp, _ll, _i, _ll, _i, _i, _vp, _ll, _vp, _ll, _vp, _f, _f, _vp,
                                      _vp, _vp, _i, _vp, _sz, _i, _vp], _i),
     "msseg_deconv_k2s2_bwd_data_inbwd": ([_vp, _ll, _vp, _vp, _ll, _i, _i, _i, _i, _i, _i, _vp, _ll, _vp, _ll, _vp, _f, _f,
@@ -106,6 +108,8 @@
                                            _i, _i, _i, _i, _i, _f, _f, _vp, _sz, _i, _vp], _i),
     "msseg_instnorm_act_pool_fwd": ([_vp, _ll, _vp, _vp, _vp, _vp, _ll, _vp, _ll, _i, _i, _i, _i, _i, _f, _f, _i, _vp], _i),
     "msseg_instnorm_act_bwd_reduce": ([_vp, _ll, _vp, _vp, _vp, _vp, _ll, _vp, _ll, _vp, _vp, _vp, _i, _i, _ll, _i, _f, _f, _vp, _sz, _i, _vp], _i),
+    "msseg_instnorm_act_poolbwd_apply": ([_vp, _ll, _vp, _vp, _vp, _vp, _ll, _vp, _ll, _vp, _vp, _ll, _i, _i, _i, _i, _i, _f, _f,
+                                          _i, _vp], _i),
     "msseg_instnorm_act_bwd_apply": ([_vp, _ll, _vp, _vp, _vp, _vp, _ll, _vp, _ll, _vp, _vp, _ll, _vp, _ll, _i, _ll, _i, _f, _f, _i, _vp], _i),
     "msseg_maxpool2_fwd": ([_vp, _ll, _vp, _ll, _i, _i, _i, _i, _i, _i, _vp], _i),
     "msseg_maxpool2_bwd": ([_vp, _ll, _vp, _ll, _vp, _ll, _i, _i, _i, _i, _i, _i, _i, _vp], _i),
@@ -490,6 +494,29 @@
     return red
 
 
+def conv3d_k3_dgrad_inbwd_nz_ok(dy, cin, cout) -> bool:
+    if dy.dim() != 5 or dy.dtype != torch.bfloat16 or cin != 32:
+        return False
+    N, D, H, W = dy.shape[:4]
+    return lib().msseg_conv3d_k3_kernel(N, D, H, W, cin, cout, dt(dy)) == 3
+
+
+def conv3d_k3_dgrad_inbwd_nz(dy, wp, da, cin, cout, yraw, fwd_stats, gamma, beta, slope, eps, dgamma=None, dbeta=None,
+                             accumulate=False):
+    _need_gpu(dy, wp, da, yraw, fwd_stats)
+    N, D, H, W = dy.shape[:4]
+    nv = N * D * H * W
+    esz = dy.element_size()
+    red = torch.empty(N, cout, 2, dtype=torch.float32, device=dy.device)
+    sc = scratch(dy.device)
+    TIMER.launch("conv3d_k3_fwd/v3", 2.0 * nv * 27 * cin * cout, nv * (cin + 2 * cout) * esz + 27 * cin * cout * esz,
+                 lambda: _ck(lib().msseg_conv3d_k3_dgrad_inbwd_nz(_p(dy), ld(dy), _p(wp), _p(da), ld(da), N, D, H, W, cin, cout,
+                                                                 _p(yraw), ld(yraw), _p(fwd_stats), _p(gamma), _p(beta), slope,
+                                                                 eps, _p(red), _p(dgamma), _p(dbeta), int(accumulate), _p(sc),
+                                                                 sc.numel(), dt(dy), _stream()), "conv3d_k3_dgrad_inbwd_nz"))
+    return red
+
+
 def conv3d_k3_small_ok(x, cin, cout) -> bool:
     if os.environ.get("MSSEG_NO_K3_SMALL") or x.dim() != 5 or x.dtype != torch.bfloat16:
         return False
@@ -931,15 +958,24 @@
 
 def instnorm_act_poolbwd_reduce(x, stats, gamma, beta, skip, g, da, slope, eps=1e-5, dgamma=None, dbeta=None,
                                 accumulate=False):
-    _need_gpu(x, stats, skip, g, da)
+    _need_gpu(x, stats, skip, g) if da is None else _need_gpu(x, stats, skip, g, da)
     N, D, H, W, Cc = x.shape
     red = torch.empty(N, Cc, 2, dtype=torch.float32, device=x.device)
     sc = scratch(x.device)
     TIMER.launch("instnorm_act_poolbwd_reduce", 0.0, _nbytes(x, skip, g, da), lambda: _ck(lib().msseg_instnorm_act_poolbwd_reduce(_p(x), ld(x), _p(stats), _p(gamma), _p(beta), _p(skip), ld(skip), _p(g),
-                                                ld(g), _p(da), ld(da), _p(red), _p(dgamma), _p(dbeta), int(accumulate),
+                                                ld(g), _p(da), ld(da) if da is not None else 0, _p(red), _p(dgamma), _p(dbeta), int(accumulate),
                                                 N, D, H, W, Cc, eps, slope, _p(sc), sc.numel(), dt(x), _stream()),
         "instnorm_act_poolbwd_reduce"))
     return red
+
+
+def instnorm_act_poolbwd_apply(x, stats, gamma, beta, skip, g, red, dx, slope, eps=1e-5):
+    _need_gpu(x, stats, skip, g, red, dx)
+    N, D, H, W, Cc = x.shape
+    TIMER.launch("instnorm_act_poolbwd_apply", 0.0, _nbytes(x, skip, g, dx), lambda: _ck(lib().msseg_instnorm_act_poolbwd_apply(
+        _p(x), ld(x), _p(stats), _p(gamma), _p(beta), _p(skip), ld(skip), _p(g), ld(g), _p(red), _p(dx), ld(dx), N, D, H, W, Cc,
+        eps, slope, dt(x), _stream()), "instnorm_act_poolbwd_apply"))
+    return dx
 
 
 def instnorm_act_bwd(x, stats, gamma, y, dy, dx, slope, eps=1e-5, dres=None, dgamma=None, dbeta=None,
diff --git a/medicalsemseg_amd/layers.py b/medicalsemseg_amd/layers.py
--- a/medicalsemseg_amd/layers.py
+++ b/medicalsemseg_amd/layers.py
@@ -274,6 +274,10 @@
             nrm, yraw, stats, act = next_norm
             if dy.shape[0] <= 8 and self.cin % 4 == 0:
                 dg, db, acc = _norm_grad_bufs(nrm)
+                if hip.conv3d_k3_dgrad_inbwd_nz_ok(dy, self.cout, self.cin):
+                    red = hip.conv3d_k3_dgrad_inbwd_nz(dy, wp, dx, self.cout, self.cin, yraw, stats, nrm.gamma, nrm.beta,
+                                                       nrm.slope, nrm.eps, dg, db, acc)
+                    return dx, red
                 red = hip.conv3d_k3_dgrad_inbwd(dy, wp, dx, self.cout, self.cin, yraw, act, stats, nrm.slope, nrm.eps,
                                                 dg, db, acc)
                 return dx, red
@@ -483,11 +487,10 @@
     def pool_bwd_reduce(self, y_raw, stats, skip_grad, pooled_grad):
         if not hip.instnorm_pool_ok(y_raw, skip_grad, pooled_grad):
             return None
-        da = torch.empty(y_raw.shape, dtype=y_raw.dtype, device=y_raw.device)
         dg, db, acc = _norm_grad_bufs(self)
-        red = hip.instnorm_act_poolbwd_reduce(y_raw, stats, self.gamma, self.beta, skip_grad, pooled_grad, da, self.slope,
+        red = hip.instnorm_act_poolbwd_reduce(y_raw, stats, self.gamma, self.beta, skip_grad, pooled_grad, None, self.slope,
                                               self.eps, dg, db, acc)
-        return da, red
+        return (skip_grad, pooled_grad), red
 
     def bwd(self, y_raw, stats, a, da, want_dres=False, red=None):
         if red is APPLIED:
@@ -495,6 +498,12 @@
                 raise RuntimeError("a residual unit cannot take an already-applied gradient")
             return da
         dy = torch.empty(y_raw.shape, dtype=y_raw.dtype, device=y_raw.device)
+        if isinstance(da, tuple):
+            if want_dres or red is None:
+                raise RuntimeError("a (skip_grad, pooled_grad) pair comes with pool_bwd_reduce's sums and no residual")
+            skip_grad, pooled_grad = da
+            return hip.instnorm_act_poolbwd_apply(y_raw, stats, self.gamma, self.beta, skip_grad, pooled_grad, red, dy,
+                                                  self.slope, self.eps)
         dres = torch.empty(y_raw.shape, dtype=y_raw.dtype, device=y_raw.device) if want_dres else None
         a_in = a if want_dres else None
         if red is not None:
```

Result: no change. 532.5 vol/s (-0.7%).
